# dsforza96/yocto-hair

Hardware: AMD Instinct MI355X
Metric: Msamples/sec (whole node), 720x720x1536spp sphere-hairblock; per-pixel L2 vs CPU ref (higher is better)
Workload: dtype f32

## Files before the change

include/yhair.h:

```cpp
#ifndef YHAIR_H_
#define YHAIR_H_

#include <stdint.h>

#ifdef __cplusplus
extern "C" {
#endif

#define YH_OK 0
#define YH_E_INVALID -1
#define YH_E_DEVICE -2
#define YH_E_STATE -3
#define YH_E_IO -4
#define YH_E_SELFTEST -5


typedef struct yh_shape {
  int          num_vertices;
  const float* positions;
  const float* normals;
  const float* radius;
  int          num_lines;
  const int*   lines;
  int          num_triangles;
  const int*   triangles;
  const float* texcoords;
} yh_shape;

typedef struct yh_texture {
  int         width, height;
  int         is_byte;
  const void* pixels;
} yh_texture;

typedef struct yh_material {
  float emission[3];
  float color[3];
  float specular, metallic, roughness, transmission, opacity, ior;
  int   thin;
  float sigma_a[3];
  float beta_m, beta_n, alpha, eta, eumelanin, pheomelanin;
  float scattering[3];
  float scanisotropy;
  float trdepth;
  int   emission_tex, color_tex, scattering_tex;
} yh_material;

typedef struct yh_material_maps {
  int specular_tex;
  int metallic_tex;
  int roughness_tex;
  int transmission_tex;
  int opacity_tex;
  int normal_tex;
} yh_material_maps;

typedef struct yh_object {
  float frame[12];
  int   shape;
  int   material;
} yh_object;

typedef struct yh_environment {
  float        frame[12];
  float        emission[3];
  int          tex_width, tex_height;
  const float* texels;
} yh_environment;

typedef struct yh_camera {
  float frame[12];
  float lens;
  float film[2];
  float focus;
  float aperture;
} yh_camera;

typedef struct yh_scene_desc {
  int                   num_shapes;
  const yh_shape*       shapes;
  int                   num_materials;
  const yh_material*    materials;
  int                   num_objects;
  const yh_object*      objects;
  int                   num_environments;
  const yh_environment* environments;
  yh_camera             camera;
  int                   num_textures;
  const yh_texture*     textures;
} yh_scene_desc;

enum {
  YH_SHADER_NAIVE    = 0,
  YH_SHADER_PATH     = 1,
  YH_SHADER_EYELIGHT = 2,
  YH_SHADER_NORMAL   = 3,
  YH_SHADER_COUNT    = 4
};

typedef struct yh_trace_params {
  int      resolution;
  int      bounces;
  float    clamp;
  uint64_t seed;
  int      shader;
  int      hair_exact;
} yh_trace_params;

typedef struct yh_workcounts {
  uint64_t samples;
  uint64_t rays;
  uint64_t nodes;
  uint64_t seg_tests;
  uint64_t tri_tests;
  uint64_t hair_shades;
  uint64_t surf_shades;
  uint64_t env_lookups;
  uint64_t env_samples;
  uint64_t cyc_trace, cyc_shade, ticks_tile, wave_iters, wave_steps, lane_steps, lane_iters;
  uint64_t cyc_geom, cyc_sample, cyc_eval, cyc_rest;
  uint64_t branch[10];
} yh_workcounts;

typedef struct yh_context yh_context;


yh_context* yh_create(int device);
void        yh_destroy(yh_context* ctx);
const char* yh_last_error(const yh_context* ctx);
const char* yh_version(void);


int yh_upload_scene(yh_context* ctx, const yh_scene_desc* scene);
int yh_upload_scene_maps(yh_context* ctx, const yh_scene_desc* scene, const yh_material_maps* maps);

int yh_init_state(yh_context* ctx, const yh_trace_params* params);
int yh_image_size(const yh_context* ctx, int* width, int* height);

int yh_set_shard(yh_context* ctx, int rank, int world);

int yh_trace_samples(yh_context* ctx, int nsamples);
int yh_trace_samples_async(yh_context* ctx, int nsamples);
int yh_synchronize(yh_context* ctx);

int yh_download(yh_context* ctx, float* rgba);
int yh_pack_tiles_device(yh_context* ctx, void* device_rgba, int64_t capacity,
    int64_t* count);
int yh_unpack_tiles_device(yh_context* ctx, const void* device_packed,
    int src_rank, int world, void* device_image);
int64_t yh_shard_pixels(const yh_context* ctx, int rank, int world);

int yh_gather_framebuffer(yh_context** contexts, int n, float* rgba);

int yh_download_rng(yh_context* ctx, uint64_t* state_inc);

int yh_trace_samples_counted(yh_context* ctx, int nsamples, yh_workcounts* out);

int yh_last_trace_ms(const yh_context* ctx, float* ms, int* launches);

int yh_launch_shape(const yh_context* ctx);
int yh_kernel_trials(const yh_context* ctx, double* ms_per_sample, int* trials, int count);
int yh_trials_pending(const yh_context* ctx);
int         yh_set_trial_cache_dir(const char* dir);
const char* yh_default_trial_cache_dir(void);

int yh_tile_costs(yh_context* ctx, uint32_t* ticks, int count);
int yh_item_costs(yh_context* ctx, uint32_t* costs, int count);


#define YH_HAIR_BRDF_FLOATS 30

enum {
  YH_LOBE_DIFFUSE            = 0,
  YH_LOBE_SPECULAR           = 1,
  YH_LOBE_METAL              = 2,
  YH_LOBE_TRANSMISSION       = 3,
  YH_LOBE_REFRACTION         = 4,
  YH_LOBE_DELTA_SPECULAR     = 5,
  YH_LOBE_DELTA_METAL        = 6,
  YH_LOBE_DELTA_TRANSMISSION = 7,
  YH_LOBE_DELTA_REFRACTION   = 8,
  YH_LOBE_COUNT              = 9
};
#define YH_SURFACE_BSDF_FLOATS 29

int yh_hair_brdf_batch(yh_context* ctx, int n, const yh_material* materials,
    const float* v, const float* normal, const float* tangent, float* brdf);
int yh_hair_eval_batch(yh_context* ctx, int n, const float* brdf,
    const float* outgoing, const float* incoming, float* f);
int yh_hair_sample_batch(yh_context* ctx, int n, const float* brdf,
    const float* outgoing, const float* rn, float* incoming);
int yh_hair_pdf_batch(yh_context* ctx, int n, const float* brdf,
    const float* outgoing, const float* incoming, float* pdf);
int yh_hair_eval_pdf_batch(yh_context* ctx, int n, const float* brdf,
    const float* outgoing, const float* incoming, float* pdf);

int yh_curves_to_lines(yh_context* ctx, int n, const float* P, const float* width0,
    const float* width1, int base_vertex, float* positions, float* normals,
    float* radius, int* lines);

int yh_bvh_build(int n, const float* boxes, float* nodes, int* primitives);
int yh_bvh_build_wide(int n, const float* boxes, int width, float* slots);

int yh_bvh_build_gpu(yh_context* ctx, int n, const float* boxes, float* nodes, int* primitives);
int yh_bvh_build_wide_gpu(yh_context* ctx, int n, const float* boxes, int width, float* slots);

int yh_surface_lobe_batch(yh_context* ctx, int kind, int n, const float* params,
    const float* normal, const float* outgoing, const float* incoming,
    const float* rn, float* out);
int yh_surface_bsdf_batch(yh_context* ctx, int n, const yh_material* materials,
    const float* normal, const float* outgoing, const float* incoming,
    const float* rn, float* out);
int yh_intersect_batch(yh_context* ctx, int n, const float* rays, int* object,
    int* element, float* uv, float* distance);

int yh_lights_batch(yh_context* ctx, int form, int n, const float* position,
    const float* direction, const float* rn, float* out);

int yh_selftest(yh_context* ctx, int which, float* worst);

typedef struct yh_scene_file yh_scene_file;
yh_scene_file*       yh_scene_load(const char* json_path, const char* camera,
          char* error, int error_len);
const yh_scene_desc* yh_scene_get(const yh_scene_file* scene);
const yh_material_maps* yh_scene_get_maps(const yh_scene_file* scene);
void                 yh_scene_free(yh_scene_file* scene);
int yh_save_image(const char* path, int width, int height, const float* rgba,
    char* error, int error_len);

#ifdef __cplusplus
}
#endif
#endif
```

yocto-hair_amd/csrc/dev_items.h:

```cpp
#ifndef YH_DEV_ITEMS_H_
#define YH_DEV_ITEMS_H_
#include "dev_path.h"

using namespace yhd;

#define YH_BLOCK 512
#define YH_MIN_WAVES 4

#define YH_QUADS (YH_BLOCK / 4)
template <bool COUNT, bool GENERAL, int BLOCK, int SHADER, int MODE = YH_MODE_QUAD>
YH_DEV void trace_items(const yhd_scene& sc, const yhd_state& st, int nsamples, yhd_counters* counters, unsigned int block = blockIdx.x,
    unsigned int blocks = gridDim.x) {
  constexpr int LPP    = YH_IS_HEX(MODE) ? 16 : YH_IS_OCT(MODE) ? 8 : 4;
  constexpr int GROUPS = BLOCK / LPP;
  extern __shared__ v4f lds_dyn[];
  YH_LDS unsigned int* lds_stack = (YH_LDS unsigned int*)lds_dyn;
  YH_LDS v4f*          lds_tabs  = (YH_LDS v4f*)(lds_stack + ((MODE == YH_MODE_QUAD ? sc.stack_entries : YH_IS_HEX(MODE) ? sc.stack_entries16 : sc.stack_entries8) + YH_HITROWS) * GROUPS);
  trace_ctx tc;
  tc.sc = &sc;
  tc.ls = nullptr, tc.sc_dev = nullptr;
  YH_LDS float* lds_cam;
  stage_tables(sc, lds_tabs, threadIdx.x, blockDim.x, tc, lds_cam);
  __syncthreads();

  tc.lds_stack = lds_stack + (threadIdx.x / LPP);
  stats_t stats = {};
  tc.stats = COUNT ? &stats : nullptr;

  const int lane = threadIdx.x & 63;
  const int by_position = (int)(blocks * (BLOCK / 64));
  int       t_first     = __builtin_amdgcn_readfirstlane((int)(block * (BLOCK / 64) + (threadIdx.x >> 6)));
  while (true) {
    int t = t_first;
    if (t < 0) {
      if (lane == 0) t = atomicAdd(st.tile_cursor, 1);
      t = __builtin_amdgcn_readfirstlane(t) + by_position;
    }
    t_first = -1;
    if (t >= st.num_tiles) break;
    unsigned long long t0 = wall_clock64();
    int  item  = st.tiles[t];
    int  half  = 0;
    if (YH_IS_OCT(MODE)) half = item & 1, item >>= 1;
    if (YH_IS_HEX(MODE)) half = item & 3, item >>= 2;
    int  tile  = item >> 2, part = item & 3;
    int  pq    = YH_IS_HEX(MODE) ? half * 4 + (lane >> 4) : YH_IS_OCT(MODE) ? half * 8 + (lane >> 3) : lane >> 2;
    int  i     = (tile % st.tiles_x) * YH_TILE + (part & 1) * 4 + (pq & 3);
    int  j     = (tile / st.tiles_x) * YH_TILE + (part >> 1) * 4 + (pq >> 2);
    bool owner = i < st.width && j < st.height;
    size_t pix = owner ? (size_t)j * st.width + i : 0;
    rng_t  rng;
    rng.state      = st.rng_state[pix];
    rng.inc        = st.rng_inc[pix];
    yhd_float4 acc = st.accum[pix];
    int    left    = owner ? nsamples : 0;
    bool   alive   = false;
    path_t ps;
    ps.bounce = 0, ps.hit = false;
    unsigned long long cyc_trace = 0, cyc_shade = 0;
    unsigned int       w_iters = 0, w_steps = 0, l_steps = 0, l_iters = 0;
    while (true) {
      if (!alive && left > 0) {
        yhd_camera cam;
        for (int k = 0; k < 12; k++) cam.frame[k] = lds_cam[k];
        cam.lens = lds_cam[12], cam.film_x = lds_cam[13], cam.film_y = lds_cam[14], cam.focus = lds_cam[15], cam.aperture = lds_cam[16];
        path_begin(cam, ps, rng, i, j, st.width, st.height);
        left--;
        alive = true;
      }
      if (!__any(alive)) break;
      unsigned long long c0 = 0, c1 = 0;
      unsigned int       steps = 0;
      if (COUNT) c0 = clock64(), l_iters += (alive && (lane & 3) == 0) ? 1 : 0, w_iters++;
      hit_t isec;
      if (alive) {
        if (COUNT) count_quad<COUNT>(stats.rays);
        isec = trace_ray<COUNT, GROUPS, !GENERAL, MODE>(tc, ps.ray, -1, &steps);
      }
      if (COUNT) {
        c1 = clock64(), cyc_trace += c1 - c0;
        unsigned int smax = steps;
        for (int off = 32; off > 0; off >>= 1) smax = max(smax, (unsigned int)__shfl_xor((int)smax, off, 64));
        w_steps += smax, l_steps += (lane & 3) == 0 ? steps : 0;
      }
      if (alive) {
        if constexpr (SHADER == YH_SHADER_PATH) alive = path_step<COUNT, GROUPS, GENERAL>(tc, ps, isec, rng, st.bounces);
        else alive = shade_step<COUNT, GROUPS, SHADER>(tc, ps, isec, rng, st.bounces);
        if (!alive) {
          path_end(ps, st.clamp, acc);
          if (COUNT) count_quad<COUNT>(stats.samples);
        }
      }
      if (COUNT) cyc_shade += clock64() - c1;
    }
    if (COUNT) {
      unsigned int v[11] = {stats.samples, stats.rays, stats.nodes, stats.seg, stats.tri, stats.hair, stats.surf,
          stats.envl, stats.envs, l_steps, l_iters};
      for (int k = 0; k < 11; k++)
        for (int off = 32; off > 0; off >>= 1) v[k] += (unsigned int)__shfl_xor((int)v[k], off, 64);
      if (lane == 0) {
        atomicAdd(&counters->samples, (unsigned long long)v[0]), atomicAdd(&counters->rays, (unsigned long long)v[1]);
        atomicAdd(&counters->nodes, (unsigned long long)v[2]), atomicAdd(&counters->seg, (unsigned long long)v[3]);
        atomicAdd(&counters->tri, (unsigned long long)v[4]), atomicAdd(&counters->hair, (unsigned long long)v[5]);
        atomicAdd(&counters->surf, (unsigned long long)v[6]), atomicAdd(&counters->envl, (unsigned long long)v[7]);
        atomicAdd(&counters->envs, (unsigned long long)v[8]);
        atomicAdd(&counters->lane_steps, (unsigned long long)v[9]), atomicAdd(&counters->lane_iters, (unsigned long long)v[10]);
        atomicAdd(&counters->cyc_trace, cyc_trace), atomicAdd(&counters->cyc_shade, cyc_shade);
        atomicAdd(&counters->wave_iters, (unsigned long long)w_iters), atomicAdd(&counters->wave_steps, (unsigned long long)w_steps);
      }
      if (lane == 0) {
        atomicAdd(&counters->c_geom, stats.c_geom), atomicAdd(&counters->c_sample, stats.c_sample);
        atomicAdd(&counters->c_eval, stats.c_eval), atomicAdd(&counters->c_rest, stats.c_rest);
      }
      {
        unsigned int b[10] = {stats.t_node, stats.l_node, stats.t_line, stats.l_line, stats.t_tri, stats.l_tri, stats.t_enter,
            stats.l_enter, stats.t_scene, stats.l_scene};
        for (int k = 0; k < 10; k++) {
          for (int off = 32; off > 0; off >>= 1) b[k] += (unsigned int)__shfl_xor((int)b[k], off, 64);
          if (lane == 0) atomicAdd(&counters->branch[k], (unsigned long long)b[k]);
        }
      }
      stats = stats_t{};
    }
    if (owner && (lane & (LPP - 1)) == 0) {
      st.rng_state[pix] = rng.state;
      st.accum[pix]     = acc;
    }
    if (lane == 0) {
      unsigned int dt = (unsigned int)(wall_clock64() - t0);
      if (YH_IS_OCT(MODE) || YH_IS_HEX(MODE)) atomicAdd(&st.tile_cost[item], dt);
      else st.tile_cost[item] = dt;
      if (COUNT) atomicAdd(&counters->cyc_tile, (unsigned long long)dt);
    }
  }
}
typedef void (*trace_kernel_t)(const yhd_scene, const yhd_state, int, yhd_counters*);
#define YH_OCT_BLOCK 256
template <bool COUNT, bool GENERAL, int BLOCK, int WAVES, int MODE = YH_MODE_QUAD>
__global__ __launch_bounds__(BLOCK, WAVES) void k_trace(const yhd_scene sc, const yhd_state st,
    int nsamples, yhd_counters* counters) {
  trace_items<COUNT, GENERAL, BLOCK, YH_SHADER_PATH, MODE>(sc, st, nsamples, counters);
}
template <bool GENERAL>
__global__ __launch_bounds__(YH_BLOCK, YH_MIN_WAVES) void k_trace_sbs(const yhd_scene sc, const yhd_state st, int nsamples, int oct_blocks,
    int quad_items, int oct_entries) {
  if ((int)blockIdx.x < oct_blocks) {
    yhd_state so   = st;
    so.tiles       = st.tiles + quad_items, so.num_tiles = oct_entries, so.tile_cursor = st.tile_cursor + 16;
    trace_items<false, GENERAL, YH_BLOCK, YH_SHADER_PATH, YH_MODE_OCT>(sc, so, nsamples, nullptr, blockIdx.x, (unsigned)oct_blocks);
  } else {
    yhd_state sq = st;
    sq.num_tiles = quad_items;
    trace_items<false, GENERAL, YH_BLOCK, YH_SHADER_PATH, YH_MODE_QUAD>(sc, sq, nsamples, nullptr, blockIdx.x - (unsigned)oct_blocks, gridDim.x - (unsigned)oct_blocks);
  }
}
#endif
```

yocto-hair_amd/csrc/dev_trace.h:

```cpp
#ifndef YH_DEV_TRACE_H_
#define YH_DEV_TRACE_H_
#include "dev_math.h"

namespace yhd {

struct rng_t {
  uint64_t state, inc;
};
YH_DEV uint32_t advance_rng(rng_t& rng) {
  uint64_t old        = rng.state;
  rng.state           = old * 6364136223846793005ULL + rng.inc;
  uint32_t xorshifted = (uint32_t)(((old >> 18u) ^ old) >> 27u);
  uint32_t rot        = (uint32_t)(old >> 59u);
  return (xorshifted >> rot) | (xorshifted << ((-rot) & 31));
}
YH_DEV float rand1f(rng_t& rng) {
  return __uint_as_float((advance_rng(rng) >> 9) | 0x3f800000u) - 1.0f;
}
YH_DEV rng_t make_rng(uint64_t seed, uint64_t seq) {
  rng_t rng;
  rng.state = 0U;
  rng.inc   = (seq << 1u) | 1u;
  advance_rng(rng);
  rng.state += seed;
  advance_rng(rng);
  return rng;
}

struct ray_t {
  f3    o, d;
  float tmin, tmax;
};
YH_DEV ray_t mkray(f3 o, f3 d) { return ray_t{o, d, ray_eps, flt_max}; }

struct hit_t {
  int   object, slot;
  float u, v, distance;
};

template <bool STRAIGHT = false, bool RAW = false>
YH_DEV bool intersect_line(f3 ro, f3 rd, float tmin, float tmax, f3 p0, f3 p1, float r0,
    float r1, float& uu, float& vv, float& dist, float a_in = 0.0f, float* rr = nullptr) {
  f3    u = rd, v = p1 - p0, w = ro - p0;
  float a = RAW ? a_in : dot(u, u), b = dot(u, v), c = dot(v, v), d = dot(u, w), e = dot(v, w);
  float det = a * c - b * b;
  if (STRAIGHT) {
    float t   = (b * e - c * d) / det;
    float s   = (a * e - b * d) / det;
    bool  ok  = det != 0 && !(t < tmin || t > tmax);
    s         = fclamp(s, 0.0f, 1.0f);
    f3    pr  = ro + rd * t;
    f3    pl  = p0 + (p1 - p0) * s;
    f3    prl = pr - pl;
    float d2  = dot(prl, prl);
    float r   = r0 * (1 - s) + r1 * s;
    ok        = ok && !(d2 > r * r);
    if (RAW) {
      uu = s, vv = d2, *rr = r, dist = t;
      return ok;
    }
    if (ok) uu = s, vv = sqrtf(d2) / r, dist = t;
    return ok;
  }
  if (det == 0) return false;
  float t = (b * e - c * d) / det;
  float s = (a * e - b * d) / det;
  if (t < tmin || t > tmax) return false;
  s        = fclamp(s, 0.0f, 1.0f);
  f3    pr = ro + rd * t;
  f3    pl = p0 + (p1 - p0) * s;
  f3    prl = pr - pl;
  float d2  = dot(prl, prl);
  float r   = r0 * (1 - s) + r1 * s;
  if (d2 > r * r) return false;
  if (RAW) uu = s, vv = d2, *rr = r;
  else uu = s, vv = sqrtf(d2) / r;
  dist = t;
  return true;
}
YH_DEV bool intersect_triangle(f3 ro, f3 rd, float tmin, float tmax, f3 p0, f3 p1, f3 p2,
    float& uu, float& vv, float& dist) {
  f3    edge1 = p1 - p0, edge2 = p2 - p0;
  f3    pvec = cross(rd, edge2);
  float det  = dot(edge1, pvec);
  if (det == 0) return false;
  float inv_det = 1.0f / det;
  f3    tvec    = ro - p0;
  float u       = dot(tvec, pvec) * inv_det;
  if (u < 0 || u > 1) return false;
  f3    qvec = cross(tvec, edge1);
  float v    = dot(rd, qvec) * inv_det;
  if (v < 0 || u + v > 1) return false;
  float t = dot(edge2, qvec) * inv_det;
  if (t < tmin || t > tmax) return false;
  uu = u, vv = v;
  dist = t;
  return true;
}
YH_DEV bool intersect_bbox(f3 ro, f3 dinv, float tmin_, float tmax_, f3 bmin, f3 bmax) {
  f3    it_min = (bmin - ro) * dinv;
  f3    it_max = (bmax - ro) * dinv;
  f3    tmin   = {fmin_(it_min.x, it_max.x), fmin_(it_min.y, it_max.y), fmin_(it_min.z, it_max.z)};
  f3    tmax   = {fmax_(it_min.x, it_max.x), fmax_(it_min.y, it_max.y), fmax_(it_min.z, it_max.z)};
  float t0     = fmax_(hmax(tmin), tmin_);
  float t1     = fmin_(hmin(tmax), tmax_);
  t1 *= 1.00000024f;
  return t0 <= t1;
}

YH_DEV bool intersect_bbox_nonan(f3 ro, f3 dinv, float tmin_, float tmax_, f3 bmin, f3 bmax) {
  f3    it_min = (bmin - ro) * dinv;
  f3    it_max = (bmax - ro) * dinv;
  float t0 = __builtin_fmaxf(__builtin_fmaxf(__builtin_fminf(it_min.x, it_max.x), __builtin_fminf(it_min.y, it_max.y)),
      __builtin_fmaxf(__builtin_fminf(it_min.z, it_max.z), tmin_));
  float t1 = __builtin_fminf(__builtin_fminf(__builtin_fmaxf(it_min.x, it_max.x), __builtin_fmaxf(it_min.y, it_max.y)),
      __builtin_fminf(__builtin_fmaxf(it_min.z, it_max.z), tmax_));
  t1 *= 1.00000024f;
  return t0 <= t1;
}

#define YH_TAG_SHAPE 0u
#define YH_TAG_SCENE 0x40000000u
#define YH_TAG_ENTER 0x80000000u
#define YH_TAG_LEAF 0xC0000000u
#define YH_TAG_MASK 0xC0000000u
#define YH_NONE 0xFFFFFFFFu

#define YH_QSTACK 96
#define YH_HITROWS 4
#define YH_LDS __attribute__((address_space(3)))
typedef float v4f __attribute__((ext_vector_type(4)));

struct lane_stack;
struct trace_ctx {
  const yhd_scene*      sc;
  YH_LDS unsigned int*  lds_stack;
  const YH_LDS v4f*     lds_scene;
  struct stats_t*       stats;
  const YH_LDS v4f*     lds_lights;
  const YH_LDS float*   lds_envtab;
  const YH_LDS v4f*     lds_mats;
  lane_stack*           ls;
  const yhd_scene*      sc_dev;
};
YH_DEV void stage_tables(const yhd_scene& sc, YH_LDS v4f* at, int tid, int nthreads, trace_ctx& tc, YH_LDS float*& lds_cam) {
  tc.lds_scene = nullptr, tc.lds_lights = nullptr, tc.lds_envtab = nullptr, tc.lds_mats = nullptr;
  if (sc.lds_scene_f4 > 0) {
    const int  nobj = YH_OBJECT_F4 * sc.num_objects, nnod = 2 * sc.num_scene_nodes, npri = (sc.num_objects + 3) / 4;
    const v4f* gobj = (const v4f*)sc.objects;
    const v4f* gpri = (const v4f*)sc.scene_prims;
    for (int i = tid; i < nobj; i += nthreads) at[i] = gobj[i];
    for (int i = tid; i < nnod; i += nthreads) at[nobj + i] = *(const v4f*)(sc.scene_nodes + i);
    for (int i = tid; i < npri; i += nthreads) at[nobj + nnod + i] = gpri[i];
    tc.lds_scene = at;
  }
  lds_cam = (YH_LDS float*)(at + sc.lds_scene_f4);
  if (tid < 17) lds_cam[tid] = ((const float*)&sc.camera)[tid];
  YH_LDS v4f* lights = at + sc.lds_scene_f4 + 5;
  if (sc.light_table_f4 > 0) {
    for (int i = tid; i < sc.light_table_f4; i += nthreads) lights[i] = *(const v4f*)(sc.light_table + i);
    tc.lds_lights = lights;
  }
  YH_LDS float* envtab = (YH_LDS float*)(lights + sc.light_table_f4);
  if (sc.env_tab_k > 0) {
    for (int i = tid; i < sc.env_tab_k; i += nthreads) envtab[i] = sc.env_tab[i];
    tc.lds_envtab = envtab;
  }
  YH_LDS v4f* mats = (YH_LDS v4f*)(envtab + (sc.env_tab_k + 3) / 4 * 4);
  if (sc.lds_materials > 0) {
    const v4f* gm = (const v4f*)sc.materials;
    for (int i = tid; i < YH_MATERIAL_F4 * sc.lds_materials; i += nthreads) mats[i] = gm[i];
    tc.lds_mats = mats;
  }
}

struct stats_t {
  unsigned int samples, rays, nodes, seg, tri, hair, surf, envl, envs;
  unsigned long long c_geom, c_sample, c_eval, c_rest;
  unsigned int t_node, l_node, t_line, l_line, t_tri, l_tri, t_enter, l_enter, t_scene, l_scene;
};
template <bool COUNT>
YH_DEV void count_branch(unsigned int& trips, unsigned int& lanes) {
  if (COUNT) {
    unsigned long long m = __ballot(1);
    if ((int)__lane_id() == __ffsll((long long)m) - 1) trips++, lanes += (unsigned int)__popcll(m);
  }
}
YH_DEV v4f ldg4(const yhd_float4* p) { return *(const v4f*)p; }
YH_DEV f3  xyz(v4f a) { return f3{a.x, a.y, a.z}; }

template <bool COUNT>
YH_DEV void count_quad(unsigned int& slot) {
  if (COUNT && (__lane_id() & 3u) == 0) slot++;
}

#define YH_MODE_QUAD 0
#define YH_MODE_OCT 2
#define YH_MODE_HEX 3
#define YH_ROW_HALF_MIRROR 0x141
#define YH_ROW_MIRROR 0x140
#define YH_MODE_OCTP 4
#define YH_IS_OCT(MODE) ((MODE) == YH_MODE_OCT || (MODE) == YH_MODE_OCTP)
#define YH_MODE_HEXP 5
#define YH_IS_HEX(MODE) ((MODE) == YH_MODE_HEX || (MODE) == YH_MODE_HEXP)
template <bool COUNT, int STRIDE, bool EXACT, bool LDS_SCENE = false, int MODE = YH_MODE_QUAD>
YH_DEV hit_t trace_ray_loop(const trace_ctx& tc, const ray_t& ray, int first_object, unsigned int* steps_out, bool& redo) {
  const yhd_scene&     sc   = *tc.sc;
  const unsigned int   q    = __lane_id() & 3u;
  const unsigned int   q_   = q;
  int                  sp   = 0;
  YH_LDS unsigned int* hrec = tc.lds_stack;
#define YH_STK(i) hrec[((i) + YH_HITROWS) * STRIDE]
  auto push = [&](unsigned int v) { YH_STK(sp) = v, sp++; };
  auto pop  = [&]() -> unsigned int { sp--; return YH_STK(sp); };
  hit_t hit;
  hit.object = -1, hit.slot = -1, hit.u = 0, hit.v = 0, hit.distance = 0;
  float tmax = ray.tmax;
  f3  wdinv = quad_rcp(ray.d);
  const int wsign = (wdinv.x < 0 ? 1 : 0) | (wdinv.y < 0 ? 2 : 0) | (wdinv.z < 0 ? 4 : 0);
  const bool wnonan = finite3(wdinv) && finite3(ray.o);
  auto box_test = [](f3 o, f3 dinv, float t0, float t1, f3 bmin, f3 bmax) {
    return EXACT ? intersect_bbox(o, dinv, t0, t1, bmin, bmax) : intersect_bbox_nonan(o, dinv, t0, t1, bmin, bmax);
  };
  if (!EXACT && !wnonan) {
    redo = true;
    return hit;
  }
  f3    lo = ray.o, ld = ray.d, ldinv = wdinv;
  constexpr bool HOIST_A = STRIDE != 64;
  float ld2 = 0.0f;
  int   lsign = wsign | (wsign << 4), cur_obj = -1, kind = 0, node_base = 0;
  unsigned long long n_nodes = 0, n_seg = 0, n_tri = 0;
  unsigned int       n_steps = 0;

  const bool in_lds = LDS_SCENE || tc.lds_scene != nullptr;
  const bool wide_scene = !LDS_SCENE && sc.scene_wide_root >= 0;
  const YH_LDS v4f* lds_snodes = in_lds ? tc.lds_scene + YH_OBJECT_F4 * sc.num_objects : nullptr;
  auto scene_prim = [&](int i) -> int {
    if (in_lds) return ((const YH_LDS int*)(lds_snodes + 2 * sc.num_scene_nodes))[i];
    return sc.scene_prims[i];
  };
  unsigned int cur;
  if (first_object >= 0) {
    cur = YH_TAG_ENTER | (unsigned)first_object;
  } else {
    if (sc.num_scene_nodes == 0) return hit;
    cur = YH_TAG_SCENE | 0u;
  }
  while (true) {
    if (COUNT) n_steps++;
    if (cur == YH_NONE) {
      if (sp == 0) break;
      cur = pop();
    }
    unsigned int tag = cur & YH_TAG_MASK;
    bool scene_node = false;
    if (!LDS_SCENE && tag == YH_TAG_SCENE && wide_scene) {
      if (COUNT) count_branch<COUNT>(tc.stats->t_scene, tc.stats->l_scene);
      const unsigned int low = cur & ~YH_TAG_MASK;
      if (low >= (1u << 27)) {
        const int start = (int)(low & 0x07FFFFFFu), num = (int)(low >> 27);
        if ((int)q >= 1 && (int)q < num) YH_STK(sp + (num - 1 - (int)q)) = YH_TAG_ENTER | (unsigned)sc.scene_prims[start + (int)q];
        sp += num - 1;
        cur = YH_TAG_ENTER | (unsigned)sc.scene_prims[start];
        tag = YH_TAG_ENTER;
      } else {
        scene_node = true;
        lo = ray.o, ldinv = wdinv, lsign = (lsign & 0x70) | (lsign >> 4);
        cur = low;
        tag = YH_TAG_SHAPE;
      }
    } else if (tag == YH_TAG_SCENE) {
      if (COUNT) count_branch<COUNT>(tc.stats->t_scene, tc.stats->l_scene);
      int idx = (int)(cur & ~YH_TAG_MASK);
      v4f n0, n1;
      if (in_lds) n0 = lds_snodes[2 * idx], n1 = lds_snodes[2 * idx + 1];
      else n0 = ldg4(sc.scene_nodes + 2 * idx), n1 = ldg4(sc.scene_nodes + 2 * idx + 1);
      if (q == 0) n_nodes++;
      cur = YH_NONE;
      if (box_test(ray.o, wdinv, ray.tmin, tmax, xyz(n0), xyz(n1))) {
        int start = __float_as_int(n0.w), meta = __float_as_int(n1.w);
        if (meta & 0x10000) {
          int axis = (meta >> 24) & 3;
          int near = (lsign >> (4 + axis)) & 1;
          push(YH_TAG_SCENE | (unsigned)(start + 1 - near));
          cur = YH_TAG_SCENE | (unsigned)(start + near);
        } else {
          int num = meta & 0xffff;
          if ((int)q >= 1 && (int)q < num) YH_STK(sp + (num - 1 - (int)q)) = YH_TAG_ENTER | (unsigned)scene_prim(start + (int)q);
          sp += num > 1 ? num - 1 : 0;
          if (num > 0) cur = YH_TAG_ENTER | (unsigned)scene_prim(start);
        }
      }
      tag = cur & YH_TAG_MASK;
      if (cur == YH_NONE || tag == YH_TAG_SCENE) continue;
    }
    if (tag == YH_TAG_ENTER) {
      if (COUNT) count_branch<COUNT>(tc.stats->t_enter, tc.stats->l_enter);
      cur_obj             = (int)(cur & ~YH_TAG_MASK);
      if (wnonan) {
        v4f bmin, bmax;
        if (in_lds) {
          const YH_LDS v4f* ob = tc.lds_scene + YH_OBJECT_F4 * cur_obj;
          bmin = ob[8], bmax = ob[9];
        } else {
          const yhd_object& o = sc.objects[cur_obj];
          bmin = v4f{o.wbox_min[0], o.wbox_min[1], o.wbox_min[2], 0}, bmax = v4f{o.wbox_max[0], o.wbox_max[1], o.wbox_max[2], 0};
        }
        if (!box_test(ray.o, wdinv, ray.tmin, tmax, xyz(bmin), xyz(bmax))) {
          cur = YH_NONE;
          continue;
        }
      }
      frame inv;
      if (in_lds) {
        const YH_LDS v4f* ob = tc.lds_scene + YH_OBJECT_F4 * cur_obj;
        v4f a = ob[3], b = ob[4], c = ob[5], d = ob[6];
        inv.x = {a.x, a.y, a.z}, inv.y = {a.w, b.x, b.y}, inv.z = {b.z, b.w, c.x}, inv.o = {c.y, c.z, c.w};
        kind = __float_as_int(d.x);
        node_base = __float_as_int(YH_IS_HEX(MODE) ? ob[10].w : YH_IS_OCT(MODE) ? ob[10].z : ob[10].x);
      } else {
        const yhd_object& o = sc.objects[cur_obj];
        inv       = ldframe(o.inv_frame);
        kind      = o.kind;
        node_base = YH_IS_HEX(MODE) ? o.lane_root16 : YH_IS_OCT(MODE) ? o.lane_root8 : o.lane_root;
      }
      lo    = transform_point(inv, ray.o);
      ld    = transform_vector(inv, ray.d);
      ldinv = quad_rcp(ld);
      lsign = (lsign & 0x70) | (ldinv.x < 0 ? 1 : 0) | (ldinv.y < 0 ? 2 : 0) | (ldinv.z < 0 ? 4 : 0);
      if (!EXACT && !(finite3(ldinv) && finite3(lo))) {
        redo = true;
        break;
      }
      if (HOIST_A) ld2 = dot(ld, ld);
      cur = YH_TAG_SHAPE | (unsigned)node_base;
      tag = YH_TAG_SHAPE;
    }
    {
      bool is_leaf    = tag == YH_TAG_LEAF;
      constexpr bool     GROUPS = MODE == YH_MODE_OCTP || MODE == YH_MODE_HEXP;
      const unsigned int qj     = MODE == YH_MODE_HEXP ? (__lane_id() >> 2) & 3u : MODE == YH_MODE_OCTP ? (__lane_id() >> 2) & 1u : 0u;
      int                grp    = 0;
      bool               idle   = false;
      unsigned int       mycur  = cur;
      if (GROUPS) {
        const bool   look = is_leaf && qj > 0 && sp >= (int)qj;
        unsigned int pk   = look ? YH_STK(sp - (int)qj) : 0u;
        unsigned int lb   = (look && (pk & YH_TAG_MASK) == YH_TAG_LEAF) ? (1u << qj) : 0u;
        lb |= (unsigned int)dpp_i<YH_ROW_HALF_MIRROR>((int)lb);
        if (MODE == YH_MODE_HEXP) lb |= (unsigned int)dpp_i<YH_ROW_MIRROR>((int)lb);
        grp   = (lb & 2u) ? ((lb & 4u) ? ((lb & 8u) ? 3 : 2) : 1) : 0;
        idle  = is_leaf && (int)qj > grp;
        mycur = (qj > 0 && !idle) ? pk : cur;
      }
      int  leaf_start = (int)(mycur & 0x07FFFFFFu), leaf_num = (int)((mycur >> 27) & 7u);
      bool mine       = !is_leaf || (int)q < leaf_num;
      int  pq         = mine ? (int)q : leaf_num - 1;
      const unsigned int nslot = (MODE == YH_MODE_QUAD || scene_node) ? q : (__lane_id() & (YH_IS_HEX(MODE) ? 15u : 7u));
      const yhd_float4*  addr  = sc.lane_blob + 2 * (size_t)(is_leaf ? (unsigned)leaf_start + (unsigned)pq * (kind == YH_KIND_LINES ? 1u : 2u) : cur + nslot);
      if (GROUPS) mine = mine && !idle;
      const v4f s0 = ldg4(addr), s1 = ldg4(addr + 1);
      if (YH_IS_HEX(MODE) && !is_leaf && !scene_node) {
        if (q == 0) n_nodes++;
        if (COUNT) count_branch<COUNT>(tc.stats->t_node, tc.stats->l_node);
        const unsigned int o    = __lane_id() & 15u;
        const unsigned int axes = __float_as_uint(s1.w);
        const unsigned int n0   = (lsign >> (axes & 3)) & 1;
        const unsigned int n1   = (lsign >> ((axes >> (2 + 2 * (o >> 3))) & 3)) & 1;
        const unsigned int n2   = (lsign >> ((axes >> (6 + 2 * (o >> 2))) & 3)) & 1;
        const unsigned int n3   = (lsign >> ((axes >> (14 + 2 * (o >> 1))) & 3)) & 1;
        const unsigned int rank = (((o >> 3) ^ n0) << 3) | ((((o >> 2) & 1) ^ n1) << 2) | ((((o >> 1) & 1) ^ n2) << 1) | ((o & 1) ^ n3);
        unsigned int ref = __float_as_uint(s1.z);
        const bool   h   = box_test(lo, ldinv, ray.tmin, tmax, f3{s0.x, s0.y, s0.z}, f3{s0.w, s1.x, s1.y}) && ref != YH_NONE;
        unsigned int bits = h ? (1u << rank) : 0u;
        unsigned int M    = bits | (unsigned int)dpp_i<YH_QUAD_XOR1>((int)bits);
        M |= (unsigned int)dpp_i<YH_QUAD_XOR2>((int)M);
        M |= (unsigned int)dpp_i<YH_ROW_HALF_MIRROR>((int)M);
        M |= (unsigned int)dpp_i<YH_ROW_MIRROR>((int)M);
        const bool first = h && (1u << rank) == (M & (0u - M));
        if (h && !first) YH_STK(sp + (int)__popc(M >> (rank + 1))) = ref;
        unsigned int mine = first ? ref : 0u;
        mine |= (unsigned int)dpp_i<YH_QUAD_XOR1>((int)mine);
        mine |= (unsigned int)dpp_i<YH_QUAD_XOR2>((int)mine);
        mine |= (unsigned int)dpp_i<YH_ROW_HALF_MIRROR>((int)mine);
        mine |= (unsigned int)dpp_i<YH_ROW_MIRROR>((int)mine);
        int nh = __popc(M);
        sp += nh > 0 ? nh - 1 : 0;
        cur = nh > 0 ? mine : YH_NONE;
      } else if (MODE != YH_MODE_QUAD && !is_leaf && !scene_node) {
        if (q == 0) n_nodes++;
        if (COUNT) count_branch<COUNT>(tc.stats->t_node, tc.stats->l_node);
        const unsigned int axes = __float_as_uint(s1.w);
        const unsigned int g    = (__lane_id() & 7u) >> 1;
        const unsigned int n0   = (lsign >> (axes & 3)) & 1;
        const unsigned int n1   = (lsign >> ((axes >> (2 + 2 * (g >> 1))) & 3)) & 1;
        const unsigned int n2   = (lsign >> ((axes >> (6 + 2 * g)) & 3)) & 1;
        const unsigned int rank = ((((g >> 1) ^ n0) << 2) | (((g & 1) ^ n1) << 1)) | ((__lane_id() & 1u) ^ n2);
        const unsigned int ref  = __float_as_uint(s1.z);
        const bool         h    = box_test(lo, ldinv, ray.tmin, tmax, f3{s0.x, s0.y, s0.z}, f3{s0.w, s1.x, s1.y}) && ref != YH_NONE;
        unsigned int bits = h ? (1u << rank) : 0u;
        unsigned int M    = bits | (unsigned int)dpp_i<YH_QUAD_XOR1>((int)bits);
        M |= (unsigned int)dpp_i<YH_QUAD_XOR2>((int)M);
        M |= (unsigned int)dpp_i<YH_ROW_HALF_MIRROR>((int)M);
        const bool first = h && (1u << rank) == (M & (0u - M));
        if (h && !first) YH_STK(sp + (int)__popc(M >> (rank + 1))) = ref;
        unsigned int mine = first ? ref : 0u;
        mine |= (unsigned int)dpp_i<YH_QUAD_XOR1>((int)mine);
        mine |= (unsigned int)dpp_i<YH_QUAD_XOR2>((int)mine);
        mine |= (unsigned int)dpp_i<YH_ROW_HALF_MIRROR>((int)mine);
        int nh = __popc(M);
        sp += nh > 0 ? nh - 1 : 0;
        cur = nh > 0 ? mine : YH_NONE;
      } else if (!is_leaf) {
        if (q == 0) n_nodes++;
        if (COUNT) count_branch<COUNT>(tc.stats->t_node, tc.stats->l_node);
        bool h = box_test(lo, ldinv, ray.tmin, tmax, f3{s0.x, s0.y, s0.z}, f3{s0.w, s1.x, s1.y});
        unsigned int ref  = __float_as_uint(s1.z);
        unsigned int axes = __float_as_uint(s1.w);
        h = h && ref != YH_NONE;
        if (!LDS_SCENE && scene_node) ref = (ref & ~YH_TAG_MASK) | YH_TAG_SCENE;
        unsigned int q = q_;
        if (STRIDE == 64) {
          unsigned int x;
          asm volatile("v_mbcnt_lo_u32_b32 %0, -1, 0\n\tv_mbcnt_hi_u32_b32 %0, -1, %0" : "=v"(x));
          q = x & 3u;
        }
        unsigned int pair = q >> 1;
        unsigned int sgn  = (lsign >> ((axes >> (2 + 2 * pair)) & 3)) & 1;
        unsigned int s0_  = (lsign >> (axes & 3)) & 1;
        unsigned int rank = ((pair ^ s0_) << 1) | ((q & 1) ^ sgn);
        unsigned int bit  = h ? (1u << rank) : 0u;
        unsigned int M    = bit | (unsigned int)dpp_i<YH_QUAD_XOR1>((int)bit);
        M |= (unsigned int)dpp_i<YH_QUAD_XOR2>((int)M);
        bool         first = h && (M & (bit - 1)) == 0;
        unsigned int after = (unsigned int)__popc(M >> (rank + 1));
        if (h && !first) YH_STK(sp + (int)after) = ref;
        unsigned int mine = first ? ref : 0u;
        mine |= (unsigned int)dpp_i<YH_QUAD_XOR1>((int)mine);
        mine |= (unsigned int)dpp_i<YH_QUAD_XOR2>((int)mine);
        int nh = __popc(M);
        sp += nh > 0 ? nh - 1 : 0;
        cur = nh > 0 ? mine : YH_NONE;
      } else {
        cur = YH_NONE;
        bool  ok = false;
        float uu = 0, vv = 0, dist = 0, rr = 1.0f;
        if (kind == YH_KIND_LINES) {
          if (COUNT) count_branch<COUNT>(tc.stats->t_line, tc.stats->l_line);
          if (mine) {
            n_seg++;
            ok = intersect_line<(STRIDE == 64), true>(lo, ld, ray.tmin, tmax, xyz(s0), xyz(s1), s0.w, s1.w, uu, vv, dist, HOIST_A ? ld2 : dot(ld, ld), &rr);
          }
        } else {
          if (COUNT) count_branch<COUNT>(tc.stats->t_tri, tc.stats->l_tri);
          v4f s2 = ldg4(addr + 2);
          if (mine) {
            n_tri++;
            ok = intersect_triangle(lo, ld, ray.tmin, tmax, xyz(s0), xyz(s1), xyz(s2), uu, vv, dist);
          }
        }
        const int my_i  = (int)(4 * qj + q);
        int       key_i = ok ? my_i : -1;
        float     key_t = dist;
        int       slot  = leaf_start + (int)q * (kind == YH_KIND_LINES ? 1 : 2);
#define YH_KEY_MERGE(CTRL, WITH_SLOT)                                                      \
  {                                                                                        \
    int   oi = dpp_i<CTRL>(key_i);                                                         \
    float ot = dpp_f<CTRL>(key_t);                                                         \
    bool  take = (oi >= 0) & ((key_i < 0) | (ot < key_t) | ((ot == key_t) & (oi > key_i)));  \
    if (WITH_SLOT) {                                                                       \
      int os = dpp_i<CTRL>(slot);                                                          \
      slot   = take ? os : slot;                                                           \
    }                                                                                      \
    key_i = take ? oi : key_i, key_t = take ? ot : key_t;                                  \
  }
        YH_KEY_MERGE(YH_QUAD_XOR1, false)
        YH_KEY_MERGE(YH_QUAD_XOR2, false)
        if (GROUPS) {
          slot = leaf_start + (key_i & 3) * (kind == YH_KIND_LINES ? 1 : 2);
          YH_KEY_MERGE(YH_ROW_HALF_MIRROR, true)
          if (MODE == YH_MODE_HEXP) YH_KEY_MERGE(YH_ROW_MIRROR, true)
          sp -= grp;
        } else {
          slot = leaf_start + (key_i & 3) * (kind == YH_KIND_LINES ? 1 : 2);
        }
#undef YH_KEY_MERGE
        if (key_i >= 0) {
          hit.object = cur_obj, hit.slot = slot;
          hit.distance = key_t;
          tmax = key_t;
          if (key_i == my_i) hrec[0] = __float_as_uint(uu), hrec[STRIDE] = __float_as_uint(vv), hrec[2 * STRIDE] = __float_as_uint(rr);
        }
      }
    }
  }
  if (hit.object >= 0) {
    int hk, lt;
    if (in_lds) {
      const YH_LDS v4f* ob = tc.lds_scene + YH_OBJECT_F4 * hit.object;
      hk = __float_as_int(ob[6].x), lt = __float_as_int(ob[10].y);
    } else {
      hk = sc.objects[hit.object].kind, lt = sc.objects[hit.object].lane_test;
    }
    hit.slot = hk == YH_KIND_LINES ? hit.slot - lt : (hit.slot - lt) >> 1;
    {
      const float hu = __uint_as_float(hrec[0]), hv = __uint_as_float(hrec[STRIDE]), hr = __uint_as_float(hrec[2 * STRIDE]);
      hit.u = hu, hit.v = hk == YH_KIND_LINES ? sqrtf(hv) / hr : hv;
    }
  }
  if (COUNT) {
    if (steps_out) *steps_out = n_steps;
    tc.stats->nodes += (unsigned int)n_nodes, tc.stats->seg += (unsigned int)n_seg, tc.stats->tri += (unsigned int)n_tri;
  }
  return hit;
}
#undef YH_STK

template <bool COUNT, int STRIDE, bool LDS_SCENE = false, int MODE = YH_MODE_QUAD>
YH_DEV hit_t trace_ray(const trace_ctx& tc, const ray_t& ray, int first_object, unsigned int* steps_out = nullptr) {
  bool  redo = false;
  hit_t hit  = trace_ray_loop<COUNT, STRIDE, false, LDS_SCENE, MODE>(tc, ray, first_object, steps_out, redo);
  if (__any(redo)) {
    if (redo) hit = trace_ray_loop<COUNT, STRIDE, true, LDS_SCENE, MODE>(tc, ray, first_object, steps_out, redo);
  }
  return hit;
}

YH_DEV int hit_element(const yhd_scene& sc, const hit_t& hit) {
  if (hit.object < 0) return -1;
  const yhd_object& o = sc.objects[hit.object];
  if (o.kind == YH_KIND_LINES) return __float_as_int(sc.prims[(size_t)o.prim_base + (size_t)hit.slot * 4 + 2].w);
  return __float_as_int(sc.prims[(size_t)o.prim_base + (size_t)hit.slot * 6].w);
}

}
#endif
```

yocto-hair_amd/csrc/kernels.hip:

```cpp
#include <hip/hip_runtime.h>

#include <algorithm>
#include <cstdlib>
#include <cstring>

#include "yhair.h"
#include "dev_items.h"

template <int SHADER>
__global__ __launch_bounds__(YH_BLOCK, YH_MIN_WAVES) void k_trace_shader(const yhd_scene sc, const yhd_state st,
    int nsamples, yhd_counters* counters) {
  trace_items<false, true, YH_BLOCK, SHADER>(sc, st, nsamples, counters);
}

__global__ void k_resolve(const yhd_state st, int samples, yhd_float4* image) {
  int lane = threadIdx.x;
  int tile = st.shard_rank + blockIdx.x * st.shard_world;
  int i    = (tile % st.tiles_x) * YH_TILE + (lane & 7);
  int j    = (tile / st.tiles_x) * YH_TILE + (lane >> 3);
  if (i >= st.width || j >= st.height) return;
  size_t     pix = (size_t)j * st.width + i;
  yhd_float4 a   = st.accum[pix];
  float      n   = (float)samples;
  image[pix]     = samples > 0 ? yhd_float4{a.x / n, a.y / n, a.z / n, a.w / n} : yhd_float4{0, 0, 0, 0};
}
__global__ void k_pack(const yhd_state st, int samples, yhd_float4* packed) {
  int lane = threadIdx.x;
  int tile = st.shard_rank + blockIdx.x * st.shard_world;
  int i    = (tile % st.tiles_x) * YH_TILE + (lane & 7);
  int j    = (tile / st.tiles_x) * YH_TILE + (lane >> 3);
  yhd_float4 out = {0, 0, 0, 0};
  if (i < st.width && j < st.height && samples > 0) {
    yhd_float4 a = st.accum[(size_t)j * st.width + i];
    float      n = (float)samples;
    out          = yhd_float4{a.x / n, a.y / n, a.z / n, a.w / n};
  }
  packed[(size_t)blockIdx.x * 64 + lane] = out;
}
__global__ void k_unpack(const yhd_float4* packed, int src_rank, int world, int num_tiles_total,
    int tiles_x, int width, int height, yhd_float4* image) {
  int k = blockIdx.x, lane = threadIdx.x;
  int tile = src_rank + k * world;
  if (tile >= num_tiles_total) return;
  int i = (tile % tiles_x) * YH_TILE + (lane & 7);
  int j = (tile / tiles_x) * YH_TILE + (lane >> 3);
  if (i < width && j < height) image[(size_t)j * width + i] = packed[(size_t)k * 64 + lane];
}

YH_DEV void unpack_brdf(const float* b, yhd_material& m, hair_hit& hh) {
  m.sigma_a[0] = b[0], m.sigma_a[1] = b[1], m.sigma_a[2] = b[2];
  m.alpha = b[3], m.eta = b[4];
  hh.h = b[5];
  for (int p = 0; p < 4; p++) m.v[p] = b[6 + p];
  m.s = b[10];
  for (int k = 0; k < 3; k++) m.sin_2k_alpha[k] = b[11 + k], m.cos_2k_alpha[k] = b[14 + k];
  hh.gamma_o = b[17];
  hh.w2b     = ldframe(b + 18);
  derive_material(m);
}

#include "yhair.h"
typedef yh_material yh_material_in;
template <int N>
YH_DEV float powt(float v) {
  if constexpr (N == 0) return 1;
  else if constexpr (N == 1) return v;
  else {
    float n2 = powt<N / 2>(v);
    return n2 * n2 * powt<(N & 1)>(v);
  }
}
__global__ void k_hair_brdf(int n, const yh_material_in* mats, const float* v, const float* nrm,
    const float* tng, float* out) {
  int i = blockIdx.x * blockDim.x + threadIdx.x;
  if (i >= n) return;
  const yh_material_in& m = mats[i];
  f3 sigma_a = mk3(0.0f);
  f3 msa = ld3(m.sigma_a), col = ld3(m.color);
  if (!is_zero(msa)) {
    sigma_a = msa;
  } else if (!is_zero(col)) {
    float bn  = m.beta_n;
    float den = 5.969f - 0.215f * bn + 2.532f * sqr(bn) - 10.73f * powt<3>(bn) +
                5.574f * powt<4>(bn) + 0.245f * powt<5>(bn);
    f3 q    = f3{logf(col.x), logf(col.y), logf(col.z)} / den;
    sigma_a = q * q;
  } else if (m.eumelanin != 0 || m.pheomelanin != 0) {
    sigma_a = m.eumelanin * f3{0.419f, 0.697f, 1.37f} + m.pheomelanin * f3{0.187f, 0.4f, 1.05f};
  }
  float bm = m.beta_m, bn = m.beta_n;
  float* o = out + 30 * (size_t)i;
  o[0] = sigma_a.x, o[1] = sigma_a.y, o[2] = sigma_a.z;
  o[3] = m.alpha, o[4] = m.eta;
  hair_hit hh = hair_setup(v[i], ld3(nrm + 3 * i), ld3(tng + 3 * i));
  o[5]     = hh.h;
  float v0 = sqr(0.726f * bm + 0.812f * sqr(bm) + 3.7f * powt<20>(bm));
  o[6] = v0, o[7] = 0.25f * v0, o[8] = 4 * v0, o[9] = 4 * v0;
  o[10] = 0.626657069f * (0.265f * bn + 1.194f * sqr(bn) + 5.372f * powt<22>(bn));
  float s0 = sinf(pif / 180 * m.alpha);
  float c0 = exact_safe_sqrt(1 - sqr(s0));
  float s1 = 2 * c0 * s0, c1 = sqr(c0) - sqr(s0);
  float s2 = 2 * c1 * s1, c2 = sqr(c1) - sqr(s1);
  o[11] = s0, o[12] = s1, o[13] = s2, o[14] = c0, o[15] = c1, o[16] = c2;
  o[17] = hh.gamma_o;
  const frame& w = hh.w2b;
  o[18] = w.x.x, o[19] = w.x.y, o[20] = w.x.z, o[21] = w.y.x, o[22] = w.y.y, o[23] = w.y.z;
  o[24] = w.z.x, o[25] = w.z.y, o[26] = w.z.z, o[27] = w.o.x, o[28] = w.o.y, o[29] = w.o.z;
}
__global__ void k_hair_eval(int n, const float* brdf, const float* wo, const float* wi, float* out) {
  int  i     = (blockIdx.x * blockDim.x + threadIdx.x) >> 2;
  bool valid = i < n;
  if (!valid) i = n - 1;
  yhd_material m;
  hair_hit     hh;
  unpack_brdf(brdf + 30 * (size_t)i, m, hh);
  f3    f;
  float pdf;
  hair_eval_pdf_quad(m, hh, ld3(wo + 3 * i), ld3(wi + 3 * i), f, pdf);
  if (valid && (threadIdx.x & 3) == 0) out[3 * i] = f.x, out[3 * i + 1] = f.y, out[3 * i + 2] = f.z;
}
__global__ void k_hair_pdf(int n, const float* brdf, const float* wo, const float* wi, float* out) {
  int  i     = (blockIdx.x * blockDim.x + threadIdx.x) >> 2;
  bool valid = i < n;
  if (!valid) i = n - 1;
  yhd_material m;
  hair_hit     hh;
  unpack_brdf(brdf + 30 * (size_t)i, m, hh);
  f3    f;
  float pdf;
  hair_eval_pdf_quad(m, hh, ld3(wo + 3 * i), ld3(wi + 3 * i), f, pdf);
  if (valid && (threadIdx.x & 3) == 0) out[i] = pdf;
}
__global__ void k_hair_sample(int n, const float* brdf, const float* wo, const float* rn, float* out) {
  int i = blockIdx.x * blockDim.x + threadIdx.x;
  if (i >= n) return;
  yhd_material m;
  hair_hit     hh;
  unpack_brdf(brdf + 30 * (size_t)i, m, hh);
  f3 w = hair_sample(m, hh, ld3(wo + 3 * i), rn[2 * i], rn[2 * i + 1]);
  out[3 * i] = w.x, out[3 * i + 1] = w.y, out[3 * i + 2] = w.z;
}
__global__ __launch_bounds__(256) void k_intersect(const yhd_scene sc, int n, const float* rays, int* object,
    int* element, float* uv, float* dist) {
  __shared__ unsigned int stacks[(YH_QSTACK + YH_HITROWS) * 64];
  int  i     = (blockIdx.x * blockDim.x + threadIdx.x) >> 2;
  bool valid = i < n;
  if (!valid) i = n - 1;
  trace_ctx tc;
  tc.sc = &sc, tc.stats = nullptr, tc.lds_scene = nullptr, tc.ls = nullptr, tc.sc_dev = nullptr, tc.lds_lights = nullptr, tc.lds_envtab = nullptr, tc.lds_mats = nullptr;
  tc.lds_stack   = (YH_LDS unsigned int*)stacks + (threadIdx.x >> 2);
  const float* r = rays + 8 * (size_t)i;
  ray_t ray      = ray_t{ld3(r), ld3(r + 3), r[6], r[7]};
  hit_t h        = trace_ray<false, 64>(tc, ray, -1);
  if (valid && (threadIdx.x & 3) == 0) {
    object[i] = h.object, element[i] = hit_element(sc, h);
    uv[2 * i] = h.u, uv[2 * i + 1] = h.v, dist[i] = h.distance;
  }
}

YH_DEV uint64_t pcg_advance(uint64_t state, uint64_t inc, uint64_t delta) {
  uint64_t cur_mult = 6364136223846793005ULL, cur_plus = inc, acc_mult = 1u, acc_plus = 0u;
  while (delta > 0) {
    if (delta & 1) {
      acc_mult *= cur_mult;
      acc_plus = acc_plus * cur_mult + cur_plus;
    }
    cur_plus = (cur_mult + 1) * cur_plus;
    cur_mult *= cur_mult;
    delta /= 2;
  }
  return acc_mult * state + acc_plus;
}
YH_DEV f3 sample_sphere(float rx, float ry) {
  float z   = 2 * ry - 1;
  float r   = sqrtf(fclamp(1 - z * z, 0.0f, 1.0f));
  float phi = 2 * pif * rx;
  return f3{r * cosf(phi), r * sinf(phi), z};
}
struct selftest_args {
  int      which;
  float    beta_m, beta_n;
  uint64_t state, inc;
  int      count;
  float    wo[3];
};
__global__ void k_selftest(selftest_args a, double* sums, unsigned int* worst_bits) {
  int   i = blockIdx.x * blockDim.x + threadIdx.x;
  float s0[3] = {0, 0, 0}, s1[3] = {0, 0, 0};
  float dev = 0.0f;
  if (i < a.count) {
    int   per_iter = a.which == 2 ? 5 : 3;
    rng_t rng;
    rng.inc   = a.inc;
    rng.state = pcg_advance(a.state, a.inc, (uint64_t)per_iter * (uint64_t)i);
    float h   = rand1f(rng);
    if (a.which == 0 && h == 0) h += 1.1920929e-07f;
    yhd_material m;
    m.sigma_a[0] = m.sigma_a[1] = m.sigma_a[2] = 0;
    m.alpha = 0, m.eta = 1.55f;
    float bm = a.beta_m, bn = a.beta_n;
    m.v[0] = sqr(0.726f * bm + 0.812f * sqr(bm) + 3.7f * powt<20>(bm));
    m.v[1] = 0.25f * m.v[0], m.v[2] = 4 * m.v[0], m.v[3] = m.v[2];
    m.s    = 0.626657069f * (0.265f * bn + 1.194f * sqr(bn) + 5.372f * powt<22>(bn));
    float s_0 = sinf(pif / 180 * m.alpha), c_0 = exact_safe_sqrt(1 - sqr(s_0));
    m.sin_2k_alpha[0] = s_0, m.cos_2k_alpha[0] = c_0;
    for (int k = 1; k < 3; k++) {
      m.sin_2k_alpha[k] = 2 * m.cos_2k_alpha[k - 1] * m.sin_2k_alpha[k - 1];
      m.cos_2k_alpha[k] = sqr(m.cos_2k_alpha[k - 1]) - sqr(m.sin_2k_alpha[k - 1]);
    }
    derive_material(m);
    hair_hit hh = hair_setup(h, f3{0, 0, 1}, f3{1, 0, 0});
    f3 wo = ld3(a.wo);
    if (a.which == 2) {
      float wx = rand1f(rng), wy = rand1f(rng);
      wo = sample_sphere(wx, wy);
    }
    float rx = rand1f(rng), ry = rand1f(rng);
    f3    f;
    float pdf;
    if (a.which == 0) {
      f3 wi = sample_sphere(rx, ry);
      hair_eval_pdf<true, false>(m, hh, wo, wi, f, pdf);
      s0[0] = f.x, s0[1] = f.y, s0[2] = f.z;
    } else {
      f3 wi = hair_sample(m, hh, wo, rx, ry);
      hair_eval_pdf<true, true>(m, hh, wo, wi, f, pdf);
      if (a.which == 1) {
        if (pdf > 0) s0[0] = f.x / pdf, s0[1] = f.y / pdf, s0[2] = f.z / pdf;
      } else if (a.which == 2) {
        if (pdf > 0) dev = fabs_(luminance(f) / pdf - 1);
      } else {
        float li = wi.z * wi.z;
        if (pdf > 0) s0[0] = f.x * li / pdf, s0[1] = f.y * li / pdf, s0[2] = f.z * li / pdf;
        f3 wu = sample_sphere(rx, ry);
        f3 fu;
        hair_eval_pdf<true, false>(m, hh, wo, wu, fu, pdf);
        float lu = wu.z * wu.z;
        s1[0] = fu.x * lu, s1[1] = fu.y * lu, s1[2] = fu.z * lu;
      }
    }
  }
  for (int k = 0; k < 3; k++) {
    double a0 = s0[k], a1 = s1[k];
    for (int off = 32; off > 0; off >>= 1) {
      a0 += __shfl_down(a0, off, 64);
      a1 += __shfl_down(a1, off, 64);
    }
    if ((threadIdx.x & 63) == 0) {
      atomicAdd(&sums[k], a0);
      atomicAdd(&sums[3 + k], a1);
    }
  }
  for (int off = 32; off > 0; off >>= 1) dev = fmaxf(dev, __shfl_down(dev, off, 64));
  if ((threadIdx.x & 63) == 0) atomicMax(worst_bits, __float_as_uint(dev));
}

__global__ void k_surface_lobe(int kind, int n, const float* params, const float* normal, const float* wo_,
    const float* wi_, const float* rn, float* out) {
  int i = blockIdx.x * blockDim.x + threadIdx.x;
  if (i >= n) return;
  const float* q = params + 8 * (size_t)i;
  float ior = q[0], rough = q[1];
  f3    eta = ld3(q + 2), etak = ld3(q + 5);
  f3    nn = ld3(normal + 3 * (size_t)i), wo = ld3(wo_ + 3 * (size_t)i), wi = ld3(wi_ + 3 * (size_t)i);
  float rnl = rn[3 * (size_t)i], rx = rn[3 * (size_t)i + 1], ry = rn[3 * (size_t)i + 2];
  f3    f = mk3(0.0f), w = mk3(0.0f);
  float pdf = 0;
  switch (kind) {
    case 0:
      f = eval_diffuse_reflection(nn, wo, wi), pdf = sample_diffuse_reflection_pdf(nn, wo, wi);
      w = sample_diffuse_reflection(nn, wo, rx, ry);
      break;
    case 1:
      f = eval_microfacet_reflection(ior, rough, nn, wo, wi), pdf = sample_microfacet_reflection_pdf(rough, nn, wo, wi);
      w = sample_microfacet_reflection(rough, nn, wo, rx, ry);
      break;
    case 2:
      f   = eval_microfacet_reflection(eta, etak, rough, nn, wo, wi);
      pdf = sample_microfacet_reflection_pdf(rough, nn, wo, wi);
      w   = sample_microfacet_reflection(rough, nn, wo, rx, ry);
      break;
    case 3:
      f = eval_microfacet_transmission(rough, nn, wo, wi), pdf = sample_microfacet_transmission_pdf(rough, nn, wo, wi);
      w = sample_microfacet_transmission(rough, nn, wo, rx, ry);
      break;
    case 4:
      f   = eval_microfacet_refraction(ior, rough, nn, wo, wi);
      pdf = sample_microfacet_refraction_pdf(ior, rough, nn, wo, wi);
      w   = sample_microfacet_refraction(ior, rough, nn, wo, rnl, rx, ry);
      break;
    case 5:
      f = eval_delta_reflection(ior, nn, wo, wi), pdf = sample_delta_reflection_pdf(nn, wo, wi);
      w = sample_delta_reflection(nn, wo);
      break;
    case 6:
      f = eval_delta_reflection(eta, etak, nn, wo, wi), pdf = sample_delta_reflection_pdf(nn, wo, wi);
      w = sample_delta_reflection(nn, wo);
      break;
    case 7:
      f = eval_delta_transmission(nn, wo, wi), pdf = sample_delta_transmission_pdf(nn, wo, wi);
      w = sample_delta_transmission(nn, wo);
      break;
    case 8:
      f = eval_delta_refraction(ior, nn, wo, wi), pdf = sample_delta_refraction_pdf(ior, nn, wo, wi);
      w = sample_delta_refraction(ior, nn, wo, rnl);
      break;
    default: break;
  }
  float* o = out + 7 * (size_t)i;
  o[0] = f.x, o[1] = f.y, o[2] = f.z, o[3] = pdf, o[4] = w.x, o[5] = w.y, o[6] = w.z;
}
__global__ void k_surface_bsdf(int n, const yhd_material* mats, const float* normal, const float* wo_,
    const float* wi_, const float* rn, float* out) {
  int i = blockIdx.x * blockDim.x + threadIdx.x;
  if (i >= n) return;
  f3    nn = ld3(normal + 3 * (size_t)i), wo = ld3(wo_ + 3 * (size_t)i), wi = ld3(wi_ + 3 * (size_t)i);
  float rnl = rn[3 * (size_t)i], rx = rn[3 * (size_t)i + 1], ry = rn[3 * (size_t)i + 2];
  surface_brdf_t b = surface_brdf(mats[i], nn, wo);
  float* o = out + 29 * (size_t)i;
  f3 lobes[5] = {b.diffuse, b.specular, b.metal, b.transmission, b.refraction};
  for (int k = 0; k < 5; k++) o[3 * k] = lobes[k].x, o[3 * k + 1] = lobes[k].y, o[3 * k + 2] = lobes[k].z;
  o[15] = b.roughness, o[16] = b.opacity;
  o[17] = b.diffuse_pdf, o[18] = b.specular_pdf, o[19] = b.metal_pdf, o[20] = b.transmission_pdf;
  o[21] = b.refraction_pdf;
  f3    f, w;
  float pdf;
  if (!is_delta(b)) {
    surface_eval_pdf(b, nn, wo, wi, f, pdf);
    w = surface_sample(b, nn, wo, rnl, rx, ry);
  } else {
    surface_eval_pdf_delta(b, nn, wo, wi, f, pdf);
    w = surface_sample_delta(b, nn, wo, rnl);
  }
  o[22] = f.x, o[23] = f.y, o[24] = f.z, o[25] = pdf, o[26] = w.x, o[27] = w.y, o[28] = w.z;
}

__global__ void k_curves_to_lines(int n, const float* P, const float* width0, const float* width1, int base_vertex,
    float* positions, float* normals, float* radius, int* lines) {
  long long t = (long long)blockIdx.x * blockDim.x + threadIdx.x;
  if (t >= 5ll * n) return;
  int c = (int)(t / 5), i = (int)(t % 5);
  const float* q = P + 12 * (size_t)c;
  f3 p0 = ld3(q), p1 = ld3(q + 3), p2 = ld3(q + 6), p3 = ld3(q + 9);
  f3    pos, tan;
  float rad;
  if (i == 0) {
    pos = p0, tan = normalize(p1 - p0), rad = width0[c];
  } else if (i == 4) {
    pos = p3, tan = normalize(p3 - p2), rad = width1[c];
  } else {
    float u = (float)i / 4;
    pos = p0 * (1 - u) * (1 - u) * (1 - u) + p1 * 3 * u * (1 - u) * (1 - u) + p2 * 3 * u * u * (1 - u) + p3 * u * u * u;
    tan = normalize((p1 - p0) * 3 * (1 - u) * (1 - u) + (p2 - p1) * 6 * u * (1 - u) + (p3 - p2) * 3 * u * u);
    rad = width0[c] * (1 - u) + width1[c] * u;
  }
  size_t v = (size_t)t;
  positions[3 * v] = pos.x, positions[3 * v + 1] = pos.y, positions[3 * v + 2] = pos.z;
  normals[3 * v] = tan.x, normals[3 * v + 1] = tan.y, normals[3 * v + 2] = tan.z;
  radius[v] = rad;
  if (i < 4) lines[8 * (size_t)c + 2 * i] = base_vertex + (int)t, lines[8 * (size_t)c + 2 * i + 1] = base_vertex + (int)t + 1;
}

extern "C" {

trace_kernel_t yhk_wide_kernel(int counted, int general, int shape);
#define YH_DENSE_WAVES 5
static_assert(yhd_shapes[YH_SHAPE_QUAD].block_threads == YH_BLOCK && yhd_shapes[YH_SHAPE_OCT].block_threads == YH_OCT_BLOCK && yhd_shapes[YH_SHAPE_HEX].block_threads == YH_OCT_BLOCK, "yhd_shapes");
static int shape_block(int shape) { return yhd_shapes[shape].block_threads; }
static int shape_groups(int shape) { return shape_block(shape) / yhd_shapes[shape].lanes_per_path; }
static trace_kernel_t trace_kernel(bool counted, bool general, int shape, int shader = YH_SHADER_PATH) {
  if (shader == YH_SHADER_NAIVE) return k_trace_shader<YH_SHADER_NAIVE>;
  if (shader == YH_SHADER_EYELIGHT) return k_trace_shader<YH_SHADER_EYELIGHT>;
  if (shader == YH_SHADER_NORMAL) return k_trace_shader<YH_SHADER_NORMAL>;
  if (yhd_shapes[shape].kind == YH_SHAPE_KIND_WIDE) return yhk_wide_kernel(counted ? 1 : 0, general ? 1 : 0, shape);
  if (yhd_shapes[shape].kind == YH_SHAPE_KIND_RETIRED) return nullptr;
  if (general && !counted && shape == YH_SHAPE_QUAD_DENSE) return k_trace<false, true, 256, YH_DENSE_WAVES - 1>;
  if (shape == YH_SHAPE_QUAD_DENSE)
    return counted ? (general ? k_trace<true, true, 256, YH_DENSE_WAVES> : k_trace<true, false, 256, YH_DENSE_WAVES>)
                   : (general ? k_trace<false, true, 256, YH_DENSE_WAVES> : k_trace<false, false, 256, YH_DENSE_WAVES>);
  return counted ? (general ? k_trace<true, true, YH_BLOCK, YH_MIN_WAVES> : k_trace<true, false, YH_BLOCK, YH_MIN_WAVES>)
                 : (general ? k_trace<false, true, YH_BLOCK, YH_MIN_WAVES> : k_trace<false, false, YH_BLOCK, YH_MIN_WAVES>);
}
static size_t trace_lds(const yhd_scene* sc, int shape) {
  const int lanes   = yhd_shapes[shape].lanes_per_path;
  const int entries = lanes == 16 ? sc->stack_entries16 : lanes == 8 ? sc->stack_entries8 : sc->stack_entries;
  return (size_t)(entries + YH_HITROWS) * shape_groups(shape) * 4 + (size_t)YHD_LDS_TABLES_F4(sc) * 16;
}
int yhk_trace(const yhd_scene* sc, const yhd_state* st, int nsamples, yhd_counters* counters, int shape,
    int grid_blocks, hipStream_t stream) {
  const bool path  = st->shader == YH_SHADER_PATH;
  if (!path) shape = YH_SHAPE_QUAD;
  if (!path && counters) return (int)hipErrorInvalidValue;
  if ((unsigned)shape >= YH_SHAPES || yhd_shapes[shape].kind == YH_SHAPE_KIND_STREAM || yhd_shapes[shape].kind == YH_SHAPE_KIND_SBS) return (int)hipErrorInvalidValue;
  size_t    lds   = trace_lds(sc, shape);
  trace_kernel_t k     = trace_kernel(counters != nullptr, sc->general_materials != 0, shape, st->shader);
  if (!k) return (int)hipErrorInvalidValue;
  if (lds > 64 * 1024) {
    hipError_t e = hipFuncSetAttribute((const void*)k, hipFuncAttributeMaxDynamicSharedMemorySize, (int)lds);
    if (e != hipSuccess) return (int)e;
  }
  hipLaunchKernelGGL(k, dim3(grid_blocks), dim3(shape_block(shape)), lds, stream, *sc, *st, nsamples, counters);
  return (int)hipGetLastError();
}
int yhk_block_threads(int shape) { return shape_block(shape); }
int yhk_stack_entries(void) { return YH_QSTACK; }
int yhk_trace_lds_bytes(const yhd_scene* sc, int shape) { return (int)trace_lds(sc, shape); }
int yhk_trace_occupancy(int lds_bytes, int general, int shape) {
  int            blocks = 0;
  trace_kernel_t k      = trace_kernel(false, general != 0, shape);
  if (!k) return 0;
  if (lds_bytes > 64 * 1024 &&
      hipFuncSetAttribute((const void*)k, hipFuncAttributeMaxDynamicSharedMemorySize, lds_bytes) != hipSuccess)
    return 0;
  if (hipOccupancyMaxActiveBlocksPerMultiprocessor(&blocks, k, shape_block(shape), lds_bytes) != hipSuccess) return 1;
  return blocks < 1 ? 0 : blocks;
}
int yhk_resolve(const yhd_state* st, int owned_tiles, int samples, void* image, hipStream_t stream) {
  if (owned_tiles) hipLaunchKernelGGL(k_resolve, dim3(owned_tiles), dim3(64), 0, stream, *st, samples, (yhd_float4*)image);
  return (int)hipGetLastError();
}
int yhk_pack(const yhd_state* st, int owned_tiles, int samples, void* packed, hipStream_t stream) {
  if (owned_tiles) hipLaunchKernelGGL(k_pack, dim3(owned_tiles), dim3(64), 0, stream, *st, samples, (yhd_float4*)packed);
  return (int)hipGetLastError();
}
int yhk_unpack(const void* packed, int src_rank, int world, int ntiles_src, int num_tiles_total, int tiles_x,
    int width, int height, void* image, hipStream_t stream) {
  if (ntiles_src)
    hipLaunchKernelGGL(k_unpack, dim3(ntiles_src), dim3(64), 0, stream, (const yhd_float4*)packed, src_rank, world,
        num_tiles_total, tiles_x, width, height, (yhd_float4*)image);
  return (int)hipGetLastError();
}
int yhk_curves_to_lines(int n, const float* P, const float* w0, const float* w1, int base_vertex, float* positions,
    float* normals, float* radius, int* lines, hipStream_t s) {
  long long threads = 5ll * n;
  hipLaunchKernelGGL(k_curves_to_lines, dim3((unsigned)((threads + 255) / 256)), dim3(256), 0, s, n, P, w0, w1, base_vertex,
      positions, normals, radius, lines);
  return (int)hipGetLastError();
}
int yhk_surface_lobe(int kind, int n, const float* params, const float* normal, const float* wo, const float* wi,
    const float* rn, float* out, hipStream_t s) {
  hipLaunchKernelGGL(k_surface_lobe, dim3((n + 255) / 256), dim3(256), 0, s, kind, n, params, normal, wo, wi, rn, out);
  return (int)hipGetLastError();
}
int yhk_surface_bsdf(int n, const void* mats, const float* normal, const float* wo, const float* wi, const float* rn,
    float* out, hipStream_t s) {
  hipLaunchKernelGGL(k_surface_bsdf, dim3((n + 255) / 256), dim3(256), 0, s, n, (const yhd_material*)mats, normal, wo, wi, rn, out);
  return (int)hipGetLastError();
}
int yhk_hair_brdf(int n, const void* mats, const float* v, const float* nrm, const float* tng, float* out, hipStream_t s) {
  hipLaunchKernelGGL(k_hair_brdf, dim3((n + 255) / 256), dim3(256), 0, s, n, (const yh_material_in*)mats, v, nrm, tng, out);
  return (int)hipGetLastError();
}
int yhk_hair_eval(int n, const float* brdf, const float* wo, const float* wi, float* out, hipStream_t s) {
  hipLaunchKernelGGL(k_hair_eval, dim3((n + 63) / 64), dim3(256), 0, s, n, brdf, wo, wi, out);
  return (int)hipGetLastError();
}
int yhk_hair_pdf(int n, const float* brdf, const float* wo, const float* wi, float* out, hipStream_t s) {
  hipLaunchKernelGGL(k_hair_pdf, dim3((n + 63) / 64), dim3(256), 0, s, n, brdf, wo, wi, out);
  return (int)hipGetLastError();
}
int yhk_hair_sample(int n, const float* brdf, const float* wo, const float* rn, float* out, hipStream_t s) {
  hipLaunchKernelGGL(k_hair_sample, dim3((n + 255) / 256), dim3(256), 0, s, n, brdf, wo, rn, out);
  return (int)hipGetLastError();
}
int yhk_intersect(const yhd_scene* sc, int n, const float* rays, int* object, int* element, float* uv, float* dist,
    hipStream_t s) {
  hipLaunchKernelGGL(k_intersect, dim3((n + 63) / 64), dim3(256), 0, s, *sc, n, rays, object, element, uv, dist);
  return (int)hipGetLastError();
}
int yhk_selftest(int which, float beta_m, float beta_n, uint64_t state, uint64_t inc, int count, const float* wo,
    double* sums, unsigned int* worst_bits, hipStream_t s) {
  selftest_args a;
  a.which = which, a.beta_m = beta_m, a.beta_n = beta_n, a.state = state, a.inc = inc, a.count = count;
  a.wo[0] = wo[0], a.wo[1] = wo[1], a.wo[2] = wo[2];
  hipLaunchKernelGGL(k_selftest, dim3((count + 255) / 256), dim3(256), 0, s, a, sums, worst_bits);
  return (int)hipGetLastError();
}
}
```

yocto-hair_amd/csrc/wide.hip:

```cpp
#include <hip/hip_runtime.h>

#include <algorithm>

#include "yhair.h"
#include "dev_items.h"

extern "C" {

trace_kernel_t yhk_wide_kernel(int counted, int general, int shape) {
  if (counted && !(general ? yhd_shapes[shape].counted_general : yhd_shapes[shape].counted_plain)) return nullptr;
  if (shape == YH_SHAPE_OCT && counted && !general) return k_trace<true, false, YH_OCT_BLOCK, YH_MIN_WAVES, YH_MODE_OCT>;
  if (shape == YH_SHAPE_OCT && !counted) return general ? k_trace<false, true, YH_OCT_BLOCK, YH_MIN_WAVES, YH_MODE_OCT> : k_trace<false, false, YH_OCT_BLOCK, YH_MIN_WAVES, YH_MODE_OCT>;
  if (shape == YH_SHAPE_HEX && !counted) return general ? k_trace<false, true, YH_OCT_BLOCK, YH_MIN_WAVES, YH_MODE_HEX> : k_trace<false, false, YH_OCT_BLOCK, YH_MIN_WAVES, YH_MODE_HEX>;
  if (shape == YH_SHAPE_HEX && counted && !general) return k_trace<true, false, YH_OCT_BLOCK, YH_MIN_WAVES, YH_MODE_HEX>;
  if (shape == YH_SHAPE_OCT_PAIRS && !counted) return general ? k_trace<false, true, YH_OCT_BLOCK, YH_MIN_WAVES, YH_MODE_OCTP> : k_trace<false, false, YH_OCT_BLOCK, YH_MIN_WAVES, YH_MODE_OCTP>;
  if (shape == YH_SHAPE_HEX_GROUPS && !counted) return general ? k_trace<false, true, YH_OCT_BLOCK, YH_MIN_WAVES, YH_MODE_HEXP> : k_trace<false, false, YH_OCT_BLOCK, YH_MIN_WAVES, YH_MODE_HEXP>;
  return nullptr;
}

static size_t sbs_lds(const yhd_scene* sc) {
  const size_t stacks = (size_t)std::max((sc->stack_entries + YH_HITROWS) * (YH_BLOCK / 4), (sc->stack_entries8 + YH_HITROWS) * (YH_BLOCK / 8)) * 4;
  return stacks + (size_t)YHD_LDS_TABLES_F4(sc) * 16;
}
int yhk_trace_sbs_lds_bytes(const yhd_scene* sc) { return (int)sbs_lds(sc); }
int yhk_trace_sbs_occupancy(int lds_bytes, int general) {
  int  blocks = 0;
  auto k      = general ? k_trace_sbs<true> : k_trace_sbs<false>;
  if (lds_bytes > 64 * 1024 && hipFuncSetAttribute((const void*)k, hipFuncAttributeMaxDynamicSharedMemorySize, lds_bytes) != hipSuccess) return 0;
  if (hipOccupancyMaxActiveBlocksPerMultiprocessor(&blocks, k, YH_BLOCK, lds_bytes) != hipSuccess) return 1;
  return blocks < 1 ? 0 : blocks;
}
int yhk_trace_sbs(const yhd_scene* sc, const yhd_state* st, int nsamples, int oct_blocks, int quad_items, int oct_entries, int grid_blocks,
    hipStream_t stream) {
  const size_t lds = sbs_lds(sc);
  auto         k   = sc->general_materials ? k_trace_sbs<true> : k_trace_sbs<false>;
  if (lds > 64 * 1024) {
    hipError_t e = hipFuncSetAttribute((const void*)k, hipFuncAttributeMaxDynamicSharedMemorySize, (int)lds);
    if (e != hipSuccess) return (int)e;
  }
  hipLaunchKernelGGL(k, dim3(grid_blocks), dim3(YH_BLOCK), lds, stream, *sc, *st, nsamples, oct_blocks, quad_items, oct_entries);
  return (int)hipGetLastError();
}
}
```

yocto-hair_amd/csrc/yh_device.h:

```cpp
#ifndef YH_DEVICE_H_
#define YH_DEVICE_H_
#include <stdint.h>

#define YH_KIND_LINES 1
#define YH_KIND_TRIANGLES 2
#define YH_TILE 8
#define YH_MAX_LIGHTS 16
#define YH_MAX_ENVS 4

typedef struct yhd_float4 { float x, y, z, w; } yhd_float4;
typedef struct yhd_int4 { int x, y, z, w; } yhd_int4;

typedef struct yhd_object {
  float frame[12];
  float inv_frame[12];
  int   kind;
  int   node_base;
  int   prim_base;
  int   vert_base;
  int   elem_base;
  int   has_normals;
  int   material;
  int   has_texcoords;
  float wbox_min[4], wbox_max[4];
  int   lane_root, lane_test;
  int   lane_root8, lane_root16;
} yhd_object;
#define YH_OBJECT_F4 11

typedef struct yhd_material {
  float  emission[3];
  float  color[3];
  float  diffuse_pdf;
  int    thin;
  float  sigma_a[3];
  float  alpha, eta;
  float  v[4];
  float  s;
  float  sin_2k_alpha[3], cos_2k_alpha[3];
  float  inv_v[4];
  float  log_inv_2v[4];
  float  exp_m2_inv_v[4];
  double mp_den[4];
  float  tl_cdf_a;
  float  tl_norm;
  int    plain;
  float  specular, metallic, roughness, ior, transmission;
  float  opacity;
  float  meta[3];
  int    has_volume;
  float  vol_density[3];
  float  vol_scatter[3];
  float  vol_anisotropy;
  int    emission_tex, color_tex, scattering_tex;
  float  trdepth;
} yhd_material;

typedef struct yhd_texture {
  int width, height;
  int srgb_base, linear_base;
} yhd_texture;

typedef struct yhd_maps {
  int   specular_tex, metallic_tex, roughness_tex, opacity_tex;
  int   normal_tex;
  int   any;
  float opacity;
  int   pad;
} yhd_maps;

typedef struct yhd_light {
  int object;
  int environment;
  int cdf_base;
  int cdf_count;
  int small_base;
} yhd_light;
#define YH_SMALL_LIGHT_TRIS 4
#define YH_SMALL_LIGHT_F4 15

typedef struct yhd_environment {
  float frame[12];
  float inv_frame[12];
  float emission[3];
  int   tex_w, tex_h;
  int   texel_base;
  int   pad0, pad1;
} yhd_environment;

typedef struct yhd_camera {
  float frame[12];
  float lens, film_x, film_y, focus, aperture;
} yhd_camera;

typedef struct yhd_scene {
  const yhd_maps*   maps;
  const yhd_float4* prims;
  const yhd_float4* vpos;
  const yhd_int4*   elems;
  const yhd_object* objects;
  const yhd_material* materials;
  const yhd_float4* scene_nodes;
  const int*        scene_prims;
  int               num_scene_nodes;
  int               num_objects;
  int               num_lights;
  int               num_environments;
  yhd_light         lights[YH_MAX_LIGHTS];
  yhd_environment   environments[YH_MAX_ENVS];
  const float*      light_cdf;
  const yhd_float4* env_texels;
  const yhd_texture* textures;
  const yhd_float4* tex_texels;
  const float*      vtex;
  yhd_camera        camera;
  int               num_nodes_total;
  int               num_prim_f4;
  int               lds_scene_f4;
  int               general_materials;
  int               stack_entries;
  const yhd_float4* light_table;
  int               light_table_f4;
  int               scene_wide_root;
  const float*      env_tab;
  int               env_tab_light;
  int               env_tab_k, env_tab_stride;
  int               lds_materials;
  int               stack_entries8;
  int               stack_entries16;
  const yhd_float4* lane_blob;
  long long         lane_blob_units;
} yhd_scene;
#define YH_MATERIAL_F4 17
#define YHD_LDS_TABLES_F4(sc) ((sc)->lds_scene_f4 + 5 + (sc)->light_table_f4 + ((sc)->env_tab_k + 3) / 4 + YH_MATERIAL_F4 * (sc)->lds_materials)

typedef struct yhd_state {
  uint64_t*   rng_state;
  uint64_t*   rng_inc;
  yhd_float4* accum;
  const int*  tiles;
  int*        tile_cursor;
  int         num_groups;
  int         group_begin[9];
  unsigned int* tile_cost;
  int         num_tiles;
  int         shader;
  int         launch_shape;
  int         width, height;
  int         tiles_x;
  int         samples_done;
  int         bounces;
  float       clamp;
  int         shard_rank, shard_world;
} yhd_state;

enum yhd_shape {
  YH_SHAPE_QUAD       = 0,
  YH_SHAPE_QUAD_DENSE = 1,
  YH_SHAPE_RETIRED    = 2,
  YH_SHAPE_STREAM     = 3,
  YH_SHAPE_OCT        = 4,
  YH_SHAPE_SBS        = 5,
  YH_SHAPE_HEX        = 6,
  YH_SHAPE_OCT_PAIRS  = 7,
  YH_SHAPE_HEX_GROUPS = 8,
  YH_SHAPES
};
enum yhd_shape_kind { YH_SHAPE_KIND_QUAD, YH_SHAPE_KIND_WIDE, YH_SHAPE_KIND_STREAM, YH_SHAPE_KIND_SBS, YH_SHAPE_KIND_RETIRED };
typedef struct yhd_shape_info {
  const char* name;
  int kind;
  int entries_per_item;
  int block_threads, lanes_per_path;
  int counted_plain, counted_general;
  int fallback;
  int tie_rank;
} yhd_shape_info;
static constexpr yhd_shape_info yhd_shapes[YH_SHAPES] = {
    {"quad",       YH_SHAPE_KIND_QUAD,    1, 512, 4,  1, 1, YH_SHAPE_QUAD, 7},
    {"quad-dense", YH_SHAPE_KIND_QUAD,    1, 256, 4,  1, 1, YH_SHAPE_QUAD, 1},
    {"retired",    YH_SHAPE_KIND_RETIRED, 1, 512, 4,  0, 0, YH_SHAPE_QUAD, 8},
    {"stream",     YH_SHAPE_KIND_STREAM,  1, 256, 1,  0, 0, -1, 0},
    {"oct",        YH_SHAPE_KIND_WIDE,    2, 256, 8,  1, 0, YH_SHAPE_QUAD, 6},
    {"sbs",        YH_SHAPE_KIND_SBS,     1, 512, 4,  0, 0, YH_SHAPE_QUAD, 2},
    {"hex",        YH_SHAPE_KIND_WIDE,    4, 256, 16, 1, 0, YH_SHAPE_QUAD, 5},
    {"oct-pairs",  YH_SHAPE_KIND_WIDE,    2, 256, 8,  0, 0, YH_SHAPE_QUAD, 4},
    {"hex-groups", YH_SHAPE_KIND_WIDE,    4, 256, 16, 0, 0, YH_SHAPE_QUAD, 3},
};

typedef struct yhd_path_slot {
  yhd_float4 ray_o;
  yhd_float4 ray_d;
  yhd_float4 weight;
  yhd_int4   rngw;
  yhd_int4   hit;
  yhd_int4   hit2;
  yhd_float4 radiance;
  yhd_int4   own;
} yhd_path_slot;
typedef struct yhd_stream {
  yhd_path_slot* slots;
  yhd_float4* medium;
  unsigned int* stack_ovf;
  unsigned long long* prof;
  unsigned long long* wave_log;
  const int*  wave_begin;
  int*        wave_fill;
  int         slots_per_wave;
  int         ovf_entries;
  long long   total_slots;
  int         prof_parts_only;
  int         suspend_lanes;
} yhd_stream;

typedef struct yhd_counters {
  unsigned long long samples, rays, nodes, seg, tri, hair, surf, envl, envs;
  unsigned long long cyc_trace, cyc_shade, cyc_tile, wave_iters, wave_steps, lane_steps, lane_iters;
  unsigned long long c_geom, c_sample, c_eval, c_rest;
  unsigned long long branch[10];
} yhd_counters;

#endif
```

yocto-hair_amd/host/batch_api.cpp:

```cpp
#include "context_internal.h"

namespace {
struct Staged {
  std::vector<DevBuf> bufs;
  yh_context*         ctx;
  int                 rc = YH_OK;
  explicit Staged(yh_context* c) : ctx(c) { bufs.reserve(8); }
  void* in(const void* src, size_t bytes) {
    bufs.emplace_back();
    if (rc == YH_OK) rc = upload(ctx, bufs.back(), src, bytes);
    return bufs.back().p;
  }
  void* out(size_t bytes) {
    bufs.emplace_back();
    if (rc == YH_OK) rc = alloc_zero(ctx, bufs.back(), bytes);
    return bufs.back().p;
  }
};
int finish(yh_context* ctx, int launch_err, void* dst, const void* src, size_t bytes) {
  if (launch_err) return fail(ctx, YH_E_DEVICE, "kernel launch: %s", hipGetErrorString((hipError_t)launch_err));
  YH_WAIT(ctx);
  HIPCHK(ctx, hipMemcpy(dst, src, bytes, hipMemcpyDeviceToHost));
  return YH_OK;
}
}

int yh_hair_brdf_batch(yh_context* ctx, int n, const yh_material* materials, const float* v, const float* normal,
    const float* tangent, float* brdf) {
  if (!ctx || n < 0 || (n && (!materials || !v || !normal || !tangent || !brdf))) return YH_E_INVALID;
  if (n == 0) return YH_OK;
  HIPCHK(ctx, hipSetDevice(ctx->device));
  Staged s(ctx);
  auto   dm = s.in(materials, sizeof(yh_material) * (size_t)n);
  auto   dv = (float*)s.in(v, 4 * (size_t)n);
  auto   dn = (float*)s.in(normal, 12 * (size_t)n);
  auto   dt = (float*)s.in(tangent, 12 * (size_t)n);
  auto   o  = (float*)s.out(120 * (size_t)n);
  if (s.rc) return s.rc;
  return finish(ctx, yhk_hair_brdf(n, dm, dv, dn, dt, o, ctx->stream), brdf, o, 120 * (size_t)n);
}
static int wowi(yh_context* ctx, int n, const float* brdf, const float* a, size_t a_floats, const float* b,
    size_t b_floats, float* out, size_t out_floats, int which) {
  if (!ctx || n < 0 || (n && (!brdf || !a || !b || !out))) return YH_E_INVALID;
  if (n == 0) return YH_OK;
  HIPCHK(ctx, hipSetDevice(ctx->device));
  Staged s(ctx);
  auto   db = (float*)s.in(brdf, 120 * (size_t)n);
  auto   da = (float*)s.in(a, 4 * a_floats * n);
  auto   dbb = (float*)s.in(b, 4 * b_floats * n);
  auto   o  = (float*)s.out(4 * out_floats * n);
  if (s.rc) return s.rc;
  int e = which == 0   ? yhk_hair_eval(n, db, da, dbb, o, ctx->stream)
          : which == 1 ? yhk_hair_sample(n, db, da, dbb, o, ctx->stream)
                       : yhk_hair_pdf(n, db, da, dbb, o, ctx->stream);
  return finish(ctx, e, out, o, 4 * out_floats * n);
}
int yh_hair_eval_batch(yh_context* ctx, int n, const float* brdf, const float* wo, const float* wi, float* f) {
  return wowi(ctx, n, brdf, wo, 3, wi, 3, f, 3, 0);
}
int yh_hair_sample_batch(yh_context* ctx, int n, const float* brdf, const float* wo, const float* rn, float* wi) {
  return wowi(ctx, n, brdf, wo, 3, rn, 2, wi, 3, 1);
}
int yh_hair_pdf_batch(yh_context* ctx, int n, const float* brdf, const float* wo, const float* wi, float* pdf) {
  return wowi(ctx, n, brdf, wo, 3, wi, 3, pdf, 1, 2);
}
int yh_hair_eval_pdf_batch(yh_context* ctx, int n, const float* brdf, const float* wo, const float* wi, float* pdf) {
  return yh_hair_pdf_batch(ctx, n, brdf, wo, wi, pdf);
}

int yh_curves_to_lines(yh_context* ctx, int n, const float* P, const float* width0, const float* width1,
    int base_vertex, float* positions, float* normals, float* radius, int* lines) {
  if (!ctx || n < 0 || (n && (!P || !width0 || !width1 || !positions || !normals || !radius || !lines))) return YH_E_INVALID;
  if (n == 0) return YH_OK;
  if (n > 400000000 || base_vertex < 0 || (long long)base_vertex + 5ll * n > 2147483647ll)
    return fail(ctx, YH_E_INVALID, "too many curves for 32-bit vertex indices");
  HIPCHK(ctx, hipSetDevice(ctx->device));
  Staged s(ctx);
  auto   dp = (float*)s.in(P, 48 * (size_t)n);
  auto   d0 = (float*)s.in(width0, 4 * (size_t)n);
  auto   d1 = (float*)s.in(width1, 4 * (size_t)n);
  auto   op = (float*)s.out(60 * (size_t)n);
  auto   on = (float*)s.out(60 * (size_t)n);
  auto   orad = (float*)s.out(20 * (size_t)n);
  auto   ol = (int*)s.out(32 * (size_t)n);
  if (s.rc) return s.rc;
  int e = yhk_curves_to_lines(n, dp, d0, d1, base_vertex, op, on, orad, ol, ctx->stream);
  if (e) return fail(ctx, YH_E_DEVICE, "k_curves_to_lines launch: %s", hipGetErrorString((hipError_t)e));
  YH_WAIT(ctx);
  HIPCHK(ctx, hipMemcpy(positions, op, 60 * (size_t)n, hipMemcpyDeviceToHost));
  HIPCHK(ctx, hipMemcpy(normals, on, 60 * (size_t)n, hipMemcpyDeviceToHost));
  HIPCHK(ctx, hipMemcpy(radius, orad, 20 * (size_t)n, hipMemcpyDeviceToHost));
  HIPCHK(ctx, hipMemcpy(lines, ol, 32 * (size_t)n, hipMemcpyDeviceToHost));
  return YH_OK;
}

int yh_bvh_build_gpu(yh_context* ctx, int n, const float* boxes, float* nodes, int* primitives) {
  if (!ctx || n < 0 || (n && !boxes)) return YH_E_INVALID;
  HIPCHK(ctx, hipSetDevice(ctx->device));
  std::vector<yhh::Box> b((size_t)n);
  if (n) memcpy((void*)b.data(), boxes, sizeof(yhh::Box) * (size_t)n);
  yhh::Tree tree;
  int       rc = build_bvh_device(ctx, b, tree);
  if (rc) return rc;
  if (nodes)
    for (size_t i = 0; i < tree.nodes.size(); i++) {
      auto&  nd = tree.nodes[i];
      float* o  = nodes + 8 * i;
      memcpy(o, nd.bbox.min, 12), memcpy(o + 3, nd.bbox.max, 12);
      int a = nd.start, c = (int)nd.num | ((int)nd.internal << 16) | ((int)nd.axis << 24);
      memcpy(o + 6, &a, 4), memcpy(o + 7, &c, 4);
    }
  if (primitives && n) memcpy(primitives, tree.primitives.data(), sizeof(int) * (size_t)n);
  return (int)tree.nodes.size();
}

int yh_bvh_build_wide_gpu(yh_context* ctx, int n, const float* boxes, int width, float* slots) {
  if (!ctx || n < 1 || !boxes || (width != 4 && width != 8 && width != 16)) return YH_E_INVALID;
  HIPCHK(ctx, hipSetDevice(ctx->device));
  YH_WAIT(ctx);
  const int L = width == 4 ? 2 : width == 8 ? 3 : 4;
  DevBuf    d_boxes, d_nodes, d_pid, d_flag, d_widx, d_out;
  int       rc;
  if ((rc = upload(ctx, d_boxes, boxes, (size_t)n * 24))) return rc;
  if ((rc = alloc_zero(ctx, d_nodes, ((size_t)2 * n + 1) * 32)) || (rc = alloc_zero(ctx, d_pid, (size_t)n * 4))) return rc;
  int num_nodes = 0, levels = 0, level_first[130], count = 0;
  int e = yhk_bvh_build_resident(n, (const float*)d_boxes.p, (float*)d_nodes.p, (int*)d_pid.p, &num_nodes, &levels, level_first, ctx->stream);
  if (e) return fail(ctx, YH_E_DEVICE, "device BVH build: %s", hipGetErrorString((hipError_t)e));
  if ((rc = alloc_zero(ctx, d_flag, ((size_t)num_nodes + 1) * 4)) || (rc = alloc_zero(ctx, d_widx, ((size_t)num_nodes + 1) * 4))) return rc;
  e = yhk_wide_index(num_nodes, (const float*)d_nodes.p, levels, level_first, L, (unsigned int*)d_flag.p, (unsigned int*)d_widx.p, &count, ctx->stream);
  if (e) return fail(ctx, YH_E_DEVICE, "wide-node index: %s", hipGetErrorString((hipError_t)e));
  if (slots) {
    if ((rc = alloc_zero(ctx, d_out, (size_t)count * width * 32))) return rc;
    e = yhk_wide_collapse(L, num_nodes, (const float*)d_nodes.p, (const unsigned int*)d_flag.p, (const unsigned int*)d_widx.p, 1, 0, 0, d_out.p, ctx->stream);
    if (e) return fail(ctx, YH_E_DEVICE, "wide collapse: %s", hipGetErrorString((hipError_t)e));
    YH_WAIT(ctx);
    HIPCHK(ctx, hipMemcpy(slots, d_out.p, (size_t)count * width * 32, hipMemcpyDeviceToHost));
  }
  return count;
}

int yh_bvh_build_wide(int n, const float* boxes, int width, float* slots) {
  if (n < 0 || (n && !boxes) || (width != 4 && width != 8 && width != 16)) return YH_E_INVALID;
  std::vector<yhh::Box> b((size_t)n);
  for (int i = 0; i < n; i++)
    for (int k = 0; k < 3; k++) b[(size_t)i].min[k] = boxes[6 * (size_t)i + k], b[(size_t)i].max[k] = boxes[6 * (size_t)i + 3 + k];
  yhh::Tree tree;
  yhh::build_bvh(tree, b);
  const void* data  = nullptr;
  size_t      count = 0;
  std::vector<yhh::WideNode>   w4;
  std::vector<yhh::WideNode8>  w8;
  std::vector<yhh::WideNode16> w16;
  if (width == 4) yhh::collapse_wide(tree, w4), data = w4.data(), count = w4.size();
  if (width == 8) yhh::collapse_wide8(tree, w8), data = w8.data(), count = w8.size();
  if (width == 16) yhh::collapse_wide16(tree, w16), data = w16.data(), count = w16.size();
  if (slots && count) memcpy(slots, data, count * (size_t)width * sizeof(yhh::WideSlot));
  return (int)count;
}

int yh_bvh_build(int n, const float* boxes, float* nodes, int* primitives) {
  if (n < 0 || (n && !boxes)) return YH_E_INVALID;
  std::vector<yhh::Box> b((size_t)n);
  for (int i = 0; i < n; i++)
    for (int k = 0; k < 3; k++) b[(size_t)i].min[k] = boxes[6 * (size_t)i + k], b[(size_t)i].max[k] = boxes[6 * (size_t)i + 3 + k];
  yhh::Tree tree;
  yhh::build_bvh(tree, b);
  if (nodes)
    for (size_t i = 0; i < tree.nodes.size(); i++) {
      auto&  nd = tree.nodes[i];
      float* o  = nodes + 8 * i;
      memcpy(o, nd.bbox.min, 12), memcpy(o + 3, nd.bbox.max, 12);
      int a = nd.start, c = (int)nd.num | ((int)nd.internal << 16) | ((int)nd.axis << 24);
      memcpy(o + 6, &a, 4), memcpy(o + 7, &c, 4);
    }
  if (primitives && n) memcpy(primitives, tree.primitives.data(), sizeof(int) * (size_t)n);
  return (int)tree.nodes.size();
}

int yh_surface_lobe_batch(yh_context* ctx, int kind, int n, const float* params, const float* normal,
    const float* outgoing, const float* incoming, const float* rn, float* out) {
  if (!ctx || n < 0 || kind < 0 || kind >= YH_LOBE_COUNT || (n && (!params || !normal || !outgoing || !incoming || !rn || !out)))
    return YH_E_INVALID;
  if (n == 0) return YH_OK;
  HIPCHK(ctx, hipSetDevice(ctx->device));
  Staged s(ctx);
  auto   dp = (float*)s.in(params, 32 * (size_t)n);
  auto   dn = (float*)s.in(normal, 12 * (size_t)n);
  auto   da = (float*)s.in(outgoing, 12 * (size_t)n);
  auto   db = (float*)s.in(incoming, 12 * (size_t)n);
  auto   dr = (float*)s.in(rn, 12 * (size_t)n);
  auto   o  = (float*)s.out(28 * (size_t)n);
  if (s.rc) return s.rc;
  return finish(ctx, yhk_surface_lobe(kind, n, dp, dn, da, db, dr, o, ctx->stream), out, o, 28 * (size_t)n);
}
int yh_surface_bsdf_batch(yh_context* ctx, int n, const yh_material* materials, const float* normal,
    const float* outgoing, const float* incoming, const float* rn, float* out) {
  if (!ctx || n < 0 || (n && (!materials || !normal || !outgoing || !incoming || !rn || !out))) return YH_E_INVALID;
  if (n == 0) return YH_OK;
  HIPCHK(ctx, hipSetDevice(ctx->device));
  std::vector<yhd_material> mats((size_t)n);
  for (int i = 0; i < n; i++) make_material(materials[i], mats[(size_t)i]);
  Staged s(ctx);
  auto   dm = s.in(mats.data(), sizeof(yhd_material) * (size_t)n);
  auto   dn = (float*)s.in(normal, 12 * (size_t)n);
  auto   da = (float*)s.in(outgoing, 12 * (size_t)n);
  auto   db = (float*)s.in(incoming, 12 * (size_t)n);
  auto   dr = (float*)s.in(rn, 12 * (size_t)n);
  auto   o  = (float*)s.out(4 * YH_SURFACE_BSDF_FLOATS * (size_t)n);
  if (s.rc) return s.rc;
  return finish(ctx, yhk_surface_bsdf(n, dm, dn, da, db, dr, o, ctx->stream), out, o, 4 * YH_SURFACE_BSDF_FLOATS * (size_t)n);
}

int yh_intersect_batch(yh_context* ctx, int n, const float* rays, int* object, int* element, float* uv,
    float* distance) {
  if (!ctx || n < 0 || (n && (!rays || !object || !element || !uv || !distance))) return YH_E_INVALID;
  if (!ctx->have_scene) return fail(ctx, YH_E_STATE, "yh_intersect_batch before yh_upload_scene");
  if (n == 0) return YH_OK;
  HIPCHK(ctx, hipSetDevice(ctx->device));
  Staged s(ctx);
  auto   dr = (float*)s.in(rays, 32 * (size_t)n);
  auto   dob = (int*)s.out(4 * (size_t)n);
  auto   del = (int*)s.out(4 * (size_t)n);
  auto   duv = (float*)s.out(8 * (size_t)n);
  auto   dd  = (float*)s.out(4 * (size_t)n);
  if (s.rc) return s.rc;
  const char* mode  = getenv("YHAIR_INTERSECT");
  int         waves = 5;
  bool        lanes = n >= 65536 && lane_kernels_can_address(ctx);
  if (mode && !strcmp(mode, "quad")) lanes = false;
  else if (mode && !strncmp(mode, "lane", 4)) {
    if (!lane_kernels_can_address(ctx))
      return fail(ctx, YH_E_INVALID, "YHAIR_INTERSECT=%s: the one-lane kernel reads the scene's trees through 32-bit byte offsets and this scene's exceed 4 GB", mode);
    lanes = true, waves = std::max(4, std::min(8, atoi(mode + 4)));
  }
  for (int i = 0; lanes && i < n; i++) lanes = rays[8 * (size_t)i + 6] == 1e-4f;
  HIPCHK(ctx, hipEventRecord(ctx->ev0, ctx->stream));
  if (lanes) {
    const int occupancy = std::min(waves, yhk_intersect_lanes_occupancy(&ctx->scene, waves));
    if (occupancy < 1) return fail(ctx, YH_E_DEVICE, "k_intersect_lanes cannot run with its LDS layout on this device");
    const int    grid        = (int)std::max<int64_t>(1, std::min<int64_t>(((int64_t)n + 255) / 256, (int64_t)ctx->num_cus * occupancy));
    const int    ovf_entries = 2 * std::max(8, ctx->stack_need);
    auto         dcur        = (int*)s.out(16);
    auto         dovf        = (unsigned int*)s.out((size_t)grid * 4 * ovf_entries * 64 * 4);
    if (s.rc) return s.rc;
    if (!ctx->d_scene_copy.p) {
      int rc = upload(ctx, ctx->d_scene_copy, &ctx->scene, sizeof(yhd_scene));
      if (rc) return rc;
    }
    int e = yhk_intersect_lanes(&ctx->scene, (const yhd_scene*)ctx->d_scene_copy.p, n, dr, dcur, dovf, ovf_entries, dob, del, duv, dd, waves, grid, ctx->stream);
    if (e) return fail(ctx, YH_E_DEVICE, "k_intersect_lanes launch: %s", hipGetErrorString((hipError_t)e));
  } else {
    int e = yhk_intersect(&ctx->scene, n, dr, dob, del, duv, dd, ctx->stream);
    if (e) return fail(ctx, YH_E_DEVICE, "k_intersect launch: %s", hipGetErrorString((hipError_t)e));
  }
  HIPCHK(ctx, hipEventRecord(ctx->ev1, ctx->stream));
  YH_WAIT(ctx);
  HIPCHK(ctx, hipEventElapsedTime(&ctx->last_ms, ctx->ev0, ctx->ev1));
  ctx->last_launches = 1;
  HIPCHK(ctx, hipMemcpy(object, dob, 4 * (size_t)n, hipMemcpyDeviceToHost));
  HIPCHK(ctx, hipMemcpy(element, del, 4 * (size_t)n, hipMemcpyDeviceToHost));
  HIPCHK(ctx, hipMemcpy(uv, duv, 8 * (size_t)n, hipMemcpyDeviceToHost));
  HIPCHK(ctx, hipMemcpy(distance, dd, 4 * (size_t)n, hipMemcpyDeviceToHost));
  return YH_OK;
}

int yh_lights_batch(yh_context* ctx, int form, int n, const float* position, const float* direction, const float* rn, float* out) {
  if (!ctx || n < 0 || (form != 0 && form != 1) || (n && (!position || !direction || !rn || !out))) return YH_E_INVALID;
  if (!ctx->have_scene) return fail(ctx, YH_E_STATE, "yh_lights_batch before yh_upload_scene");
  if (n == 0) return YH_OK;
  HIPCHK(ctx, hipSetDevice(ctx->device));
  Staged s(ctx);
  auto   dp = (float*)s.in(position, 12 * (size_t)n);
  auto   dd = (float*)s.in(direction, 12 * (size_t)n);
  auto   dr = (float*)s.in(rn, 16 * (size_t)n);
  auto   o  = (float*)s.out(32 * (size_t)n);
  if (s.rc) return s.rc;
  if (form == 0) return finish(ctx, yhk_lights(&ctx->scene, n, dp, dd, dr, o, ctx->stream), out, o, 32 * (size_t)n);
  if (!lane_kernels_can_address(ctx))
    return fail(ctx, YH_E_INVALID, "yh_lights_batch: the one-lane form reads the scene's trees through 32-bit byte offsets and this scene's exceed 4 GB");
  const int ovf_entries = 2 * std::max(8, ctx->stack_need);
  auto      dovf        = (unsigned int*)s.out((size_t)((n + 255) / 256) * 4 * ovf_entries * 64 * 4);
  if (s.rc) return s.rc;
  if (!ctx->d_scene_copy.p) {
    int rc = upload(ctx, ctx->d_scene_copy, &ctx->scene, sizeof(yhd_scene));
    if (rc) return rc;
  }
  return finish(ctx, yhk_lights_lanes(&ctx->scene, (const yhd_scene*)ctx->d_scene_copy.p, n, dp, dd, dr, dovf, ovf_entries, o, ctx->stream), out, o, 32 * (size_t)n);
}

int yh_selftest(yh_context* ctx, int which, float* worst) {
  if (!ctx) return YH_E_INVALID;
  if (which < 0 || which > 3) return fail(ctx, YH_E_INVALID, "unknown self-test %d", which);
  HIPCHK(ctx, hipSetDevice(ctx->device));
  DevBuf sums, wbits;
  int    rc;
  if ((rc = alloc_zero(ctx, sums, 6 * sizeof(double)))) return rc;
  if ((rc = alloc_zero(ctx, wbits, 4))) return rc;
  auto lum = [](const double* s) { return (float)(0.2126 * s[0] + 0.7152 * s[1] + 0.0722 * s[2]); };
  auto sample_sphere = [](float rx, float ry, float* w) {
    float z = 2 * ry - 1;
    float r = std::sqrt(fmin_(fmax_(1 - z * z, 0.0f), 1.0f));
    float phi = 2 * pif * rx;
    w[0] = r * std::cos(phi), w[1] = r * std::sin(phi), w[2] = z;
  };
  Rng   rng = make_rng(199382389514ULL);
  float wo[3] = {0, 0, 1};
  if (which == 0 || which == 1) {
    float x = rand1f(rng), y = rand1f(rng);
    sample_sphere(x, y, wo);
  }
  bool  ok  = true;
  float dev = 0;
  auto run = [&](float bm, float bn, int count, int per_iter, double* out, float* dmax) -> int {
    HIPCHK(ctx, hipMemsetAsync(sums.p, 0, 6 * sizeof(double), ctx->stream));
    HIPCHK(ctx, hipMemsetAsync(wbits.p, 0, 4, ctx->stream));
    int e = yhk_selftest(which, bm, bn, rng.state, rng.inc, count, wo, (double*)sums.p, (unsigned int*)wbits.p, ctx->stream);
    if (e) return fail(ctx, YH_E_DEVICE, "k_selftest launch: %s", hipGetErrorString((hipError_t)e));
    YH_WAIT(ctx);
    HIPCHK(ctx, hipMemcpy(out, sums.p, 6 * sizeof(double), hipMemcpyDeviceToHost));
    unsigned int bits;
    HIPCHK(ctx, hipMemcpy(&bits, wbits.p, 4, hipMemcpyDeviceToHost));
    memcpy(dmax, &bits, 4);
    skip_rng(rng, (uint64_t)count * per_iter);
    return YH_OK;
  };
  double s[6];
  float  d;
  if (which == 0 || which == 1) {
    for (float bm = 0.1f; bm < 1.0f; bm += 0.2f)
      for (float bn = 0.1f; bn < 1.0f; bn += 0.2f) {
        const int count = 300000;
        if ((rc = run(bm, bn, count, 3, s, &d))) return rc;
        float avg = which == 0 ? lum(s) / (count * (1 / (4 * pif))) : lum(s) / count;
        float lo = which == 0 ? 0.95f : 0.99f, hi = which == 0 ? 1.05f : 1.01f;
        if (!(avg >= lo && avg <= hi)) ok = false;
        dev = fmax_(dev, std::fabs(avg - 1));
      }
  } else if (which == 2) {
    for (float bm = 0.1f; bm < 1.0f; bm += 0.2f)
      for (float bn = 0.4f; bn < 1.0f; bn += 0.2f) {
        if ((rc = run(bm, bn, 10000, 5, s, &d))) return rc;
        if (!(d <= 0.001f)) ok = false;
        dev = fmax_(dev, d);
      }
  } else {
    for (float bm = 0.2f; bm < 1.0f; bm += 0.2f)
      for (float bn = 0.4f; bn < 1.0f; bn += 0.2f) {
        const int count = 64 * 1024;
        float x = rand1f(rng), y = rand1f(rng);
        sample_sphere(x, y, wo);
        if ((rc = run(bm, bn, count, 3, s, &d))) return rc;
        float fi = lum(s) / count, fu = lum(s + 3) / (count * (1 / (4 * pif)));
        float err = std::fabs(fi - fu) / fu;
        if (err >= 0.05f) ok = false;
        dev = fmax_(dev, err);
      }
  }
  if (worst) *worst = dev;
  if (!ok) return fail(ctx, YH_E_SELFTEST, "TEST FAILED! (self-test %d, worst deviation %g)", which, dev);
  return YH_OK;
}
```

yocto-hair_amd/host/context_internal.h:

```cpp
#ifndef YH_CONTEXT_INTERNAL_H_
#define YH_CONTEXT_INTERNAL_H_
#include <hip/hip_runtime_api.h>
#include <dlfcn.h>
#include <fcntl.h>
#include <sys/stat.h>
#include <unistd.h>
#include <rccl/rccl.h>

#include <algorithm>
#include <chrono>
#include <cmath>
#include <cstdarg>
#include <cstddef>
#include <cstdio>
#include <cstdlib>
#include <cstring>
#include <limits>
#include <map>
#include <mutex>
#include <tuple>
#include <string>
#include <memory>
#include <thread>
#include <vector>

#include "../csrc/yh_device.h"
#include "bvh_build.h"
#include "deadline.h"
#include "yhair.h"

extern "C" {
int yhk_trace(const yhd_scene*, const yhd_state*, int, yhd_counters*, int shape, int grid_blocks, hipStream_t);
int yhk_trace_exact(const yhd_scene*, const yhd_state*, int nsamples, int lds_bytes, int grid_blocks, hipStream_t);
int yhk_trace_exact_occupancy(int lds_bytes, int general);
int yhk_block_threads(int shape);
int yhk_trace_occupancy(int lds_bytes, int general, int shape);
int yhk_trace_sbs(const yhd_scene*, const yhd_state*, int nsamples, int oct_blocks, int quad_items, int oct_entries, int grid_blocks, hipStream_t);
int yhk_trace_sbs_lds_bytes(const yhd_scene* sc);
int yhk_trace_sbs_occupancy(int lds_bytes, int general);
int yhk_trace_lds_bytes(const yhd_scene* sc, int shape);
int yhk_stack_entries(void);
int yhk_stream(const yhd_scene*, const yhd_scene* sc_dev, const yhd_state*, int, const yhd_stream*, int grid_blocks, hipStream_t);
int yhk_lane_tests(const yhd_float4* prims, yhd_float4* blob, int kind, int prim_base, int num_prims, long long test_off, hipStream_t);
int yhk_stream_block_threads(void);
int yhk_stream_lds_bytes(int tables_f4, int slots_per_wave);
int yhk_stream_occupancy(int lds_bytes, int general);
int yhk_intersect_lanes_occupancy(const yhd_scene* sc, int waves);
int yhk_intersect_lanes(const yhd_scene* sc, const yhd_scene* sc_dev, int n, const float* rays, int* cursor, unsigned int* stack_ovf,
    int ovf_entries, int* object, int* element, float* uv, float* dist, int waves, int grid_blocks, hipStream_t stream);
int yhk_resolve(const yhd_state*, int, int, void*, hipStream_t);
int yhk_pack(const yhd_state*, int, int, void*, hipStream_t);
int yhk_unpack(const void*, int, int, int, int, int, int, int, void*, hipStream_t);
int yhk_hair_brdf(int, const void*, const float*, const float*, const float*, float*, hipStream_t);
int yhk_hair_eval(int, const float*, const float*, const float*, float*, hipStream_t);
int yhk_hair_pdf(int, const float*, const float*, const float*, float*, hipStream_t);
int yhk_hair_sample(int, const float*, const float*, const float*, float*, hipStream_t);
int yhk_intersect(const yhd_scene*, int, const float*, int*, int*, float*, float*, hipStream_t);
int yhk_bvh_build_gpu(int n, const float* boxes, float* nodes8, int* primitives, int* num_nodes, int* depth, hipStream_t);
int yhk_prim_boxes(int lines, int n, const float* pos, const float* radius, const int* idx, float* boxes, hipStream_t);
int yhk_bvh_build_resident(int n, const float* d_boxes, float* d_nodes, int* d_pid, int* num_nodes, int* levels, int* level_first, hipStream_t);
int yhk_leaf_records(int lines, int n, const int* pid, const float* pos, const float* nrm, const float* radius, const int* idx, void* prims_out, hipStream_t);
int yhk_wide_index(int num_nodes, const float* d_nodes, int levels, const int* level_first, int L, unsigned int* d_flag, unsigned int* d_widx, int* count, hipStream_t);
int yhk_wide_collapse(int L, int num_nodes, const float* d_nodes, const unsigned int* d_flag, const unsigned int* d_widx, int lines, long long node_off, long long test_off, void* blob, hipStream_t);
int yhk_curves_to_lines(int, const float*, const float*, const float*, int, float*, float*, float*, int*, hipStream_t);
int yhk_surface_lobe(int, int, const float*, const float*, const float*, const float*, const float*, float*, hipStream_t);
int yhk_surface_bsdf(int, const void*, const float*, const float*, const float*, const float*, float*, hipStream_t);
int yhk_lights(const yhd_scene*, int, const float*, const float*, const float*, float*, hipStream_t);
int yhk_lights_lanes(const yhd_scene* sc, const yhd_scene* sc_dev, int n, const float* position, const float* direction, const float* rn,
    unsigned int* stack_ovf, int ovf_entries, float* out, hipStream_t stream);
int yhk_selftest(int, float, float, uint64_t, uint64_t, int, const float*, double*, unsigned int*, hipStream_t);
}

struct DevBuf {
  void*  p = nullptr;
  size_t bytes = 0;
  DevBuf() = default;
  DevBuf(const DevBuf&) = delete;
  DevBuf& operator=(const DevBuf&) = delete;
  DevBuf(DevBuf&& o) noexcept : p(o.p), bytes(o.bytes) { o.p = nullptr, o.bytes = 0; }
  ~DevBuf() { reset(); }
  void reset() {
    if (p) (void)hipFree(p);
    p = nullptr, bytes = 0;
  }
};

namespace {



const float pif = (float)3.14159265358979323846;

struct F3 {
  float x, y, z;
};
F3    operator+(F3 a, F3 b) { return {a.x + b.x, a.y + b.y, a.z + b.z}; }
F3    operator-(F3 a, F3 b) { return {a.x - b.x, a.y - b.y, a.z - b.z}; }
F3    operator-(F3 a) { return {-a.x, -a.y, -a.z}; }
F3    operator*(F3 a, float b) { return {a.x * b, a.y * b, a.z * b}; }
float dot(F3 a, F3 b) { return a.x * b.x + a.y * b.y + a.z * b.z; }
F3    cross(F3 a, F3 b) { return {a.y * b.z - a.z * b.y, a.z * b.x - a.x * b.z, a.x * b.y - a.y * b.x}; }
float fmin_(float a, float b) { return (a < b) ? a : b; }
float fmax_(float a, float b) { return (a > b) ? a : b; }
F3    ld3(const float* p) { return {p[0], p[1], p[2]}; }
void  st3(float* p, F3 a) { p[0] = a.x, p[1] = a.y, p[2] = a.z; }

void inverse_frame(const float* f, bool non_rigid, float* out) {
  F3 x = ld3(f), y = ld3(f + 3), z = ld3(f + 6), o = ld3(f + 9);
  F3 rx, ry, rz;
  if (non_rigid) {
    F3    c0 = cross(y, z), c1 = cross(z, x), c2 = cross(x, y);
    float det = dot(x, cross(y, z));
    float s   = 1 / det;
    rx = F3{c0.x, c1.x, c2.x} * s, ry = F3{c0.y, c1.y, c2.y} * s, rz = F3{c0.z, c1.z, c2.z} * s;
  } else {
    rx = {x.x, y.x, z.x}, ry = {x.y, y.y, z.y}, rz = {x.z, y.z, z.z};
  }
  F3 ro = -(rx * o.x + ry * o.y + rz * o.z);
  st3(out, rx), st3(out + 3, ry), st3(out + 6, rz), st3(out + 9, ro);
}
F3 transform_point(const float* f, F3 b) {
  return ld3(f) * b.x + ld3(f + 3) * b.y + ld3(f + 6) * b.z + ld3(f + 9);
}

struct Rng {
  uint64_t state, inc;
};
uint32_t advance_rng(Rng& rng) {
  uint64_t old        = rng.state;
  rng.state           = old * 6364136223846793005ULL + rng.inc;
  uint32_t xorshifted = (uint32_t)(((old >> 18u) ^ old) >> 27u);
  uint32_t rot        = (uint32_t)(old >> 59u);
  return (xorshifted >> rot) | (xorshifted << ((-rot) & 31));
}
Rng make_rng(uint64_t seed, uint64_t seq = 1) {
  Rng rng{0, (seq << 1u) | 1u};
  advance_rng(rng);
  rng.state += seed;
  advance_rng(rng);
  return rng;
}
float rand1f(Rng& rng) {
  uint32_t u = (advance_rng(rng) >> 9) | 0x3f800000u;
  float    f;
  memcpy(&f, &u, 4);
  return f - 1.0f;
}
void skip_rng(Rng& rng, uint64_t delta) {
  uint64_t cur_mult = 6364136223846793005ULL, cur_plus = rng.inc, acc_mult = 1u, acc_plus = 0u;
  while (delta > 0) {
    if (delta & 1) acc_mult *= cur_mult, acc_plus = acc_plus * cur_mult + cur_plus;
    cur_plus = (cur_mult + 1) * cur_plus;
    cur_mult *= cur_mult;
    delta /= 2;
  }
  rng.state = acc_mult * rng.state + acc_plus;
}

float sqr(float v) { return v * v; }
template <int N>
float powt(float v) {
  if constexpr (N == 0) return 1;
  else if constexpr (N == 1) return v;
  else {
    float n2 = powt<N / 2>(v);
    return n2 * n2 * powt<(N & 1)>(v);
  }
}

}

template <typename F>
void parallel_for(int n, F&& fn) {
  int nt = (int)std::min<unsigned>(16u, std::max(1u, std::thread::hardware_concurrency()));
  if (n < 65536 || nt == 1) {
    for (int i = 0; i < n; i++) fn(i);
    return;
  }
  std::vector<std::thread> pool;
  for (int t = 0; t < nt; t++)
    pool.emplace_back([=, &fn] {
      int lo = (int)((int64_t)n * t / nt), hi = (int)((int64_t)n * (t + 1) / nt);
      for (int i = lo; i < hi; i++) fn(i);
    });
  for (auto& th : pool) th.join();
}

struct yh_context {
  int         device = 0;
  hipStream_t stream = nullptr;
  hipEvent_t  ev0 = nullptr, ev1 = nullptr;
  int         hy_quad_items = 0, hy_oct_entries = 0;
  std::vector<int> hy_oct_items;
  int         num_cus = 0;
  std::string device_name;
  std::string error = "no error";
  yhh::BoundedCall sync_call;
  bool        poisoned = false;
  bool      have_scene = false;
  yhd_scene scene{};
  DevBuf    d_prims, d_vpos, d_elems, d_objects, d_materials, d_scene_nodes,
      d_scene_prims, d_light_cdf, d_env_texels, d_light_table, d_env_tab;
  int       stack_need = 0, stack_need8 = 0, stack_need16 = 0;
  struct LaneShape { int kind, num_nodes, prim_base, num_prims; long long node_off, test_off, node_off8, node_off16; };
  std::vector<LaneShape>   lane_shapes;
  long long                lane_units = 0;
  DevBuf                   d_lane_blob;
  bool             have_state = false;
  yhd_state        state{};
  yh_trace_params  params{};
  DevBuf           d_textures, d_tex_texels, d_vtex, d_maps;
  DevBuf           d_rng_state, d_rng_inc, d_accum, d_tiles, d_image, d_counters, d_tile_cursor, d_tile_cost;
  std::vector<int> owned;
  std::vector<unsigned int>  item_cost;
  int              rank = 0, world = 1;
  int              num_tiles_total = 0;
  float            last_ms = 0;
  int              last_launches = 0;
  int              last_nsamples = 0;
  unsigned         launches_of_image = 0;
  int              launch_shape = YH_SHAPE_QUAD;
  int              last_shape = -1;
  bool             async_pending = false;
  bool             last_counted = false;
  DevBuf                  d_gather_send, d_gather_recv;
  std::vector<ncclComm_t> comms;
  std::vector<int>        comm_devices;
  double           shape_ms[YH_SHAPES] = {};
  int              shape_trials[YH_SHAPES] = {};
  uint64_t         scene_key = 0;
  bool             trials_from_disk = false;
  bool             trials_on_disk = false;
  bool             have_costs = false;
  bool             costs_settled = false;
  bool             planned_settled = false;
  int              dense = -1;
  int              chain16 = -1;
  int              chain = -1;
  DevBuf           d_st_slots, d_st_medium, d_st_ovf, d_st_prof, d_st_wave_log, d_st_wave_begin, d_st_wave_fill, d_scene_copy;
  int              st_items = 0;
  size_t           st_share_waves = 0;
  int              st_share_slots = 0;
  std::vector<int>    st_share_begin, st_share_items;
  std::vector<double> st_share_cost;
  std::vector<unsigned long long> st_last_log;
  bool                st_log_fresh = false;
  std::vector<float>  st_wave_speed;
  std::vector<float>  item_scale;
  std::vector<double> stream_speed = {1.10, 1.045, 0.97, 0.885};
  size_t           st_slots = 0, st_medium_slots = 0, st_ovf_words = 0;
  yhd_stream       stream_pool{};
};

#pragma GCC visibility push(hidden)
extern std::string g_create_error;
#define HIPCHK(ctx, call)                                                                               \
  do {                                                                                                  \
    hipError_t e_ = (call);                                                                             \
    if (e_ != hipSuccess) return fail(ctx, YH_E_DEVICE, "%s: %s", #call, hipGetErrorString(e_));       \
  } while (0)

#define YH_WAIT(ctx)                                      \
  do {                                                    \
    if (int wrc_ = wait_for_launch(ctx)) return wrc_;     \
  } while (0)

constexpr int YH_TRIAL_SPP = 32;
constexpr double YH_TRIAL_TIE  = 1.15;
constexpr double YH_FINAL_TIE  = 1.05;
constexpr int    YH_TRIALS_MAX = 2;

int fail(yh_context* ctx, int code, const char* fmt, ...);
int upload(yh_context* ctx, DevBuf& buf, const void* src, size_t bytes);
int upload_keep(yh_context* ctx, DevBuf& buf, const void* src, size_t bytes);
int alloc_zero(yh_context* ctx, DevBuf& buf, size_t bytes);
yhd_float4 node_lo(const yhh::Node& n);
yhd_float4 node_hi(const yhh::Node& n);
int forced_shape();
void trials_load(yh_context* ctx);
bool trials_off();
void record_launch(yh_context* ctx, int nsamples, bool fresh_costs);
bool trial_pending(const yh_context* ctx);
int pick_launch_shape(const yh_context* ctx, int nsamples);
bool settle_launch_shape(yh_context* ctx, bool counted, int nsamples, bool sync);
void build_work_items(const yh_context* ctx, std::vector<int>& items);
void prepare_work_list(yh_context* ctx, std::vector<int>& items, int shape);
int upload_work_items(yh_context* ctx);
int expensive_items(const yh_context* ctx, const std::vector<int>& items);
bool side_by_side_grids(const yh_context* ctx, int* oct_blocks, int* quad_blocks);
void split_items_side_by_side(yh_context* ctx, std::vector<int>& items);
void lay_out_range(const yh_context* ctx, int* items, size_t n, int wpb, int G, int block_offset = 0);
int replan_after_launch(yh_context* ctx, int nsamples);
bool lane_kernels_can_address(const yh_context* ctx);
int stream_geometry(const yh_context* ctx, int num_items, int* slots_per_wave, int* grid_blocks, int* lds_out, bool* single_generation = nullptr);
void note_stream_wave_log(yh_context* ctx, const unsigned long long* log, size_t waves);
void deal_items_for_stream(yh_context* ctx, std::vector<int>& items);
int build_bvh_device(yh_context* ctx, const std::vector<yhh::Box>& boxes, yhh::Tree& tree);
int stream_impl(yh_context* ctx, int nsamples, bool sync);
int trace_impl(yh_context* ctx, int nsamples, bool counted, bool sync);
int wait_for_launch(yh_context* ctx);
int side_by_side_impl(yh_context* ctx, int nsamples, bool sync);
void destroy_communicators(yh_context* ctx);
inline int tiles_of(int n) { return (n + YH_TILE - 1) / YH_TILE; }
void make_material(const yh_material& m, yhd_material& d);
#pragma GCC visibility pop
#endif
```

yocto-hair_amd/host/scene_upload.cpp:

```cpp
#include "context_internal.h"

#include <atomic>

static int dev_alloc(yh_context* ctx, DevBuf& buf, size_t bytes) {
  buf.reset();
  HIPCHK(ctx, hipMalloc(&buf.p, std::max<size_t>(bytes, 16)));
  buf.bytes = std::max<size_t>(bytes, 16);
  return YH_OK;
}

void make_material(const yh_material& m, yhd_material& d) {
  memset(&d, 0, sizeof(d));
  memcpy(d.emission, m.emission, 12);
  memcpy(d.color, m.color, 12);
  float dmax    = fmax_(fmax_(m.color[0], m.color[1]), m.color[2]);
  d.diffuse_pdf = dmax ? dmax / dmax : 0.0f;
  d.thin        = m.thin;
  d.specular = m.specular, d.metallic = m.metallic, d.roughness = m.roughness, d.ior = m.ior;
  d.transmission = m.transmission;
  d.opacity      = m.opacity * ((1.0f + 1.0f + 1.0f) / 3);
  if (d.opacity > 0.999f) d.opacity = 1;
  d.emission_tex = m.emission_tex - 1, d.color_tex = m.color_tex - 1, d.scattering_tex = m.scattering_tex - 1;
  d.trdepth = m.trdepth;
  d.plain = m.specular == 0 && m.metallic == 0 && m.transmission == 0 && d.opacity == 1 && m.emission_tex == 0 &&
            m.color_tex == 0 && m.scattering_tex == 0;
  for (int c = 0; c < 3; c++) {
    float r   = fmin_(fmax_(m.color[c], 0.0f), 0.99f);
    d.meta[c] = (1 + std::sqrt(r)) / (1 - std::sqrt(r));
  }
  d.has_volume = !m.thin && m.transmission != 0;
  for (int c = 0; c < 3; c++) {
    d.vol_density[c] = d.has_volume ? -std::log(fmin_(fmax_(m.color[c], 0.0001f), 1.0f)) / m.trdepth : 0.0f;
    d.vol_scatter[c] = m.scattering[c];
  }
  d.vol_anisotropy = m.scanisotropy;
  F3 sa{0, 0, 0};
  if (m.sigma_a[0] || m.sigma_a[1] || m.sigma_a[2]) {
    sa = ld3(m.sigma_a);
  } else if (m.color[0] || m.color[1] || m.color[2]) {
    float bn  = m.beta_n;
    float den = 5.969f - 0.215f * bn + 2.532f * sqr(bn) - 10.73f * powt<3>(bn) + 5.574f * powt<4>(bn) +
                0.245f * powt<5>(bn);
    F3 q = {std::log(m.color[0]) / den, std::log(m.color[1]) / den, std::log(m.color[2]) / den};
    sa   = {q.x * q.x, q.y * q.y, q.z * q.z};
  } else if (m.eumelanin || m.pheomelanin) {
    F3 e = F3{0.419f, 0.697f, 1.37f}, p = F3{0.187f, 0.4f, 1.05f};
    sa   = F3{m.eumelanin * e.x, m.eumelanin * e.y, m.eumelanin * e.z} +
         F3{m.pheomelanin * p.x, m.pheomelanin * p.y, m.pheomelanin * p.z};
  }
  st3(d.sigma_a, sa);
  d.alpha = m.alpha, d.eta = m.eta;
  float bm = m.beta_m, bn = m.beta_n;
  d.v[0] = sqr(0.726f * bm + 0.812f * sqr(bm) + 3.7f * powt<20>(bm));
  d.v[1] = 0.25f * d.v[0];
  d.v[2] = 4 * d.v[0];
  d.v[3] = d.v[2];
  d.s    = 0.626657069f * (0.265f * bn + 1.194f * sqr(bn) + 5.372f * powt<22>(bn));
  d.sin_2k_alpha[0] = std::sin(pif / 180 * d.alpha);
  d.cos_2k_alpha[0] = std::sqrt(fmax_(0.0f, 1 - sqr(d.sin_2k_alpha[0])));
  for (int i = 1; i < 3; i++) {
    d.sin_2k_alpha[i] = 2 * d.cos_2k_alpha[i - 1] * d.sin_2k_alpha[i - 1];
    d.cos_2k_alpha[i] = sqr(d.cos_2k_alpha[i - 1]) - sqr(d.sin_2k_alpha[i - 1]);
  }
  for (int p = 0; p < 4; p++) {
    d.inv_v[p]        = 1 / d.v[p];
    d.log_inv_2v[p]   = std::log(1 / (2 * d.v[p]));
    d.exp_m2_inv_v[p] = std::exp(-2 / d.v[p]);
    d.mp_den[p]       = ::sinh((double)(1 / d.v[p])) * 2 * d.v[p];
  }
  float cb   = 1 / (1 + std::exp(-pif / d.s));
  float ca   = 1 / (1 + std::exp(-(-pif) / d.s));
  d.tl_cdf_a = ca;
  d.tl_norm  = cb - ca;
}


static bool has_effective_map(const yh_material_maps& m) {
  return m.specular_tex || m.metallic_tex || m.roughness_tex || m.opacity_tex || m.normal_tex;
}

static_assert(sizeof(yhd_maps) == 32, "yhd_maps");

static bool tree_levels(const yhh::Tree& tree, int& levels, int* level_first) {
  std::vector<int> level(tree.nodes.size(), 0);
  for (size_t n = 0; n < tree.nodes.size(); n++)
    if (tree.nodes[n].internal) level[(size_t)tree.nodes[n].start] = level[(size_t)tree.nodes[n].start + 1] = level[n] + 1;
  const int num_nodes = (int)tree.nodes.size();
  levels = level.empty() ? 1 : level.back() + 1;
  if (levels > 128) return false;
  for (int l = 0; l <= levels; l++) level_first[l] = num_nodes;
  for (size_t n = tree.nodes.size(); n-- > 0;) level_first[level[n]] = (int)n;
  return true;
}

int yh_upload_scene(yh_context* ctx, const yh_scene_desc* sd) { return yh_upload_scene_maps(ctx, sd, nullptr); }

int yh_upload_scene_maps(yh_context* ctx, const yh_scene_desc* sd, const yh_material_maps* maps) {
  if (!ctx) return YH_E_INVALID;
  if (!sd) return fail(ctx, YH_E_INVALID, "scene is NULL");
  HIPCHK(ctx, hipSetDevice(ctx->device));
  if (ctx->poisoned) return fail(ctx, YH_E_DEVICE, "a launch of this context exceeded its deadline: the context refuses further work, destroy it");
  YH_WAIT(ctx);
  if (sd->num_objects <= 0) return fail(ctx, YH_E_INVALID, "scene has no objects");
  if (sd->num_environments > YH_MAX_ENVS) return fail(ctx, YH_E_INVALID, "more than %d environments", YH_MAX_ENVS);
  bool any_maps = false;
  if (maps)
    for (int i = 0; i < sd->num_materials; i++) {
      const yh_material_maps& m = maps[i];
      for (int id : {m.specular_tex, m.metallic_tex, m.roughness_tex, m.transmission_tex, m.opacity_tex, m.normal_tex})
        if (id < 0 || id > sd->num_textures) return fail(ctx, YH_E_INVALID, "material %d: a map references a missing texture (%d of %d)", i, id, sd->num_textures);
      any_maps = any_maps || has_effective_map(m);
    }
  const bool timing = getenv("YHAIR_TIMING") && atoi(getenv("YHAIR_TIMING")) != 0;
  auto       t_last = std::chrono::steady_clock::now();
  auto       lap    = [&](const char* what) {
    if (!timing) return;
    auto now = std::chrono::steady_clock::now();
    fprintf(stderr, "[yhair] upload: %-28s %8.1f ms\n", what, std::chrono::duration<double, std::milli>(now - t_last).count());
    t_last = now;
  };
  struct ShapeInfo {
    int kind, prim_base, vert_base, elem_base, has_normals, depth;
    int depth8, depth16;
    yhh::Box root;
    int num_prims;
    int num_nodes = 0, levels = 1;
    int level_first[130] = {0};
    int wide_count[3] = {0, 0, 0};
    std::vector<yhd_float4> host_prims;
  };
  std::vector<ShapeInfo>  info(sd->num_shapes);
  std::vector<DevBuf>     d_tree(sd->num_shapes);
  std::vector<yhd_float4> vpos;
  std::vector<float>      vtex;
  std::vector<yhd_int4>   elems;
  size_t total_prim_f4 = 0;
  for (int si = 0; si < sd->num_shapes; si++) {
    auto& s = sd->shapes[si];
    if (s.num_vertices <= 0 || !s.positions) return fail(ctx, YH_E_INVALID, "shape %d has no vertices", si);
    const bool lines = s.num_lines > 0;
    if (!lines && s.num_triangles <= 0) return fail(ctx, YH_E_INVALID, "shape %d has no lines or triangles", si);
    const int nel = lines ? s.num_lines : s.num_triangles;
    if (nel >= (1 << 27)) return fail(ctx, YH_E_INVALID, "shape %d has %d elements (limit %d)", si, nel, (1 << 27) - 1);
    info[si].kind = lines ? YH_KIND_LINES : YH_KIND_TRIANGLES, info[si].num_prims = nel, info[si].has_normals = s.normals != nullptr;
    info[si].prim_base = (int)total_prim_f4;
    total_prim_f4 += (size_t)nel * (lines ? 4 : 6);
  }
  if (total_prim_f4 > (size_t)std::numeric_limits<int>::max()) return fail(ctx, YH_E_INVALID, "scene too large for 32-bit record offsets (%zu primitive float4)", total_prim_f4);
  int rc;
  ctx->have_scene = false, ctx->have_state = false;
  ctx->scene.lane_blob = nullptr, ctx->scene.prims = nullptr;
  ctx->d_prims.reset(), ctx->d_lane_blob.reset();
  if ((rc = dev_alloc(ctx, ctx->d_prims, total_prim_f4 * 16))) return rc;
  lap("validation, record array");
  const char* bvh_env   = getenv("YHAIR_BVH");
  const bool  host_only = bvh_env && !strcmp(bvh_env, "host"), device_all = bvh_env && !strcmp(bvh_env, "device");
  for (int si = 0; si < sd->num_shapes; si++) {
    auto&      s     = sd->shapes[si];
    auto&      I     = info[si];
    const bool lines = I.kind == YH_KIND_LINES;
    const int  nel   = I.num_prims;
    const int* idx   = lines ? s.lines : s.triangles;
    {
      std::atomic<bool> bad{false};
      parallel_for(nel * (lines ? 2 : 3), [&](int k) {
        if (idx[k] < 0 || idx[k] >= s.num_vertices) bad = true;
      });
      if (bad) return fail(ctx, YH_E_INVALID, "shape %d: vertex index out of range", si);
    }
    I.vert_base = (int)vpos.size(), I.elem_base = (int)elems.size();
    yhd_float4* d_recs = (yhd_float4*)ctx->d_prims.p + I.prim_base;
    if ((nel >= 32768 || device_all) && !host_only) {
      const size_t nv = (size_t)s.num_vertices;
      DevBuf d_pos, d_nrm, d_rad, d_idx, d_boxes, d_pid;
      auto h2d = [&](DevBuf& buf, const void* src, size_t bytes) -> int {
        if (int arc = dev_alloc(ctx, buf, bytes)) return arc;
        HIPCHK(ctx, hipMemcpyAsync(buf.p, src, bytes, hipMemcpyHostToDevice, ctx->stream));
        return YH_OK;
      };
      if ((rc = h2d(d_pos, s.positions, nv * 12))) return rc;
      if (s.radius && (rc = h2d(d_rad, s.radius, nv * 4))) return rc;
      if ((rc = h2d(d_idx, idx, (size_t)nel * (lines ? 8 : 12)))) return rc;
      if ((rc = dev_alloc(ctx, d_boxes, (size_t)nel * 24))) return rc;
      if ((rc = dev_alloc(ctx, d_pid, (size_t)nel * 4))) return rc;
      if ((rc = dev_alloc(ctx, d_tree[si], ((size_t)2 * nel + 1) * 32))) return rc;
      int e = yhk_prim_boxes(lines ? 1 : 0, nel, (const float*)d_pos.p, (const float*)d_rad.p, (const int*)d_idx.p, (float*)d_boxes.p, ctx->stream);
      if (e) return fail(ctx, YH_E_DEVICE, "primitive bounds: %s", hipGetErrorString((hipError_t)e));
      if (s.normals && (rc = h2d(d_nrm, s.normals, nv * 12))) return rc;
      e = yhk_bvh_build_resident(nel, (const float*)d_boxes.p, (float*)d_tree[si].p, (int*)d_pid.p, &I.num_nodes, &I.levels, I.level_first, ctx->stream);
      if (e) return fail(ctx, YH_E_DEVICE, "device BVH build: %s", hipGetErrorString((hipError_t)e));
      lap("device: bounds + reference tree");
      e = yhk_leaf_records(lines ? 1 : 0, nel, (const int*)d_pid.p, (const float*)d_pos.p, (const float*)d_nrm.p, (const float*)d_rad.p, (const int*)d_idx.p, d_recs, ctx->stream);
      if (e) return fail(ctx, YH_E_DEVICE, "leaf records: %s", hipGetErrorString((hipError_t)e));
      float root8[8];
      HIPCHK(ctx, hipMemcpyAsync(root8, d_tree[si].p, 32, hipMemcpyDeviceToHost, ctx->stream));
      YH_WAIT(ctx);
      memcpy(I.root.min, root8, 12), memcpy(I.root.max, root8 + 3, 12);
      lap("device: leaf records");
    } else {
      auto pos = [&](int v) { return ld3(s.positions + 3 * (size_t)v); };
      auto rad = [&](int v) { return s.radius ? s.radius[v] : 0.001f; };
      std::vector<yhh::Box> boxes(nel);
      parallel_for(nel, [&](int e) {
        if (lines) {
          int a = idx[2 * e], b = idx[2 * e + 1];
          F3  p0 = pos(a), p1 = pos(b);
          float r0 = rad(a), r1 = rad(b);
          float lo0[3] = {p0.x - r0, p0.y - r0, p0.z - r0}, lo1[3] = {p1.x - r1, p1.y - r1, p1.z - r1};
          float hi0[3] = {p0.x + r0, p0.y + r0, p0.z + r0}, hi1[3] = {p1.x + r1, p1.y + r1, p1.z + r1};
          for (int k = 0; k < 3; k++) boxes[e].min[k] = fmin_(lo0[k], lo1[k]), boxes[e].max[k] = fmax_(hi0[k], hi1[k]);
        } else {
          const float* p0 = s.positions + 3 * (size_t)idx[3 * e];
          const float* p1 = s.positions + 3 * (size_t)idx[3 * e + 1];
          const float* p2 = s.positions + 3 * (size_t)idx[3 * e + 2];
          for (int k = 0; k < 3; k++) {
            boxes[e].min[k] = fmin_(p0[k], fmin_(p1[k], p2[k]));
            boxes[e].max[k] = fmax_(p0[k], fmax_(p1[k], p2[k]));
          }
        }
      });
      yhh::Tree tree;
      yhh::build_bvh(tree, boxes);
      static_assert(sizeof(yhh::Node) == 32 && offsetof(yhh::Node, start) == 24 && offsetof(yhh::Node, num) == 28 && offsetof(yhh::Node, internal) == 30 && offsetof(yhh::Node, axis) == 31,
          "yhh::Node is the device's node record");
      I.num_nodes = (int)tree.nodes.size();
      if (!tree_levels(tree, I.levels, I.level_first)) return fail(ctx, YH_E_INVALID, "shape %d: tree of %d levels", si, I.levels);
      if ((rc = upload(ctx, d_tree[si], tree.nodes.data(), tree.nodes.size() * 32))) return rc;
      I.root = tree.nodes[0].bbox;
      auto nrm = [&](int v) { return s.normals ? ld3(s.normals + 3 * (size_t)v) : F3{0, 0, 0}; };
      const size_t per = lines ? 4 : 6;
      I.host_prims.resize(per * (size_t)nel);
      yhd_float4* out = I.host_prims.data();
      parallel_for(nel, [&](int slot) {
        int   e = tree.primitives[slot];
        float ew;
        memcpy(&ew, &e, 4);
        yhd_float4* r = out + per * (size_t)slot;
        if (lines) {
          int a = idx[2 * e], b = idx[2 * e + 1];
          F3  p0 = pos(a), p1 = pos(b), t0 = nrm(a), t1 = nrm(b);
          r[0] = {p0.x, p0.y, p0.z, rad(a)}, r[1] = {p1.x, p1.y, p1.z, rad(b)};
          r[2] = {t0.x, t0.y, t0.z, ew}, r[3] = {t1.x, t1.y, t1.z, 0};
        } else {
          int a = idx[3 * e], b = idx[3 * e + 1], cc = idx[3 * e + 2];
          F3  p0 = pos(a), p1 = pos(b), p2 = pos(cc), n0 = nrm(a), n1 = nrm(b), n2 = nrm(cc);
          r[0] = {p0.x, p0.y, p0.z, ew}, r[1] = {p1.x, p1.y, p1.z, 0}, r[2] = {p2.x, p2.y, p2.z, 0};
          r[3] = {n0.x, n0.y, n0.z, 0}, r[4] = {n1.x, n1.y, n1.z, 0}, r[5] = {n2.x, n2.y, n2.z, 0};
        }
      });
      HIPCHK(ctx, hipMemcpy(d_recs, I.host_prims.data(), I.host_prims.size() * 16, hipMemcpyHostToDevice));
      lap("host: small shape");
    }
    {
      const int deepest = std::max(0, I.levels - 2);
      I.depth = 1 + deepest / 2, I.depth8 = 1 + deepest / 3, I.depth16 = 1 + deepest / 4;
    }
    {
      const bool per_vertex = !lines || s.texcoords != nullptr;
      if (!per_vertex) {
        I.vert_base = 0, I.elem_base = 0;
      } else {
        auto pos = [&](int v) { return ld3(s.positions + 3 * (size_t)v); };
        const size_t at = vpos.size();
        vpos.resize(at + (size_t)s.num_vertices);
        vtex.resize(2 * (at + (size_t)s.num_vertices), 0.0f);
        if (s.texcoords) memcpy(&vtex[2 * at], s.texcoords, sizeof(float) * 2 * (size_t)s.num_vertices);
        parallel_for(s.num_vertices, [&](int v) {
          F3 p = pos(v);
          vpos[at + (size_t)v] = {p.x, p.y, p.z, lines ? (s.radius ? s.radius[v] : 0.001f) : 0.0f};
        });
        const size_t ea = elems.size();
        elems.resize(ea + (size_t)nel);
        parallel_for(nel, [&](int e) {
          elems[ea + (size_t)e] = lines ? yhd_int4{idx[2 * e], idx[2 * e + 1], 0, 0}
                                        : yhd_int4{idx[3 * e], idx[3 * e + 1], idx[3 * e + 2], 0};
        });
      }
    }
  }
  std::vector<yhh::Box> obj_boxes(sd->num_objects);
  for (int oi = 0; oi < sd->num_objects; oi++) {
    auto& o = sd->objects[oi];
    if (o.shape < 0 || o.shape >= sd->num_shapes || o.material < 0 || o.material >= sd->num_materials)
      return fail(ctx, YH_E_INVALID, "object %d references a missing shape or material", oi);
    const yhh::Box& b = info[o.shape].root;
    float lo[3] = {std::numeric_limits<float>::max(), std::numeric_limits<float>::max(), std::numeric_limits<float>::max()};
    float hi[3] = {std::numeric_limits<float>::lowest(), std::numeric_limits<float>::lowest(),
        std::numeric_limits<float>::lowest()};
    for (int c = 0; c < 8; c++) {
      F3 corner = {(c & 4) ? b.max[0] : b.min[0], (c & 2) ? b.max[1] : b.min[1], (c & 1) ? b.max[2] : b.min[2]};
      F3 t      = transform_point(o.frame, corner);
      float tv[3] = {t.x, t.y, t.z};
      for (int k = 0; k < 3; k++) lo[k] = fmin_(lo[k], tv[k]), hi[k] = fmax_(hi[k], tv[k]);
    }
    for (int k = 0; k < 3; k++) obj_boxes[oi].min[k] = lo[k], obj_boxes[oi].max[k] = hi[k];
  }
  yhh::Tree scene_tree;
  yhh::build_bvh(scene_tree, obj_boxes);
  static_assert(sizeof(yhd_object) == 16 * YH_OBJECT_F4, "yhd_object is staged to LDS as float4");
  const int  lds_scene_f4 = YH_OBJECT_F4 * sd->num_objects + 2 * (int)scene_tree.nodes.size() + (sd->num_objects + 3) / 4;
  const bool scene_wide   = lds_scene_f4 * 16 > 10240;
  DevBuf d_stree, d_sflag, d_sidx;
  int    scene_wide_count = 0, scene_wide_depth = 0;
  if (scene_wide) {
    int levels = 1, level_first[130] = {0};
    const int nn = (int)scene_tree.nodes.size();
    if (!tree_levels(scene_tree, levels, level_first)) return fail(ctx, YH_E_INVALID, "scene tree of %d levels", levels);
    if ((rc = upload(ctx, d_stree, scene_tree.nodes.data(), scene_tree.nodes.size() * 32))) return rc;
    if ((rc = dev_alloc(ctx, d_sflag, ((size_t)nn + 1) * 4))) return rc;
    if ((rc = dev_alloc(ctx, d_sidx, ((size_t)nn + 1) * 4))) return rc;
    int e = yhk_wide_index(nn, (const float*)d_stree.p, levels, level_first, 2, (unsigned int*)d_sflag.p, (unsigned int*)d_sidx.p, &scene_wide_count, ctx->stream);
    if (e) return fail(ctx, YH_E_DEVICE, "wide-node index of the scene tree: %s", hipGetErrorString((hipError_t)e));
    scene_wide_depth = 1 + std::max(0, levels - 2) / 2;
  }
  std::vector<DevBuf> d_wflag((size_t)sd->num_shapes * 3), d_widx((size_t)sd->num_shapes * 3);
  for (int si = 0; si < sd->num_shapes; si++)
    for (int w = 0; w < 3; w++) {
      auto&  I = info[si];
      DevBuf &f = d_wflag[(size_t)si * 3 + w], &x = d_widx[(size_t)si * 3 + w];
      if ((rc = dev_alloc(ctx, f, ((size_t)I.num_nodes + 1) * 4))) return rc;
      if ((rc = dev_alloc(ctx, x, ((size_t)I.num_nodes + 1) * 4))) return rc;
      int e = yhk_wide_index(I.num_nodes, (const float*)d_tree[si].p, I.levels, I.level_first, 2 + w, (unsigned int*)f.p, (unsigned int*)x.p, &I.wide_count[w], ctx->stream);
      if (e) return fail(ctx, YH_E_DEVICE, "wide-node index: %s", hipGetErrorString((hipError_t)e));
    }
  ctx->lane_shapes.assign((size_t)sd->num_shapes, yh_context::LaneShape{});
  long long U8 = 0, U16 = 0, blob_units = 0;
  {
    long long at = 4ll * scene_wide_count;
    for (int si = 0; si < sd->num_shapes; si++) {
      auto& L = ctx->lane_shapes[(size_t)si];
      L.kind = info[si].kind, L.num_nodes = info[si].wide_count[0], L.prim_base = info[si].prim_base, L.num_prims = info[si].num_prims;
      L.test_off = at, at += (long long)L.num_prims * (L.kind == YH_KIND_LINES ? 1 : 2);
    }
    at = (at + 3) / 4 * 4 + 4;
    if (at >= (1ll << 27)) return fail(ctx, YH_E_INVALID, "scene too large for 27-bit leaf offsets (%lld test-record units)", at);
    for (int si = 0; si < sd->num_shapes; si++) ctx->lane_shapes[(size_t)si].node_off = at, at += 4ll * info[si].wide_count[0];
    ctx->lane_units = at + 4;
    U8 = (ctx->lane_units + 3) / 4 * 4, at = U8;
    for (int si = 0; si < sd->num_shapes; si++) ctx->lane_shapes[(size_t)si].node_off8 = at, at += 8ll * info[si].wide_count[1];
    U16 = at;
    for (int si = 0; si < sd->num_shapes; si++) ctx->lane_shapes[(size_t)si].node_off16 = at, at += 16ll * info[si].wide_count[2];
    blob_units = at + 4;
    if (blob_units >= (1ll << 30)) return fail(ctx, YH_E_INVALID, "scene too large for 30-bit node offsets (%lld units)", blob_units);
    (void)U16;
  }
  if ((rc = alloc_zero(ctx, ctx->d_lane_blob, (size_t)blob_units * 32))) return rc;
  for (int si = 0; si < sd->num_shapes; si++) {
    auto& L = ctx->lane_shapes[(size_t)si];
    auto& I = info[si];
    int e = yhk_lane_tests((const yhd_float4*)ctx->d_prims.p, (yhd_float4*)ctx->d_lane_blob.p, L.kind, L.prim_base, L.num_prims, L.test_off, ctx->stream);
    const long long offs[3] = {L.node_off, L.node_off8, L.node_off16};
    for (int w = 0; w < 3 && !e; w++)
      e = yhk_wide_collapse(2 + w, I.num_nodes, (const float*)d_tree[si].p, (const unsigned int*)d_wflag[(size_t)si * 3 + w].p, (const unsigned int*)d_widx[(size_t)si * 3 + w].p,
          L.kind == YH_KIND_LINES ? 1 : 0, offs[w], L.test_off, ctx->d_lane_blob.p, ctx->stream);
    if (e) return fail(ctx, YH_E_DEVICE, "wide collapse: %s", hipGetErrorString((hipError_t)e));
  }
  if (scene_wide) {
    int e = yhk_wide_collapse(2, (int)scene_tree.nodes.size(), (const float*)d_stree.p, (const unsigned int*)d_sflag.p, (const unsigned int*)d_sidx.p, 1, 0, 0, ctx->d_lane_blob.p, ctx->stream);
    if (e) return fail(ctx, YH_E_DEVICE, "wide collapse of the scene tree: %s", hipGetErrorString((hipError_t)e));
  }
  YH_WAIT(ctx);
  d_tree.clear(), d_wflag.clear(), d_widx.clear(), d_stree.reset(), d_sflag.reset(), d_sidx.reset();
  lap("device: wide collapses, blob");
  std::vector<yhd_object> objects(sd->num_objects);
  for (int oi = 0; oi < sd->num_objects; oi++) {
    auto& o = sd->objects[oi];
    auto& I = info[o.shape];
    auto& d = objects[oi];
    memcpy(d.frame, o.frame, 48);
    inverse_frame(o.frame, true, d.inv_frame);
    d.kind = I.kind, d.node_base = 0, d.prim_base = I.prim_base, d.vert_base = I.vert_base;
    d.elem_base = I.elem_base, d.has_normals = I.has_normals, d.material = o.material, d.has_texcoords = sd->shapes[o.shape].texcoords != nullptr;
    const auto& LS = ctx->lane_shapes[(size_t)o.shape];
    d.lane_root = (int)LS.node_off, d.lane_test = (int)LS.test_off, d.lane_root8 = (int)LS.node_off8, d.lane_root16 = (int)LS.node_off16;
    {
      const float *lo = obj_boxes[oi].min, *hi = obj_boxes[oi].max;
      float ext = fmax_(fmax_(hi[0] - lo[0], hi[1] - lo[1]), hi[2] - lo[2]);
      float eps = 1e-3f * ext + 1e-5f;
      for (int k = 0; k < 3; k++) d.wbox_min[k] = lo[k] - eps, d.wbox_max[k] = hi[k] + eps;
      d.wbox_min[3] = d.wbox_max[3] = 0;
    }
  }
  if (vpos.size() > (size_t)std::numeric_limits<int>::max()) return fail(ctx, YH_E_INVALID, "scene too large for 32-bit vertex offsets (%zu)", vpos.size());
  std::vector<yhd_float4> scene_nodes;
  for (auto& n : scene_tree.nodes) scene_nodes.push_back(node_lo(n)), scene_nodes.push_back(node_hi(n));
  int max_shape_depth = 0;
  for (auto& I : info) max_shape_depth = std::max(max_shape_depth, I.depth);
  const int scene_need = scene_wide ? 3 * scene_wide_depth + 4 : scene_tree.max_depth + 4;
  ctx->stack_need = scene_need + 3 * max_shape_depth + 2;
  int max_shape_depth8 = 0;
  for (auto& I : info) max_shape_depth8 = std::max(max_shape_depth8, I.depth8);
  ctx->stack_need8 = scene_need + 7 * max_shape_depth8 + 2;
  int max_shape_depth16 = 0;
  for (auto& I : info) max_shape_depth16 = std::max(max_shape_depth16, I.depth16);
  ctx->stack_need16 = scene_need + 15 * max_shape_depth16 + 2;
  if (ctx->stack_need > yhk_stack_entries())
    return fail(ctx, YH_E_INVALID, "BVH too deep for the traversal stack (%d > %d)", ctx->stack_need, yhk_stack_entries());
  std::vector<yhd_material> materials(sd->num_materials);
  int general_materials = 0;
  std::vector<yhd_maps> mat_maps(any_maps ? (size_t)sd->num_materials : 0);
  for (int i = 0; i < sd->num_materials; i++) {
    make_material(sd->materials[i], materials[i]);
    if (any_maps) {
      const yh_material_maps& m = maps[i];
      yhd_maps&               d = mat_maps[(size_t)i];
      d.specular_tex = m.specular_tex - 1, d.metallic_tex = m.metallic_tex - 1, d.roughness_tex = m.roughness_tex - 1;
      d.opacity_tex = m.opacity_tex - 1, d.normal_tex = m.normal_tex - 1;
      d.any = has_effective_map(m) ? 1 : 0, d.opacity = sd->materials[i].opacity, d.pad = 0;
      if (d.any) materials[i].plain = 0;
    }
    if (!materials[i].plain) general_materials = 1;
  }
  yhd_scene sc{};
  std::vector<float>      light_cdf;
  std::vector<yhd_float4> env_texels;
  std::vector<int>        small_lights;
  for (int oi = 0; oi < sd->num_objects; oi++) {
    auto& o = sd->objects[oi];
    auto& m = sd->materials[o.material];
    if (m.emission[0] == 0 && m.emission[1] == 0 && m.emission[2] == 0) continue;
    auto& s = sd->shapes[o.shape];
    if (s.num_lines > 0 || s.num_triangles <= 0) continue;
    if (sc.num_lights >= YH_MAX_LIGHTS) return fail(ctx, YH_E_INVALID, "more than %d lights: object %d of %d is emissive too (each instance of an emitter counts)", YH_MAX_LIGHTS, oi, sd->num_objects);
    auto& L = sc.lights[sc.num_lights++];
    L.object = oi, L.environment = -1, L.cdf_base = (int)light_cdf.size(), L.cdf_count = s.num_triangles, L.small_base = -1;
    if (s.num_triangles <= YH_SMALL_LIGHT_TRIS) small_lights.push_back(sc.num_lights - 1);
    else general_materials = 1;
    for (int t = 0; t < s.num_triangles; t++) {
      F3 p0 = ld3(s.positions + 3 * (size_t)s.triangles[3 * t]), p1 = ld3(s.positions + 3 * (size_t)s.triangles[3 * t + 1]),
         p2 = ld3(s.positions + 3 * (size_t)s.triangles[3 * t + 2]);
      F3    c    = cross(p1 - p0, p2 - p0);
      float area = std::sqrt(dot(c, c)) / 2;
      if (t) area += light_cdf.back();
      light_cdf.push_back(area);
    }
  }
  sc.num_environments = sd->num_environments;
  for (int ei = 0; ei < sd->num_environments; ei++) {
    auto& e = sd->environments[ei];
    auto& d = sc.environments[ei];
    memcpy(d.frame, e.frame, 48);
    inverse_frame(e.frame, false, d.inv_frame);
    memcpy(d.emission, e.emission, 12);
    d.tex_w = e.texels ? e.tex_width : 0, d.tex_h = e.texels ? e.tex_height : 0;
    d.texel_base = (int)env_texels.size();
    if (e.texels)
      for (size_t t = 0; t < (size_t)e.tex_width * e.tex_height; t++)
        env_texels.push_back({e.texels[3 * t], e.texels[3 * t + 1], e.texels[3 * t + 2], 0});
    if (e.emission[0] == 0 && e.emission[1] == 0 && e.emission[2] == 0) continue;
    if (sc.num_lights >= YH_MAX_LIGHTS) return fail(ctx, YH_E_INVALID, "more than %d lights", YH_MAX_LIGHTS);
    auto& L = sc.lights[sc.num_lights++];
    L.object = -1, L.environment = ei, L.cdf_base = (int)light_cdf.size(), L.cdf_count = 0, L.small_base = -1;
    if (e.texels) {
      size_t n    = (size_t)e.tex_width * e.tex_height;
      L.cdf_count = (int)n;
      for (size_t i = 0; i < n; i++) {
        int   iy    = (int)(i / e.tex_width);
        float th    = (iy + 0.5f) * pif / e.tex_height;
        float mx    = fmax_(fmax_(e.texels[3 * i], e.texels[3 * i + 1]), e.texels[3 * i + 2]);
        float value = mx * std::sin(th);
        if (i) value += light_cdf.back();
        light_cdf.push_back(value);
      }
    }
  }
  if (sc.num_lights == 0) return fail(ctx, YH_E_INVALID, "scene has no lights (the path sampler needs at least one)");
  std::vector<yhd_float4> light_table;
  for (int li : small_lights) {
    auto& L  = sc.lights[li];
    auto& I  = info[sd->objects[L.object].shape];
    if (I.host_prims.empty()) {
      I.host_prims.resize((size_t)6 * L.cdf_count);
      HIPCHK(ctx, hipMemcpy(I.host_prims.data(), (const yhd_float4*)ctx->d_prims.p + I.prim_base, I.host_prims.size() * 16, hipMemcpyDeviceToHost));
    }
    const yhd_float4* rec = I.host_prims.data();
    L.small_base = (int)light_table.size();
    yhd_float4 b0{I.root.min[0], I.root.min[1], I.root.min[2], 0}, b1{I.root.max[0], I.root.max[1], I.root.max[2], light_cdf[(size_t)L.cdf_base + L.cdf_count - 1]};
    memcpy(&b0.w, &L.cdf_count, 4);
    light_table.push_back(b0), light_table.push_back(b1);
    for (int t = 0; t < YH_SMALL_LIGHT_TRIS; t++)
      for (int k = 0; k < 3; k++) light_table.push_back(t < L.cdf_count ? rec[6 * t + k] : yhd_float4{0, 0, 0, 0});
    yhd_float4 cdf{0, 0, 0, 0};
    for (int t = 0; t < L.cdf_count; t++) (&cdf.x)[t] = light_cdf[(size_t)L.cdf_base + t];
    light_table.push_back(cdf);
  }
  std::vector<float> env_tab;
  sc.env_tab_light = -1, sc.env_tab_k = 0, sc.env_tab_stride = 0;
  for (int li = 0; li < sc.num_lights && sc.env_tab_light < 0; li++) {
    auto& L = sc.lights[li];
    if (L.environment < 0 || L.cdf_count < 4096) continue;
    const int n = L.cdf_count, S = (n + 2047) / 2048, K = (n + S - 1) / S;
    env_tab.resize((size_t)K);
    for (int k = 0; k < K; k++) env_tab[(size_t)k] = light_cdf[(size_t)L.cdf_base + (size_t)std::min<int64_t>(n, (int64_t)(k + 1) * S) - 1];
    sc.env_tab_light = li, sc.env_tab_k = K, sc.env_tab_stride = S;
  }
  std::vector<yhd_texture> textures((size_t)std::max(0, sd->num_textures));
  std::vector<yhd_float4>  tex_texels;
  {
    std::vector<char> need_linear(textures.size(), 0);
    for (int i = 0; i < sd->num_materials; i++) {
      auto& m = sd->materials[i];
      for (int id : {m.emission_tex, m.color_tex, m.scattering_tex})
        if (id < 0 || id > sd->num_textures) return fail(ctx, YH_E_INVALID, "material %d references a missing texture", i);
      if (m.emission_tex > 0) need_linear[(size_t)m.emission_tex - 1] = 1;
      if (any_maps)
        for (int id : {maps[i].specular_tex, maps[i].metallic_tex, maps[i].roughness_tex, maps[i].opacity_tex, maps[i].normal_tex})
          if (id > 0) need_linear[(size_t)id - 1] = 1;
    }
    auto srgb_to_rgb = [](float srgb) {
      return (srgb <= 0.04045) ? srgb / 12.92f : std::pow((srgb + 0.055f) / (1.0f + 0.055f), 2.4f);
    };
    std::vector<char> used(textures.size(), !any_maps);
    if (any_maps)
      for (int i = 0; i < sd->num_materials; i++) {
        auto& m = sd->materials[i];
        for (int id : {m.emission_tex, m.color_tex, m.scattering_tex})
          if (id > 0) used[(size_t)id - 1] = 1;
      }
    for (size_t t = 0; t < textures.size(); t++) used[t] = used[t] || need_linear[t];
    for (size_t t = 0; t < textures.size(); t++) {
      auto& src = sd->textures[t];
      if (src.width <= 0 || src.height <= 0 || !src.pixels) return fail(ctx, YH_E_INVALID, "texture %d is empty", (int)t);
      size_t n = (size_t)src.width * src.height;
      auto&  d = textures[t];
      d.width = src.width, d.height = src.height, d.srgb_base = (int)tex_texels.size(), d.linear_base = -1;
      if (!used[t]) {
        d.srgb_base = -1;
        continue;
      }
      tex_texels.resize(tex_texels.size() + n);
      yhd_float4* out = tex_texels.data() + d.srgb_base;
      if (src.is_byte) {
        auto b = (const unsigned char*)src.pixels;
        parallel_for((int)n, [&](int i) {
          out[i] = {srgb_to_rgb(b[3 * (size_t)i] / 255.0f), srgb_to_rgb(b[3 * (size_t)i + 1] / 255.0f),
              srgb_to_rgb(b[3 * (size_t)i + 2] / 255.0f), 0};
        });
        if (need_linear[t]) {
          d.linear_base = (int)tex_texels.size();
          tex_texels.resize(tex_texels.size() + n);
          yhd_float4* lin = tex_texels.data() + d.linear_base;
          parallel_for((int)n, [&](int i) { lin[i] = {b[3 * (size_t)i] / 255.0f, b[3 * (size_t)i + 1] / 255.0f, b[3 * (size_t)i + 2] / 255.0f, 0}; });
        }
      } else {
        auto f = (const float*)src.pixels;
        parallel_for((int)n, [&](int i) { out[i] = {f[3 * (size_t)i], f[3 * (size_t)i + 1], f[3 * (size_t)i + 2], 0}; });
        d.linear_base = d.srgb_base;
      }
    }
  }
  lap("objects, materials, lights");
  if ((rc = upload(ctx, ctx->d_vpos, vpos.data(), vpos.size() * 16))) return rc;
  if ((rc = upload(ctx, ctx->d_elems, elems.data(), elems.size() * 16))) return rc;
  if ((rc = upload(ctx, ctx->d_objects, objects.data(), objects.size() * sizeof(yhd_object)))) return rc;
  if ((rc = upload(ctx, ctx->d_materials, materials.data(), materials.size() * sizeof(yhd_material)))) return rc;
  if ((rc = upload(ctx, ctx->d_scene_nodes, scene_nodes.data(), scene_nodes.size() * 16))) return rc;
  std::vector<int> scene_prims_padded = scene_tree.primitives;
  scene_prims_padded.resize((scene_prims_padded.size() + 3) / 4 * 4, 0);
  if ((rc = upload(ctx, ctx->d_scene_prims, scene_prims_padded.data(), scene_prims_padded.size() * 4))) return rc;
  if ((rc = upload(ctx, ctx->d_light_cdf, light_cdf.data(), light_cdf.size() * 4))) return rc;
  if ((rc = upload(ctx, ctx->d_light_table, light_table.data(), light_table.size() * 16))) return rc;
  if ((rc = upload(ctx, ctx->d_env_tab, env_tab.data(), env_tab.size() * 4))) return rc;
  if ((rc = upload(ctx, ctx->d_env_texels, env_texels.data(), env_texels.size() * 16))) return rc;
  if ((rc = upload(ctx, ctx->d_textures, textures.data(), textures.size() * sizeof(yhd_texture)))) return rc;
  if ((rc = upload(ctx, ctx->d_tex_texels, tex_texels.data(), tex_texels.size() * 16))) return rc;
  if ((rc = upload(ctx, ctx->d_vtex, vtex.data(), vtex.size() * 4))) return rc;
  if (any_maps) {
    if ((rc = upload(ctx, ctx->d_maps, mat_maps.data(), mat_maps.size() * sizeof(yhd_maps)))) return rc;
  } else {
    ctx->d_maps.reset();
  }
  lap("hipMalloc + H2D copies");
  sc.prims = (const yhd_float4*)ctx->d_prims.p;
  sc.vpos = (const yhd_float4*)ctx->d_vpos.p;
  sc.elems = (const yhd_int4*)ctx->d_elems.p;
  sc.objects = (const yhd_object*)ctx->d_objects.p, sc.materials = (const yhd_material*)ctx->d_materials.p;
  sc.scene_nodes = (const yhd_float4*)ctx->d_scene_nodes.p, sc.scene_prims = (const int*)ctx->d_scene_prims.p;
  sc.num_scene_nodes = (int)scene_tree.nodes.size(), sc.num_objects = sd->num_objects;
  sc.light_cdf = (const float*)ctx->d_light_cdf.p, sc.env_texels = (const yhd_float4*)ctx->d_env_texels.p;
  sc.light_table = (const yhd_float4*)ctx->d_light_table.p, sc.light_table_f4 = (int)light_table.size();
  sc.env_tab = (const float*)ctx->d_env_tab.p;
  sc.stack_entries = std::max(8, (ctx->stack_need + 7) / 8 * 8);
  sc.stack_entries8 = std::max(8, (ctx->stack_need8 + 7) / 8 * 8);
  sc.stack_entries16 = std::max(8, (ctx->stack_need16 + 7) / 8 * 8);
  sc.lane_blob = (const yhd_float4*)ctx->d_lane_blob.p, sc.lane_blob_units = blob_units;
  sc.textures = (const yhd_texture*)ctx->d_textures.p, sc.tex_texels = (const yhd_float4*)ctx->d_tex_texels.p;
  sc.vtex = (const float*)ctx->d_vtex.p;
  sc.maps = any_maps ? (const yhd_maps*)ctx->d_maps.p : nullptr;
  memcpy(sc.camera.frame, sd->camera.frame, 48);
  sc.camera.lens = sd->camera.lens, sc.camera.film_x = sd->camera.film[0], sc.camera.film_y = sd->camera.film[1];
  sc.camera.focus = sd->camera.focus, sc.camera.aperture = sd->camera.aperture;
  sc.num_nodes_total = 0, sc.num_prim_f4 = (int)total_prim_f4;
  for (auto& I : info) sc.num_nodes_total += I.wide_count[0];
  sc.general_materials = general_materials;
  sc.lds_scene_f4    = scene_wide ? 0 : lds_scene_f4;
  sc.scene_wide_root = scene_wide ? 0 : -1;
  {
    static_assert(sizeof(yhd_material) == 16 * YH_MATERIAL_F4, "yhd_material is staged to LDS as float4");
    sc.lds_materials = sd->num_materials <= 24 ? sd->num_materials : 0;
    if (sc.lds_materials == 0 || sc.lds_scene_f4 == 0) sc.general_materials = 1;
  }
  ctx->scene      = sc;
  {
    uint64_t h = 1469598103934665603ULL;
    auto mix = [&](const void* p, size_t n) {
      const unsigned char* b = (const unsigned char*)p;
      for (size_t i = 0; i < n; i++) h = (h ^ b[i]) * 1099511628211ULL;
    };
    mix(&sd->camera, sizeof(sd->camera));
    mix(sd->materials, sizeof(yh_material) * (size_t)sd->num_materials);
    mix(sd->objects, sizeof(yh_object) * (size_t)sd->num_objects);
    for (int i = 0; i < sd->num_shapes; i++) {
      const yh_shape& sh = sd->shapes[i];
      int counts[3] = {sh.num_vertices, sh.num_lines, sh.num_triangles};
      mix(counts, sizeof(counts));
      if (sh.positions && sh.num_vertices > 0) {
        const size_t n = (size_t)sh.num_vertices, take = std::min<size_t>(n, 256);
        mix(sh.positions, take * 12), mix(sh.positions + 3 * (n - take), take * 12);
      }
    }
    for (int i = 0; i < sd->num_environments; i++) mix(&sd->environments[i], offsetof(yh_environment, texels));
    if (any_maps) mix(maps, sizeof(yh_material_maps) * (size_t)sd->num_materials);
    ctx->scene_key = h;
  }
  ctx->d_scene_copy.reset();
  ctx->have_scene = true;
  ctx->have_state = false;
  ctx->launch_shape = YH_SHAPE_QUAD;
  ctx->item_cost.clear();
  ctx->have_costs = false, ctx->costs_settled = false, ctx->dense = -1, ctx->chain = -1, ctx->chain16 = -1;
  for (double& t : ctx->shape_ms) t = 0;
  for (int& t : ctx->shape_trials) t = 0;
  ctx->trials_from_disk = false;
  lap("scene table, fingerprint");
  return YH_OK;
}

int build_bvh_device(yh_context* ctx, const std::vector<yhh::Box>& boxes, yhh::Tree& tree) {
  int                n = (int)boxes.size(), num_nodes = 0, depth = 0;
  std::vector<float> nodes8((size_t)(2 * n + 1) * 8);
  tree.primitives.resize((size_t)n);
  static_assert(sizeof(yhh::Box) == 24, "boxes are passed as 6 floats");
  int e = yhk_bvh_build_gpu(n, (const float*)boxes.data(), nodes8.data(), tree.primitives.data(), &num_nodes, &depth, ctx->stream);
  if (e) return fail(ctx, YH_E_DEVICE, "device BVH build: %s", hipGetErrorString((hipError_t)e));
  tree.nodes.resize((size_t)num_nodes);
  tree.max_depth = depth;
  for (int i = 0; i < num_nodes; i++) {
    const float* o  = &nodes8[(size_t)i * 8];
    yhh::Node&   nd = tree.nodes[(size_t)i];
    memcpy(nd.bbox.min, o, 12), memcpy(nd.bbox.max, o + 3, 12);
    int start, meta;
    memcpy(&start, o + 6, 4), memcpy(&meta, o + 7, 4);
    nd.start = start, nd.num = (short)(meta & 0xFFFF), nd.internal = (meta >> 16) & 1, nd.axis = (unsigned char)((meta >> 24) & 3);
  }
  return YH_OK;
}
```

yocto-hair_amd/python/yhair_capi.py:

```python
import ctypes as C
import os

import numpy as np

ROOT = os.path.dirname(os.path.dirname(os.path.dirname(os.path.abspath(__file__))))
LIB_PATH = os.environ.get("YHAIR_LIB", os.path.join(ROOT, "yocto-hair_amd", "libyhair.so"))

YH_OK, YH_E_INVALID, YH_E_DEVICE, YH_E_STATE, YH_E_IO, YH_E_SELFTEST = 0, -1, -2, -3, -4, -5
YH_HAIR_BRDF_FLOATS = 30
SURFACE_BSDF_FLOATS = 29
(LOBE_DIFFUSE, LOBE_SPECULAR, LOBE_METAL, LOBE_TRANSMISSION, LOBE_REFRACTION, LOBE_DELTA_SPECULAR,
 LOBE_DELTA_METAL, LOBE_DELTA_TRANSMISSION, LOBE_DELTA_REFRACTION) = range(9)
LOBE_COUNT = 9

c_float_p = C.POINTER(C.c_float)
c_int_p = C.POINTER(C.c_int)


class Shape(C.Structure):
    _fields_ = [("num_vertices", C.c_int), ("positions", c_float_p), ("normals", c_float_p),
                ("radius", c_float_p), ("num_lines", C.c_int), ("lines", c_int_p),
                ("num_triangles", C.c_int), ("triangles", c_int_p), ("texcoords", c_float_p)]


class Texture(C.Structure):
    _fields_ = [("width", C.c_int), ("height", C.c_int), ("is_byte", C.c_int), ("pixels", C.c_void_p)]


class Material(C.Structure):
    _fields_ = [("emission", C.c_float * 3), ("color", C.c_float * 3), ("specular", C.c_float),
                ("metallic", C.c_float), ("roughness", C.c_float), ("transmission", C.c_float),
                ("opacity", C.c_float), ("ior", C.c_float), ("thin", C.c_int),
                ("sigma_a", C.c_float * 3), ("beta_m", C.c_float), ("beta_n", C.c_float),
                ("alpha", C.c_float), ("eta", C.c_float), ("eumelanin", C.c_float),
                ("pheomelanin", C.c_float), ("scattering", C.c_float * 3), ("scanisotropy", C.c_float),
                ("trdepth", C.c_float), ("emission_tex", C.c_int), ("color_tex", C.c_int),
                ("scattering_tex", C.c_int)]


class MaterialMaps(C.Structure):
    _fields_ = [("specular_tex", C.c_int), ("metallic_tex", C.c_int), ("roughness_tex", C.c_int),
                ("transmission_tex", C.c_int), ("opacity_tex", C.c_int), ("normal_tex", C.c_int)]


class Object(C.Structure):
    _fields_ = [("frame", C.c_float * 12), ("shape", C.c_int), ("material", C.c_int)]


class Environment(C.Structure):
    _fields_ = [("frame", C.c_float * 12), ("emission", C.c_float * 3), ("tex_width", C.c_int),
                ("tex_height", C.c_int), ("texels", c_float_p)]


class Camera(C.Structure):
    _fields_ = [("frame", C.c_float * 12), ("lens", C.c_float), ("film", C.c_float * 2),
                ("focus", C.c_float), ("aperture", C.c_float)]


class SceneDesc(C.Structure):
    _fields_ = [("num_shapes", C.c_int), ("shapes", C.POINTER(Shape)),
                ("num_materials", C.c_int), ("materials", C.POINTER(Material)),
                ("num_objects", C.c_int), ("objects", C.POINTER(Object)),
                ("num_environments", C.c_int), ("environments", C.POINTER(Environment)),
                ("camera", Camera), ("num_textures", C.c_int), ("textures", C.POINTER(Texture))]


SHADER_NAMES = ["naive", "path", "eyelight", "normal"]


class TraceParams(C.Structure):
    _fields_ = [("resolution", C.c_int), ("bounces", C.c_int), ("clamp", C.c_float),
                ("seed", C.c_uint64), ("shader", C.c_int), ("hair_exact", C.c_int)]

    @staticmethod
    def default(resolution=720, bounces=8, clamp=100.0, seed=961748941, shader="path", hair_exact=False):
        return TraceParams(resolution, bounces, clamp, seed, SHADER_NAMES.index(shader) if isinstance(shader, str) else shader,
                           1 if hair_exact else 0)


class WorkCounts(C.Structure):
    _fields_ = [(n, C.c_uint64) for n in ("samples", "rays", "nodes", "seg_tests", "tri_tests",
                                          "hair_shades", "surf_shades", "env_lookups",
                                          "env_samples", "cyc_trace", "cyc_shade", "ticks_tile",
                                          "wave_iters", "wave_steps", "lane_steps", "lane_iters", "cyc_geom", "cyc_sample",
                                          "cyc_eval", "cyc_rest")] + [("branch", C.c_uint64 * 10)]

    def as_dict(self):
        d = {n: int(getattr(self, n)) for n, _ in self._fields_ if n != "branch"}
        names = ("node", "line", "tri", "enter", "scene")
        for k, nm in enumerate(names):
            d["trips_" + nm], d["lanes_" + nm] = int(self.branch[2 * k]), int(self.branch[2 * k + 1])
        return d

    def bytes_per_sample(self, spp_per_launch, env_textured=True):
        s = max(1, self.samples)
        return (32 * self.nodes + 44 * self.seg_tests + 52 * self.tri_tests +
                104 * self.hair_shades + (48 * self.env_lookups if env_textured else 0) + 88 * self.env_samples) / s \
            + 32.0 / spp_per_launch


def fptr(a):
    return a.ctypes.data_as(c_float_p)


def iptr(a):
    return a.ctypes.data_as(c_int_p)


def hair_material_rows(mats12):
    mats12 = np.ascontiguousarray(mats12, dtype=np.float32).reshape(-1, 12)
    arr = (Material * len(mats12))()
    for i, r in enumerate(mats12):
        m = arr[i]
        m.sigma_a[:] = r[0:3].tolist()
        m.beta_m, m.beta_n, m.alpha, m.eta = map(float, r[3:7])
        m.color[:] = r[7:10].tolist()
        m.eumelanin, m.pheomelanin = float(r[10]), float(r[11])
        m.opacity, m.ior, m.thin, m.trdepth = 1.0, 1.5, 1, 0.01
    return arr


_SIGS = {
    "yh_create": (C.c_void_p, [C.c_int]),
    "yh_destroy": (None, [C.c_void_p]),
    "yh_last_error": (C.c_char_p, [C.c_void_p]),
    "yh_version": (C.c_char_p, []),
    "yh_upload_scene": (C.c_int, [C.c_void_p, C.POINTER(SceneDesc)]),
    "yh_upload_scene_maps": (C.c_int, [C.c_void_p, C.POINTER(SceneDesc), C.POINTER(MaterialMaps)]),
    "yh_init_state": (C.c_int, [C.c_void_p, C.POINTER(TraceParams)]),
    "yh_image_size": (C.c_int, [C.c_void_p, c_int_p, c_int_p]),
    "yh_set_shard": (C.c_int, [C.c_void_p, C.c_int, C.c_int]),
    "yh_trace_samples": (C.c_int, [C.c_void_p, C.c_int]),
    "yh_trace_samples_async": (C.c_int, [C.c_void_p, C.c_int]),
    "yh_synchronize": (C.c_int, [C.c_void_p]),
    "yh_download": (C.c_int, [C.c_void_p, c_float_p]),
    "yh_pack_tiles_device": (C.c_int, [C.c_void_p, C.c_void_p, C.c_int64, C.POINTER(C.c_int64)]),
    "yh_unpack_tiles_device": (C.c_int, [C.c_void_p, C.c_void_p, C.c_int, C.c_int, C.c_void_p]),
    "yh_gather_framebuffer": (C.c_int, [C.POINTER(C.c_void_p), C.c_int, c_float_p]),
    "yh_shard_pixels": (C.c_int64, [C.c_void_p, C.c_int, C.c_int]),
    "yh_download_rng": (C.c_int, [C.c_void_p, C.POINTER(C.c_uint64)]),
    "yh_trace_samples_counted": (C.c_int, [C.c_void_p, C.c_int, C.POINTER(WorkCounts)]),
    "yh_last_trace_ms": (C.c_int, [C.c_void_p, c_float_p, c_int_p]),
    "yh_launch_shape": (C.c_int, [C.c_void_p]),
    "yh_tile_costs": (C.c_int, [C.c_void_p, C.POINTER(C.c_uint32), C.c_int]),
    "yh_item_costs": (C.c_int, [C.c_void_p, C.POINTER(C.c_uint32), C.c_int]),
    "yh_kernel_trials": (C.c_int, [C.c_void_p, C.POINTER(C.c_double), C.POINTER(C.c_int), C.c_int]),
    "yh_trials_pending": (C.c_int, [C.c_void_p]),
    "yh_set_trial_cache_dir": (C.c_int, [C.c_char_p]),
    "yh_default_trial_cache_dir": (C.c_char_p, []),
    "yh_hair_brdf_batch": (C.c_int, [C.c_void_p, C.c_int, C.POINTER(Material), c_float_p,
                                     c_float_p, c_float_p, c_float_p]),
    "yh_curves_to_lines": (C.c_int, [C.c_void_p, C.c_int, c_float_p, c_float_p, c_float_p, C.c_int, c_float_p,
                                     c_float_p, c_float_p, c_int_p]),
    "yh_bvh_build_gpu": (C.c_int, [C.c_void_p, C.c_int, c_float_p, c_float_p, c_int_p]),
    "yh_bvh_build": (C.c_int, [C.c_int, c_float_p, c_float_p, c_int_p]),
    "yh_bvh_build_wide": (C.c_int, [C.c_int, c_float_p, C.c_int, c_float_p]),
    "yh_bvh_build_wide_gpu": (C.c_int, [C.c_void_p, C.c_int, c_float_p, C.c_int, c_float_p]),
    "yh_surface_lobe_batch": (C.c_int, [C.c_void_p, C.c_int, C.c_int, c_float_p, c_float_p, c_float_p, c_float_p,
                                        c_float_p, c_float_p]),
    "yh_surface_bsdf_batch": (C.c_int, [C.c_void_p, C.c_int, C.POINTER(Material), c_float_p, c_float_p, c_float_p,
                                        c_float_p, c_float_p]),
    "yh_hair_eval_batch": (C.c_int, [C.c_void_p, C.c_int, c_float_p, c_float_p, c_float_p, c_float_p]),
    "yh_hair_sample_batch": (C.c_int, [C.c_void_p, C.c_int, c_float_p, c_float_p, c_float_p, c_float_p]),
    "yh_hair_pdf_batch": (C.c_int, [C.c_void_p, C.c_int, c_float_p, c_float_p, c_float_p, c_float_p]),
    "yh_hair_eval_pdf_batch": (C.c_int, [C.c_void_p, C.c_int, c_float_p, c_float_p, c_float_p, c_float_p]),
    "yh_intersect_batch": (C.c_int, [C.c_void_p, C.c_int, c_float_p, c_int_p, c_int_p, c_float_p, c_float_p]),
    "yh_lights_batch": (C.c_int, [C.c_void_p, C.c_int, C.c_int, c_float_p, c_float_p, c_float_p, c_float_p]),
    "yh_selftest": (C.c_int, [C.c_void_p, C.c_int, c_float_p]),
    "yh_scene_load": (C.c_void_p, [C.c_char_p, C.c_char_p, C.c_char_p, C.c_int]),
    "yh_scene_get": (C.POINTER(SceneDesc), [C.c_void_p]),
    "yh_scene_get_maps": (C.POINTER(MaterialMaps), [C.c_void_p]),
    "yh_scene_free": (None, [C.c_void_p]),
    "yh_save_image": (C.c_int, [C.c_char_p, C.c_int, C.c_int, c_float_p, C.c_char_p, C.c_int]),
}
EXPORTS = tuple(_SIGS)

_lib = None


def load(path=None):
    global _lib
    if _lib is None or path:
        p = path or LIB_PATH
        if not os.path.exists(p):
            raise RuntimeError(f"{p} is missing: run `python -c 'import __graft_entry__ as g; g.build()'` "
                               "(there is no CPU fallback for the product path)")
        lib = C.CDLL(p)
        for name, (res, args) in _SIGS.items():
            try:
                fn = getattr(lib, name)
            except AttributeError:
                if "YHAIR_LIB" in os.environ:
                    continue
                raise
            fn.restype, fn.argtypes = res, args
        if path:
            return lib
        _lib = lib
    return _lib


class YhError(RuntimeError):
    pass


def set_trial_cache_dir(path=None, default=False):
    lib = load()
    if not hasattr(lib, "yh_set_trial_cache_dir"):
        return None
    d = lib.yh_default_trial_cache_dir() if default else (path.encode() if path else None)
    lib.yh_set_trial_cache_dir(d)
    return d.decode() if d else None


class SceneFile:

    def __init__(self, json_path, camera=""):
        lib = load()
        err = C.create_string_buffer(512)
        self.handle = lib.yh_scene_load(str(json_path).encode(), camera.encode(), err, 512)
        if not self.handle:
            raise YhError(err.value.decode())
        self.desc = lib.yh_scene_get(self.handle)
        self.maps = lib.yh_scene_get_maps(self.handle)

    def close(self):
        if self.handle and load is not None:
            load().yh_scene_free(self.handle)
            self.handle = None

    def __del__(self):
        try:
            self.close()
        except Exception:
            pass


def gather_framebuffer(contexts):
    lib = load()
    w, h = C.c_int(), C.c_int()
    contexts[0]._chk(lib.yh_image_size(contexts[0].h, C.byref(w), C.byref(h)))
    img = np.zeros((h.value, w.value, 4), np.float32)
    arr = (C.c_void_p * len(contexts))(*[c.h for c in contexts])
    contexts[0]._chk(lib.yh_gather_framebuffer(arr, len(contexts), fptr(img)))
    return img


class Context:

    def __init__(self, device=0):
        self.lib = load()
        self.h = self.lib.yh_create(device)
        if not self.h:
            raise YhError("yh_create failed: " + self.lib.yh_last_error(None).decode())

    def _chk(self, rc):
        if rc != YH_OK:
            raise YhError(f"yhair error {rc}: " + self.lib.yh_last_error(self.h).decode())

    def close(self):
        if self.h:
            self.lib.yh_destroy(self.h)
            self.h = None

    def __del__(self):
        try:
            self.close()
        except Exception:
            pass

    def upload_scene(self, desc, maps=None):
        if maps is None:
            self._chk(self.lib.yh_upload_scene(self.h, desc))
        else:
            self._chk(self.lib.yh_upload_scene_maps(self.h, desc, C.cast(maps, C.POINTER(MaterialMaps))))

    def set_shard(self, rank, world):
        self._chk(self.lib.yh_set_shard(self.h, rank, world))

    def init_state(self, params):
        self._chk(self.lib.yh_init_state(self.h, C.byref(params)))
        w, h = C.c_int(), C.c_int()
        self._chk(self.lib.yh_image_size(self.h, C.byref(w), C.byref(h)))
        self.width, self.height = w.value, h.value
        return self.width, self.height

    def trace_samples(self, n):
        self._chk(self.lib.yh_trace_samples(self.h, n))

    def trace_samples_async(self, n):
        self._chk(self.lib.yh_trace_samples_async(self.h, n))

    def synchronize(self):
        self._chk(self.lib.yh_synchronize(self.h))

    def trace_samples_counted(self, n):
        wc = WorkCounts()
        self._chk(self.lib.yh_trace_samples_counted(self.h, n, C.byref(wc)))
        return wc

    def launch_shape(self):
        return int(self.lib.yh_launch_shape(self.h))

    def last_trace_ms(self):
        ms, n = C.c_float(), C.c_int()
        self._chk(self.lib.yh_last_trace_ms(self.h, C.byref(ms), C.byref(n)))
        return ms.value, n.value

    def tile_costs(self):
        tx, ty = (self.width + 7) // 8, (self.height + 7) // 8
        out = np.zeros(tx * ty, np.uint32)
        self._chk(self.lib.yh_tile_costs(self.h, out.ctypes.data_as(C.POINTER(C.c_uint32)), len(out)))
        return out.reshape(ty, tx)

    def kernel_trials(self):
        ms, tr = (C.c_double * 16)(), (C.c_int * 16)()
        n = self.lib.yh_kernel_trials(self.h, ms, tr, 16)
        self._chk(min(n, 0))
        return {k: (round(ms[k], 5), tr[k]) for k in range(min(n, 16)) if tr[k] or ms[k]}

    def trials_pending(self):
        n = self.lib.yh_trials_pending(self.h)
        self._chk(min(n, 0))
        return n > 0

    def item_costs(self):
        w, h = C.c_int(), C.c_int()
        self._chk(self.lib.yh_image_size(self.h, C.byref(w), C.byref(h)))
        n = ((w.value + 7) // 8) * ((h.value + 7) // 8) * 4
        out = np.zeros(n, np.uint32)
        self._chk(self.lib.yh_item_costs(self.h, out.ctypes.data_as(C.POINTER(C.c_uint32)), n))
        return out

    def download(self):
        img = np.zeros((self.height, self.width, 4), np.float32)
        self._chk(self.lib.yh_download(self.h, fptr(img)))
        return img

    def download_rng(self):
        rng = np.zeros((self.height * self.width, 2), np.uint64)
        self._chk(self.lib.yh_download_rng(self.h, rng.ctypes.data_as(C.POINTER(C.c_uint64))))
        return rng

    def shard_pixels(self, rank, world):
        return int(self.lib.yh_shard_pixels(self.h, rank, world))

    def pack_tiles_device(self, dev_ptr, capacity):
        n = C.c_int64()
        self._chk(self.lib.yh_pack_tiles_device(self.h, C.c_void_p(dev_ptr), capacity, C.byref(n)))
        return n.value

    def unpack_tiles_device(self, packed_ptr, src_rank, world, image_ptr):
        self._chk(self.lib.yh_unpack_tiles_device(self.h, C.c_void_p(packed_ptr), src_rank, world,
                                                  C.c_void_p(image_ptr)))

    def hair_brdf(self, mats12, v, normal, tangent):
        mats = hair_material_rows(mats12)
        n = len(mats)
        v = np.ascontiguousarray(v, np.float32)
        normal = np.ascontiguousarray(normal, np.float32)
        tangent = np.ascontiguousarray(tangent, np.float32)
        out = np.zeros((n, 30), np.float32)
        self._chk(self.lib.yh_hair_brdf_batch(self.h, n, mats, fptr(v), fptr(normal), fptr(tangent), fptr(out)))
        return out

    def _wowi(self, fn, brdf, a, b, width):
        brdf = np.ascontiguousarray(brdf, np.float32)
        a = np.ascontiguousarray(a, np.float32)
        b = np.ascontiguousarray(b, np.float32)
        n = len(brdf)
        out = np.zeros((n, width) if width > 1 else (n,), np.float32)
        self._chk(fn(self.h, n, fptr(brdf), fptr(a), fptr(b), fptr(out)))
        return out

    def hair_eval(self, brdf, wo, wi):
        return self._wowi(self.lib.yh_hair_eval_batch, brdf, wo, wi, 3)

    def hair_sample(self, brdf, wo, rn):
        return self._wowi(self.lib.yh_hair_sample_batch, brdf, wo, rn, 3)

    def hair_pdf(self, brdf, wo, wi):
        return self._wowi(self.lib.yh_hair_pdf_batch, brdf, wo, wi, 1)

    def curves_to_lines(self, P, width0, width1, base_vertex=0):
        P = np.ascontiguousarray(P, np.float32).reshape(-1, 12)
        w0, w1 = np.ascontiguousarray(width0, np.float32), np.ascontiguousarray(width1, np.float32)
        n = len(P)
        pos, nrm = np.zeros((5 * n, 3), np.float32), np.zeros((5 * n, 3), np.float32)
        rad, lines = np.zeros(5 * n, np.float32), np.zeros((4 * n, 2), np.int32)
        self._chk(self.lib.yh_curves_to_lines(self.h, n, fptr(P), fptr(w0), fptr(w1), base_vertex, fptr(pos), fptr(nrm),
                                              fptr(rad), iptr(lines)))
        return pos, nrm, rad, lines

    def surface_lobe(self, kind, params8, normal, wo, wi, rn3):
        a = [np.ascontiguousarray(x, np.float32) for x in (params8, normal, wo, wi, rn3)]
        out = np.zeros((len(a[0]), 7), np.float32)
        self._chk(self.lib.yh_surface_lobe_batch(self.h, kind, len(a[0]), *(fptr(x) for x in a), fptr(out)))
        return out

    def surface_bsdf(self, materials, normal, wo, wi, rn3):
        a = [np.ascontiguousarray(x, np.float32) for x in (normal, wo, wi, rn3)]
        out = np.zeros((len(a[0]), SURFACE_BSDF_FLOATS), np.float32)
        self._chk(self.lib.yh_surface_bsdf_batch(self.h, len(a[0]), materials, *(fptr(x) for x in a), fptr(out)))
        return out

    def intersect(self, rays):
        rays = np.ascontiguousarray(rays, np.float32).reshape(-1, 8)
        n = len(rays)
        obj, elem = np.zeros(n, np.int32), np.zeros(n, np.int32)
        uv, dist = np.zeros((n, 2), np.float32), np.zeros(n, np.float32)
        self._chk(self.lib.yh_intersect_batch(self.h, n, fptr(rays), iptr(obj), iptr(elem), fptr(uv), fptr(dist)))
        return obj, elem, uv, dist

    def lights(self, form, position, direction, rn4):
        a = [np.ascontiguousarray(x, np.float32) for x in (position, direction, rn4)]
        n = len(a[0])
        out = np.zeros((n, 8), np.float32)
        self._chk(self.lib.yh_lights_batch(self.h, form, n, *(fptr(x) for x in a), fptr(out)))
        return out

    def selftest(self, which):
        worst = C.c_float()
        rc = self.lib.yh_selftest(self.h, which, C.byref(worst))
        if rc not in (YH_OK, YH_E_SELFTEST):
            self._chk(rc)
        return rc == YH_OK, worst.value
```

Before: 2565.

## Precompute per-object ray transforms once per ray in LDS for small scenes

For scenes with a single top-level node and at most four non-general objects, the trace loop now tests the scene node and every object box in a prologue. For each object it stores the ray transformed into object space, the reciprocal direction, the sign mask, the box entry/exit distances and the root node in a per-group LDS record. Later object entries during traversal read these records and skip recomputing the instance transform, culling entries whose stored interval is beyond the current tmax. This costs extra LDS per group and is enabled only when the added LDS does not lower occupancy. A plain-intersection test API and kernel are also added.

```diff
diff --git a/include/yhair.h b/include/yhair.h
--- a/include/yhair.h
+++ b/include/yhair.h
@@ -213,6 +213,9 @@
     const float* rn, float* out);
 int yh_intersect_batch(yh_context* ctx, int n, const float* rays, int* object,
     int* element, float* uv, float* distance);
+int yh_intersect_plain_batch(yh_context* ctx, int form, int n, const float* rays,
+    int* object, int* element, float* uv, float* distance);
+int yh_scene_once(const yh_context* ctx);
 
 int yh_lights_batch(yh_context* ctx, int form, int n, const float* position,
     const float* direction, const float* rn, float* out);
diff --git a/yocto-hair_amd/csrc/dev_items.h b/yocto-hair_amd/csrc/dev_items.h
--- a/yocto-hair_amd/csrc/dev_items.h
+++ b/yocto-hair_amd/csrc/dev_items.h
@@ -8,7 +8,7 @@
 #define YH_MIN_WAVES 4
 
 #define YH_QUADS (YH_BLOCK / 4)
-template <bool COUNT, bool GENERAL, int BLOCK, int SHADER, int MODE = YH_MODE_QUAD>
+template <bool COUNT, bool GENERAL, int BLOCK, int SHADER, int MODE = YH_MODE_QUAD, bool ONCE = false>
 YH_DEV void trace_items(const yhd_scene& sc, const yhd_state& st, int nsamples, yhd_counters* counters, unsigned int block = blockIdx.x,
     unsigned int blocks = gridDim.x) {
   constexpr int LPP    = YH_IS_HEX(MODE) ? 16 : YH_IS_OCT(MODE) ? 8 : 4;
@@ -24,6 +24,7 @@
   __syncthreads();
 
   tc.lds_stack = lds_stack + (threadIdx.x / LPP);
+  tc.lds_once  = ONCE ? lds_tabs + YHD_LDS_TABLES_F4(&sc) + (threadIdx.x / LPP) : nullptr;
   stats_t stats = {};
   tc.stats = COUNT ? &stats : nullptr;
 
@@ -75,7 +76,7 @@
       hit_t isec;
       if (alive) {
         if (COUNT) count_quad<COUNT>(stats.rays);
-        isec = trace_ray<COUNT, GROUPS, !GENERAL, MODE>(tc, ps.ray, -1, &steps);
+        isec = trace_ray<COUNT, GROUPS, !GENERAL, MODE, ONCE>(tc, ps.ray, -1, &steps);
       }
       if (COUNT) {
         c1 = clock64(), cyc_trace += c1 - c0;
@@ -136,22 +137,23 @@
 }
 typedef void (*trace_kernel_t)(const yhd_scene, const yhd_state, int, yhd_counters*);
 #define YH_OCT_BLOCK 256
-template <bool COUNT, bool GENERAL, int BLOCK, int WAVES, int MODE = YH_MODE_QUAD>
+template <bool COUNT, bool GENERAL, int BLOCK, int WAVES, int MODE = YH_MODE_QUAD, bool ONCE = false>
 __global__ __launch_bounds__(BLOCK, WAVES) void k_trace(const yhd_scene sc, const yhd_state st,
     int nsamples, yhd_counters* counters) {
-  trace_items<COUNT, GENERAL, BLOCK, YH_SHADER_PATH, MODE>(sc, st, nsamples, counters);
+  static_assert(!ONCE || !GENERAL, "the prologue form exists for the plain variants");
+  trace_items<COUNT, GENERAL, BLOCK, YH_SHADER_PATH, MODE, ONCE>(sc, st, nsamples, counters);
 }
-template <bool GENERAL>
+template <bool GENERAL, bool ONCE = false>
 __global__ __launch_bounds__(YH_BLOCK, YH_MIN_WAVES) void k_trace_sbs(const yhd_scene sc, const yhd_state st, int nsamples, int oct_blocks,
     int quad_items, int oct_entries) {
   if ((int)blockIdx.x < oct_blocks) {
     yhd_state so   = st;
     so.tiles       = st.tiles + quad_items, so.num_tiles = oct_entries, so.tile_cursor = st.tile_cursor + 16;
-    trace_items<false, GENERAL, YH_BLOCK, YH_SHADER_PATH, YH_MODE_OCT>(sc, so, nsamples, nullptr, blockIdx.x, (unsigned)oct_blocks);
+    trace_items<false, GENERAL, YH_BLOCK, YH_SHADER_PATH, YH_MODE_OCT, ONCE>(sc, so, nsamples, nullptr, blockIdx.x, (unsigned)oct_blocks);
   } else {
     yhd_state sq = st;
     sq.num_tiles = quad_items;
-    trace_items<false, GENERAL, YH_BLOCK, YH_SHADER_PATH, YH_MODE_QUAD>(sc, sq, nsamples, nullptr, blockIdx.x - (unsigned)oct_blocks, gridDim.x - (unsigned)oct_blocks);
+    trace_items<false, GENERAL, YH_BLOCK, YH_SHADER_PATH, YH_MODE_QUAD, ONCE>(sc, sq, nsamples, nullptr, blockIdx.x - (unsigned)oct_blocks, gridDim.x - (unsigned)oct_blocks);
   }
 }
 #endif
diff --git a/yocto-hair_amd/csrc/dev_trace.h b/yocto-hair_amd/csrc/dev_trace.h
--- a/yocto-hair_amd/csrc/dev_trace.h
+++ b/yocto-hair_amd/csrc/dev_trace.h
@@ -142,6 +142,7 @@
   const YH_LDS v4f*     lds_mats;
   lane_stack*           ls;
   const yhd_scene*      sc_dev;
+  YH_LDS v4f*           lds_once;
 };
 YH_DEV void stage_tables(const yhd_scene& sc, YH_LDS v4f* at, int tid, int nthreads, trace_ctx& tc, YH_LDS float*& lds_cam) {
   tc.lds_scene = nullptr, tc.lds_lights = nullptr, tc.lds_envtab = nullptr, tc.lds_mats = nullptr;
@@ -203,7 +204,7 @@
 #define YH_IS_OCT(MODE) ((MODE) == YH_MODE_OCT || (MODE) == YH_MODE_OCTP)
 #define YH_MODE_HEXP 5
 #define YH_IS_HEX(MODE) ((MODE) == YH_MODE_HEX || (MODE) == YH_MODE_HEXP)
-template <bool COUNT, int STRIDE, bool EXACT, bool LDS_SCENE = false, int MODE = YH_MODE_QUAD>
+template <bool COUNT, int STRIDE, bool EXACT, bool LDS_SCENE = false, int MODE = YH_MODE_QUAD, bool ONCE = false>
 YH_DEV hit_t trace_ray_loop(const trace_ctx& tc, const ray_t& ray, int first_object, unsigned int* steps_out, bool& redo) {
   const yhd_scene&     sc   = *tc.sc;
   const unsigned int   q    = __lane_id() & 3u;
@@ -240,8 +241,43 @@
     if (in_lds) return ((const YH_LDS int*)(lds_snodes + 2 * sc.num_scene_nodes))[i];
     return sc.scene_prims[i];
   };
+  static_assert(!ONCE || (LDS_SCENE && !EXACT), "the prologue form reads the scene level from LDS and leaves NaN slabs to the second pass");
   unsigned int cur;
-  if (first_object >= 0) {
+  if constexpr (ONCE) {
+    cur = YH_NONE;
+    const v4f n0 = lds_snodes[0], n1 = lds_snodes[1];
+    if (q == 0) n_nodes++;
+    if (COUNT) count_branch<COUNT>(tc.stats->t_scene, tc.stats->l_scene);
+    if (COUNT) count_branch<COUNT>(tc.stats->t_enter, tc.stats->l_enter);
+    if (box_test(ray.o, wdinv, ray.tmin, tmax, xyz(n0), xyz(n1))) {
+      const int start = __float_as_int(n0.w), num = __float_as_int(n1.w) & 0xffff;
+      for (int k = num - 1; k >= 0; k--) {
+        const int         obj = scene_prim(start + k);
+        const YH_LDS v4f* ob  = tc.lds_scene + YH_OBJECT_F4 * obj;
+        const f3    it_min = (xyz(ob[8]) - ray.o) * wdinv, it_max = (xyz(ob[9]) - ray.o) * wdinv;
+        const float t0  = __builtin_fmaxf(__builtin_fmaxf(__builtin_fminf(it_min.x, it_max.x), __builtin_fminf(it_min.y, it_max.y)),
+            __builtin_fmaxf(__builtin_fminf(it_min.z, it_max.z), ray.tmin));
+        const float far = __builtin_fminf(__builtin_fminf(__builtin_fmaxf(it_min.x, it_max.x), __builtin_fmaxf(it_min.y, it_max.y)),
+            __builtin_fmaxf(it_min.z, it_max.z));
+        if (!(t0 <= __builtin_fminf(far, tmax) * 1.00000024f)) continue;
+        const v4f a = ob[3], b = ob[4], c = ob[5];
+        frame     inv;
+        inv.x = {a.x, a.y, a.z}, inv.y = {a.w, b.x, b.y}, inv.z = {b.z, b.w, c.x}, inv.o = {c.y, c.z, c.w};
+        const f3  o_ = transform_point(inv, ray.o), d_ = transform_vector(inv, ray.d), di = quad_rcp(d_);
+        const int sg = (di.x < 0 ? 1 : 0) | (di.y < 0 ? 2 : 0) | (di.z < 0 ? 4 : 0);
+        if (!(finite3(di) && finite3(o_))) redo = true;
+        const int root = __float_as_int(YH_IS_HEX(MODE) ? ob[10].w : YH_IS_OCT(MODE) ? ob[10].z : ob[10].x);
+        YH_LDS v4f* rec = tc.lds_once + 4 * k * STRIDE;
+        rec[0]          = v4f{o_.x, o_.y, o_.z, t0};
+        rec[STRIDE]     = v4f{d_.x, d_.y, d_.z, far};
+        rec[2 * STRIDE] = v4f{di.x, di.y, di.z, dot(d_, d_)};
+        rec[3 * STRIDE] = v4f{__int_as_float(sg), ob[6].x, __int_as_float(root), __int_as_float(obj)};
+        if (cur != YH_NONE) push(cur);
+        cur = YH_TAG_ENTER | (unsigned)k;
+      }
+    }
+    if (redo) cur = YH_NONE, sp = 0;
+  } else if (first_object >= 0) {
     cur = YH_TAG_ENTER | (unsigned)first_object;
   } else {
     if (sc.num_scene_nodes == 0) return hit;
@@ -255,6 +291,27 @@
     }
     unsigned int tag = cur & YH_TAG_MASK;
     bool scene_node = false;
+    if constexpr (ONCE) {
+      if (tag == YH_TAG_ENTER) {
+        if (COUNT) count_branch<COUNT>(tc.stats->t_enter, tc.stats->l_enter);
+        const YH_LDS v4f* rec;
+        v4f               r0, r1;
+        while (true) {
+          rec = tc.lds_once + 4 * (int)(cur & 3u) * STRIDE;
+          r0 = rec[0], r1 = rec[STRIDE];
+          if (r0.w <= __builtin_fminf(r1.w, tmax) * 1.00000024f) break;
+          cur = YH_NONE;
+          if (sp == 0) break;
+          cur = pop();
+        }
+        if (cur == YH_NONE) continue;
+        const v4f r2 = rec[2 * STRIDE], r3 = rec[3 * STRIDE];
+        lo = xyz(r0), ld = xyz(r1), ldinv = xyz(r2), ld2 = r2.w;
+        lsign = __float_as_int(r3.x), kind = __float_as_int(r3.y), node_base = __float_as_int(r3.z), cur_obj = __float_as_int(r3.w);
+        cur = YH_TAG_SHAPE | (unsigned)node_base;
+        tag = YH_TAG_SHAPE;
+      }
+    } else {
     if (!LDS_SCENE && tag == YH_TAG_SCENE && wide_scene) {
       if (COUNT) count_branch<COUNT>(tc.stats->t_scene, tc.stats->l_scene);
       const unsigned int low = cur & ~YH_TAG_MASK;
@@ -336,6 +393,7 @@
       if (HOIST_A) ld2 = dot(ld, ld);
       cur = YH_TAG_SHAPE | (unsigned)node_base;
       tag = YH_TAG_SHAPE;
+    }
     }
     {
       bool is_leaf    = tag == YH_TAG_LEAF;
@@ -517,10 +575,10 @@
 }
 #undef YH_STK
 
-template <bool COUNT, int STRIDE, bool LDS_SCENE = false, int MODE = YH_MODE_QUAD>
+template <bool COUNT, int STRIDE, bool LDS_SCENE = false, int MODE = YH_MODE_QUAD, bool ONCE = false>
 YH_DEV hit_t trace_ray(const trace_ctx& tc, const ray_t& ray, int first_object, unsigned int* steps_out = nullptr) {
   bool  redo = false;
-  hit_t hit  = trace_ray_loop<COUNT, STRIDE, false, LDS_SCENE, MODE>(tc, ray, first_object, steps_out, redo);
+  hit_t hit  = trace_ray_loop<COUNT, STRIDE, false, LDS_SCENE, MODE, ONCE>(tc, ray, first_object, steps_out, redo);
   if (__any(redo)) {
     if (redo) hit = trace_ray_loop<COUNT, STRIDE, true, LDS_SCENE, MODE>(tc, ray, first_object, steps_out, redo);
   }
diff --git a/yocto-hair_amd/csrc/kernels.hip b/yocto-hair_amd/csrc/kernels.hip
--- a/yocto-hair_amd/csrc/kernels.hip
+++ b/yocto-hair_amd/csrc/kernels.hip
@@ -368,7 +368,7 @@
 static_assert(yhd_shapes[YH_SHAPE_QUAD].block_threads == YH_BLOCK && yhd_shapes[YH_SHAPE_OCT].block_threads == YH_OCT_BLOCK && yhd_shapes[YH_SHAPE_HEX].block_threads == YH_OCT_BLOCK, "yhd_shapes");
 static int shape_block(int shape) { return yhd_shapes[shape].block_threads; }
 static int shape_groups(int shape) { return shape_block(shape) / yhd_shapes[shape].lanes_per_path; }
-static trace_kernel_t trace_kernel(bool counted, bool general, int shape, int shader = YH_SHADER_PATH) {
+static trace_kernel_t trace_kernel(bool counted, bool general, int shape, int shader = YH_SHADER_PATH, bool once = false) {
   if (shader == YH_SHADER_NAIVE) return k_trace_shader<YH_SHADER_NAIVE>;
   if (shader == YH_SHADER_EYELIGHT) return k_trace_shader<YH_SHADER_EYELIGHT>;
   if (shader == YH_SHADER_NORMAL) return k_trace_shader<YH_SHADER_NORMAL>;
@@ -378,13 +378,15 @@
   if (shape == YH_SHAPE_QUAD_DENSE)
     return counted ? (general ? k_trace<true, true, 256, YH_DENSE_WAVES> : k_trace<true, false, 256, YH_DENSE_WAVES>)
                    : (general ? k_trace<false, true, 256, YH_DENSE_WAVES> : k_trace<false, false, 256, YH_DENSE_WAVES>);
+  if (once && !general) return counted ? k_trace<true, false, YH_BLOCK, YH_MIN_WAVES, YH_MODE_QUAD, true> : k_trace<false, false, YH_BLOCK, YH_MIN_WAVES, YH_MODE_QUAD, true>;
   return counted ? (general ? k_trace<true, true, YH_BLOCK, YH_MIN_WAVES> : k_trace<true, false, YH_BLOCK, YH_MIN_WAVES>)
                  : (general ? k_trace<false, true, YH_BLOCK, YH_MIN_WAVES> : k_trace<false, false, YH_BLOCK, YH_MIN_WAVES>);
 }
 static size_t trace_lds(const yhd_scene* sc, int shape) {
   const int lanes   = yhd_shapes[shape].lanes_per_path;
   const int entries = lanes == 16 ? sc->stack_entries16 : lanes == 8 ? sc->stack_entries8 : sc->stack_entries;
-  return (size_t)(entries + YH_HITROWS) * shape_groups(shape) * 4 + (size_t)YHD_LDS_TABLES_F4(sc) * 16;
+  const size_t once = shape == YH_SHAPE_QUAD ? (size_t)YHD_ONCE_F4(sc, shape_groups(shape)) * 16 : 0;
+  return (size_t)(entries + YH_HITROWS) * shape_groups(shape) * 4 + (size_t)YHD_LDS_TABLES_F4(sc) * 16 + once;
 }
 int yhk_trace(const yhd_scene* sc, const yhd_state* st, int nsamples, yhd_counters* counters, int shape,
     int grid_blocks, hipStream_t stream) {
@@ -393,7 +395,7 @@
   if (!path && counters) return (int)hipErrorInvalidValue;
   if ((unsigned)shape >= YH_SHAPES || yhd_shapes[shape].kind == YH_SHAPE_KIND_STREAM || yhd_shapes[shape].kind == YH_SHAPE_KIND_SBS) return (int)hipErrorInvalidValue;
   size_t    lds   = trace_lds(sc, shape);
-  trace_kernel_t k     = trace_kernel(counters != nullptr, sc->general_materials != 0, shape, st->shader);
+  trace_kernel_t k     = trace_kernel(counters != nullptr, sc->general_materials != 0, shape, st->shader, sc->scene_once > 0);
   if (!k) return (int)hipErrorInvalidValue;
   if (lds > 64 * 1024) {
     hipError_t e = hipFuncSetAttribute((const void*)k, hipFuncAttributeMaxDynamicSharedMemorySize, (int)lds);
diff --git a/yocto-hair_amd/csrc/wide.hip b/yocto-hair_amd/csrc/wide.hip
--- a/yocto-hair_amd/csrc/wide.hip
+++ b/yocto-hair_amd/csrc/wide.hip
@@ -19,8 +19,9 @@
 }
 
 static size_t sbs_lds(const yhd_scene* sc) {
-  const size_t stacks = (size_t)std::max((sc->stack_entries + YH_HITROWS) * (YH_BLOCK / 4), (sc->stack_entries8 + YH_HITROWS) * (YH_BLOCK / 8)) * 4;
-  return stacks + (size_t)YHD_LDS_TABLES_F4(sc) * 16;
+  const size_t quads  = (size_t)(sc->stack_entries + YH_HITROWS) * (YH_BLOCK / 4) * 4 + (size_t)YHD_ONCE_F4(sc, YH_BLOCK / 4) * 16;
+  const size_t octets = (size_t)(sc->stack_entries8 + YH_HITROWS) * (YH_BLOCK / 8) * 4 + (size_t)YHD_ONCE_F4(sc, YH_BLOCK / 8) * 16;
+  return std::max(quads, octets) + (size_t)YHD_LDS_TABLES_F4(sc) * 16;
 }
 int yhk_trace_sbs_lds_bytes(const yhd_scene* sc) { return (int)sbs_lds(sc); }
 int yhk_trace_sbs_occupancy(int lds_bytes, int general) {
@@ -33,7 +34,7 @@
 int yhk_trace_sbs(const yhd_scene* sc, const yhd_state* st, int nsamples, int oct_blocks, int quad_items, int oct_entries, int grid_blocks,
     hipStream_t stream) {
   const size_t lds = sbs_lds(sc);
-  auto         k   = sc->general_materials ? k_trace_sbs<true> : k_trace_sbs<false>;
+  auto         k   = sc->general_materials ? k_trace_sbs<true> : sc->scene_once > 0 ? k_trace_sbs<false, true> : k_trace_sbs<false>;
   if (lds > 64 * 1024) {
     hipError_t e = hipFuncSetAttribute((const void*)k, hipFuncAttributeMaxDynamicSharedMemorySize, (int)lds);
     if (e != hipSuccess) return (int)e;
diff --git a/yocto-hair_amd/csrc/yh_device.h b/yocto-hair_amd/csrc/yh_device.h
--- a/yocto-hair_amd/csrc/yh_device.h
+++ b/yocto-hair_amd/csrc/yh_device.h
@@ -130,7 +130,10 @@
   int               stack_entries16;
   const yhd_float4* lane_blob;
   long long         lane_blob_units;
+  int               scene_once;
+  int               pad_once;
 } yhd_scene;
+#define YHD_ONCE_F4(sc, groups) (4 * (sc)->scene_once * (groups))
 #define YH_MATERIAL_F4 17
 #define YHD_LDS_TABLES_F4(sc) ((sc)->lds_scene_f4 + 5 + (sc)->light_table_f4 + ((sc)->env_tab_k + 3) / 4 + YH_MATERIAL_F4 * (sc)->lds_materials)
 
diff --git a/yocto-hair_amd/host/batch_api.cpp b/yocto-hair_amd/host/batch_api.cpp
--- a/yocto-hair_amd/host/batch_api.cpp
+++ b/yocto-hair_amd/host/batch_api.cpp
@@ -263,6 +263,32 @@
   HIPCHK(ctx, hipMemcpy(distance, dd, 4 * (size_t)n, hipMemcpyDeviceToHost));
   return YH_OK;
 }
+
+int yh_intersect_plain_batch(yh_context* ctx, int form, int n, const float* rays, int* object, int* element, float* uv, float* distance) {
+  if (!ctx || n < 0 || (form != 0 && form != 1) || (n && (!rays || !object || !element || !uv || !distance))) return YH_E_INVALID;
+  if (!ctx->have_scene) return fail(ctx, YH_E_STATE, "yh_intersect_plain_batch before yh_upload_scene");
+  if (ctx->scene.general_materials || ctx->scene.lds_scene_f4 == 0)
+    return fail(ctx, YH_E_INVALID, "yh_intersect_plain_batch: this scene renders with the GENERAL kernel variants (materials beyond diffuse / hair, a light read through memory, or tables too large for LDS)");
+  if (n == 0) return YH_OK;
+  HIPCHK(ctx, hipSetDevice(ctx->device));
+  Staged s(ctx);
+  auto   dr  = (float*)s.in(rays, 32 * (size_t)n);
+  auto   dob = (int*)s.out(4 * (size_t)n);
+  auto   del = (int*)s.out(4 * (size_t)n);
+  auto   duv = (float*)s.out(8 * (size_t)n);
+  auto   dd  = (float*)s.out(4 * (size_t)n);
+  if (s.rc) return s.rc;
+  int e = yhk_intersect_plain(&ctx->scene, form, n, dr, dob, del, duv, dd, ctx->stream);
+  if (e) return fail(ctx, YH_E_DEVICE, "k_intersect_plain launch: %s", hipGetErrorString((hipError_t)e));
+  YH_WAIT(ctx);
+  HIPCHK(ctx, hipMemcpy(object, dob, 4 * (size_t)n, hipMemcpyDeviceToHost));
+  HIPCHK(ctx, hipMemcpy(element, del, 4 * (size_t)n, hipMemcpyDeviceToHost));
+  HIPCHK(ctx, hipMemcpy(uv, duv, 8 * (size_t)n, hipMemcpyDeviceToHost));
+  HIPCHK(ctx, hipMemcpy(distance, dd, 4 * (size_t)n, hipMemcpyDeviceToHost));
+  return YH_OK;
+}
+
+int yh_scene_once(const yh_context* ctx) { return !ctx ? YH_E_INVALID : !ctx->have_scene ? YH_E_STATE : ctx->scene.scene_once; }
 
 int yh_lights_batch(yh_context* ctx, int form, int n, const float* position, const float* direction, const float* rn, float* out) {
   if (!ctx || n < 0 || (form != 0 && form != 1) || (n && (!position || !direction || !rn || !out))) return YH_E_INVALID;
diff --git a/yocto-hair_amd/host/context_internal.h b/yocto-hair_amd/host/context_internal.h
--- a/yocto-hair_amd/host/context_internal.h
+++ b/yocto-hair_amd/host/context_internal.h
@@ -66,6 +66,7 @@
 int yhk_surface_lobe(int, int, const float*, const float*, const float*, const float*, const float*, float*, hipStream_t);
 int yhk_surface_bsdf(int, const void*, const float*, const float*, const float*, const float*, float*, hipStream_t);
 int yhk_lights(const yhd_scene*, int, const float*, const float*, const float*, float*, hipStream_t);
+int yhk_intersect_plain(const yhd_scene*, int form, int, const float*, int*, int*, float*, float*, hipStream_t);
 int yhk_lights_lanes(const yhd_scene* sc, const yhd_scene* sc_dev, int n, const float* position, const float* direction, const float* rn,
     unsigned int* stack_ovf, int ovf_entries, float* out, hipStream_t stream);
 int yhk_selftest(int, float, float, uint64_t, uint64_t, int, const float*, double*, unsigned int*, hipStream_t);
diff --git a/yocto-hair_amd/host/scene_upload.cpp b/yocto-hair_amd/host/scene_upload.cpp
--- a/yocto-hair_amd/host/scene_upload.cpp
+++ b/yocto-hair_amd/host/scene_upload.cpp
@@ -600,6 +600,16 @@
     sc.lds_materials = sd->num_materials <= 24 ? sd->num_materials : 0;
     if (sc.lds_materials == 0 || sc.lds_scene_f4 == 0) sc.general_materials = 1;
   }
+  {
+    sc.scene_once = 0, sc.pad_once = 0;
+    if (!sc.general_materials && sc.num_scene_nodes == 1 && sc.num_objects >= 1 && sc.num_objects <= 4) {
+      const int quad0 = yhk_trace_occupancy(yhk_trace_lds_bytes(&sc, YH_SHAPE_QUAD), 0, YH_SHAPE_QUAD);
+      const int sbs0  = yhk_trace_sbs_occupancy(yhk_trace_sbs_lds_bytes(&sc), 0);
+      sc.scene_once = sc.num_objects;
+      if (yhk_trace_occupancy(yhk_trace_lds_bytes(&sc, YH_SHAPE_QUAD), 0, YH_SHAPE_QUAD) < quad0 || yhk_trace_sbs_occupancy(yhk_trace_sbs_lds_bytes(&sc), 0) < sbs0)
+        sc.scene_once = 0;
+    }
+  }
   ctx->scene      = sc;
   {
     uint64_t h = 1469598103934665603ULL;
diff --git a/yocto-hair_amd/python/yhair_capi.py b/yocto-hair_amd/python/yhair_capi.py
--- a/yocto-hair_amd/python/yhair_capi.py
+++ b/yocto-hair_amd/python/yhair_capi.py
@@ -165,6 +165,8 @@
     "yh_hair_pdf_batch": (C.c_int, [C.c_void_p, C.c_int, c_float_p, c_float_p, c_float_p, c_float_p]),
     "yh_hair_eval_pdf_batch": (C.c_int, [C.c_void_p, C.c_int, c_float_p, c_float_p, c_float_p, c_float_p]),
     "yh_intersect_batch": (C.c_int, [C.c_void_p, C.c_int, c_float_p, c_int_p, c_int_p, c_float_p, c_float_p]),
+    "yh_intersect_plain_batch": (C.c_int, [C.c_void_p, C.c_int, C.c_int, c_float_p, c_int_p, c_int_p, c_float_p, c_float_p]),
+    "yh_scene_once": (C.c_int, [C.c_void_p]),
     "yh_lights_batch": (C.c_int, [C.c_void_p, C.c_int, C.c_int, c_float_p, c_float_p, c_float_p, c_float_p]),
     "yh_selftest": (C.c_int, [C.c_void_p, C.c_int, c_float_p]),
     "yh_scene_load": (C.c_void_p, [C.c_char_p, C.c_char_p, C.c_char_p, C.c_int]),
@@ -412,6 +414,20 @@
         self._chk(self.lib.yh_intersect_batch(self.h, n, fptr(rays), iptr(obj), iptr(elem), fptr(uv), fptr(dist)))
         return obj, elem, uv, dist
 
+    def intersect_plain(self, form, rays):
+        rays = np.ascontiguousarray(rays, np.float32).reshape(-1, 8)
+        n = len(rays)
+        obj, elem = np.zeros(n, np.int32), np.zeros(n, np.int32)
+        uv, dist = np.zeros((n, 2), np.float32), np.zeros(n, np.float32)
+        self._chk(self.lib.yh_intersect_plain_batch(self.h, form, n, fptr(rays), iptr(obj), iptr(elem), fptr(uv), fptr(dist)))
+        return obj, elem, uv, dist
+
+    def scene_once(self):
+        rc = int(self.lib.yh_scene_once(self.h))
+        if rc < 0:
+            self._chk(rc)
+        return rc
+
     def lights(self, form, position, direction, rn4):
         a = [np.ascontiguousarray(x, np.float32) for x in (position, direction, rn4)]
         n = len(a[0])
diff --git a/yocto-hair_amd/unit/intersect_quad.hip b/yocto-hair_amd/unit/intersect_quad.hip
--- /dev/null
+++ b/yocto-hair_amd/unit/intersect_quad.hip
@@ -0,0 +1,49 @@
+#include <hip/hip_runtime.h>
+
+#include "yhair.h"
+#include "dev_path.h"
+
+using namespace yhd;
+
+#define YH_UQ_BLOCK 512
+template <int MODE, bool ONCE>
+__global__ __launch_bounds__(YH_UQ_BLOCK) void k_intersect_plain(const yhd_scene sc, int n, const float* rays, int* object, int* element,
+    float* uv, float* dist) {
+  constexpr int LPP = YH_IS_OCT(MODE) ? 8 : 4, GROUPS = YH_UQ_BLOCK / LPP;
+  extern __shared__ v4f lds_dyn[];
+  YH_LDS unsigned int* lds_stack = (YH_LDS unsigned int*)lds_dyn;
+  YH_LDS v4f*          lds_tabs  = (YH_LDS v4f*)(lds_stack + ((YH_IS_OCT(MODE) ? sc.stack_entries8 : sc.stack_entries) + YH_HITROWS) * GROUPS);
+  trace_ctx tc;
+  tc.sc = &sc, tc.ls = nullptr, tc.sc_dev = nullptr, tc.stats = nullptr;
+  YH_LDS float* lds_cam;
+  stage_tables(sc, lds_tabs, threadIdx.x, blockDim.x, tc, lds_cam);
+  __syncthreads();
+  tc.lds_stack = lds_stack + (threadIdx.x / LPP);
+  tc.lds_once  = ONCE ? lds_tabs + YHD_LDS_TABLES_F4(&sc) + (threadIdx.x / LPP) : nullptr;
+  int  i     = (int)((blockIdx.x * blockDim.x + threadIdx.x) / LPP);
+  bool valid = i < n;
+  if (!valid) i = n - 1;
+  const float* r   = rays + 8 * (size_t)i;
+  const ray_t  ray = ray_t{ld3(r), ld3(r + 3), r[6], r[7]};
+  const hit_t  h   = trace_ray<false, GROUPS, true, MODE, ONCE>(tc, ray, -1);
+  if (valid && (threadIdx.x & (LPP - 1)) == 0) {
+    object[i] = h.object, element[i] = hit_element(sc, h);
+    uv[2 * i] = h.u, uv[2 * i + 1] = h.v, dist[i] = h.distance;
+  }
+}
+
+extern "C" {
+int yhk_intersect_plain(const yhd_scene* sc, int form, int n, const float* rays, int* object, int* element, float* uv, float* dist, hipStream_t s) {
+  const int  lpp = form ? 8 : 4, groups = YH_UQ_BLOCK / lpp;
+  const bool once = sc->scene_once > 0;
+  const int  lds  = ((form ? sc->stack_entries8 : sc->stack_entries) + YH_HITROWS) * groups * 4 + YHD_LDS_TABLES_F4(sc) * 16 + YHD_ONCE_F4(sc, groups) * 16;
+  auto k = form ? (once ? k_intersect_plain<YH_MODE_OCT, true> : k_intersect_plain<YH_MODE_OCT, false>)
+                : (once ? k_intersect_plain<YH_MODE_QUAD, true> : k_intersect_plain<YH_MODE_QUAD, false>);
+  if (lds > 64 * 1024) {
+    hipError_t e = hipFuncSetAttribute((const void*)k, hipFuncAttributeMaxDynamicSharedMemorySize, lds);
+    if (e != hipSuccess) return (int)e;
+  }
+  hipLaunchKernelGGL(k, dim3((unsigned)(((long long)n + groups - 1) / groups)), dim3(YH_UQ_BLOCK), (size_t)lds, s, *sc, n, rays, object, element, uv, dist);
+  return (int)hipGetLastError();
+}
+}
```

Result: faster. 2682 (median of 6 runs) (+4.5%).
